# acerbilab/pyvbmc

Measured on AMD Instinct MI355X. Metric: ELBO+entropy evals/sec at D=10, K=50, N=400, Ns=1e6 (1e6-sample-equivalent evals/s), higher is better.
Workload: dtype f64; 1 GPU; BASELINE config 3 per GPU: D=10 K=50 N=400 S=1, Ns=1000000 MC samples per GPU (job Ns=1000000), value+grad _neg_elcbo with soft bounds, eps=philox; parallelism=single GPU

## Files before the change

### include/vbmc_hip.h

```cpp
#ifndef VBMC_HIP_H
#define VBMC_HIP_H

#include <stddef.h>
#include <stdint.h>

#ifdef __cplusplus
extern "C" {
#endif

typedef struct vbmc_ctx vbmc_ctx;

enum {
  VBMC_OK = 0,
  VBMC_E_ARG = -1,
  VBMC_E_HIP = -2,
  VBMC_E_RCCL = -3,
  VBMC_E_NODEV = -4,
  VBMC_E_UNSUP = -5,
  VBMC_E_NONFINITE = -6,
  VBMC_E_NOMEM = -7,
  VBMC_E_NOTPD = -8,
  VBMC_W_GP_CHANGED = 1,
  VBMC_W_NOT_FUSED = 2
};

enum { VBMC_MEAN_ZERO = 0, VBMC_MEAN_CONST = 1, VBMC_MEAN_NEGQUAD = 2 };

enum {
  VBMC_EPS_RESIDENT = 0,
  VBMC_EPS_PHILOX = 1
};


int vbmc_abi_version(void);

int vbmc_device_count(int* n_out);

int vbmc_ctx_create(int device_id, vbmc_ctx** out);
void vbmc_ctx_destroy(vbmc_ctx* ctx);

int vbmc_host_affinity(const vbmc_ctx* ctx, int* bound_out, int* n_cpus_out);

const char* vbmc_last_error(const vbmc_ctx* ctx);

int vbmc_device_info(const vbmc_ctx* ctx, char* name, int name_len, int* cu_count,
                     int* clock_khz, uint64_t* hbm_bytes);

int vbmc_synchronize(vbmc_ctx* ctx);

int vbmc_set_timing(vbmc_ctx* ctx, int on);

int vbmc_last_kernel_ms(vbmc_ctx* ctx, int which, double* ms_out);

int vbmc_last_host_us(const vbmc_ctx* ctx, double out[5]);
int vbmc_last_step_marks(const vbmc_ctx* ctx, double out[4]);
int vbmc_set_release_callback(vbmc_ctx* ctx, void (*fn)(void*), void* user);

int vbmc_set_option(vbmc_ctx* ctx, const char* key, int value);

int vbmc_last_entmc_plan(const vbmc_ctx* ctx, int out[4]);

int vbmc_ws_span_layout(int cus, int pb, int front, int nb, int pad, int K, int64_t* part_lo, int* first_part,
                        int* rows_per_component);

int vbmc_host_checksum(const double* const* ptrs, const int64_t* lens, int n, uint64_t* out);

int vbmc_set_gp_watch(vbmc_ctx* ctx, const double* const* ptrs, const int64_t* lens, int n, uint64_t expected);

int vbmc_armed_stats(const vbmc_ctx* ctx, uint64_t out[6]);

int vbmc_last_elbo_raw(const vbmc_ctx* ctx, double* out, int n);


int vbmc_set_mixture(vbmc_ctx* ctx, int D, int K, const double* mu_KxD,
                     const double* sigma_K, const double* lambd_D, const double* w_K,
                     const double* eta_K);

int vbmc_set_mixture_dk(vbmc_ctx* ctx, int D, int K, const double* mu_DxK,
                        const double* sigma_K, const double* lambd_D, const double* w_K,
                        const double* eta_K);

int vbmc_theta_to_mixture(vbmc_ctx* ctx, const double* theta, int n_theta,
                          int optimize_mask, double* mu_KxD, double* sigma_K,
                          double* lambd_D, double* w_K, double* eta_K);


int vbmc_mixture_pdf(vbmc_ctx* ctx, int64_t n, const double* x_nxD, int log_flag,
                     int grad_flag, double df, double* y_n, double* dy_nxD);


int vbmc_set_eps(vbmc_ctx* ctx, int K, int64_t n_half, int D, const double* eps_half,
                 int64_t row_begin, int64_t row_count);

int vbmc_mt19937_randn(uint32_t* key, int* pos, int* has_gauss, double* gauss, double* out,
                       int64_t n, int n_threads);

int vbmc_mt19937_randn_dev(vbmc_ctx* ctx, uint32_t* key, int* pos, int* has_gauss, double* gauss, double* out,
                           int64_t n);
int vbmc_randn_dev_info(const vbmc_ctx* ctx, int* window_reused);
int vbmc_mt_jump_host(const uint32_t* key_in, uint64_t n_words, uint32_t* key_out);
int vbmc_mt_jump_polys(uint64_t stride_words, int count, uint32_t* out);

int vbmc_set_eps_numpy(vbmc_ctx* ctx, uint32_t* key, int* pos, int* has_gauss, double* gauss, int K,
                       int64_t n_half, int D, int64_t row_begin, int64_t row_count, int n_threads);

int vbmc_entmc(vbmc_ctx* ctx, int64_t ns_per_comp, int eps_mode, uint64_t seed,
               int64_t row_begin, int64_t row_count, int grad_flags, int jacobian_flag,
               double* H, double* dH, double* raw_out);

int vbmc_philox_normals(vbmc_ctx* ctx, int K, int64_t n_half, int D, uint64_t seed, int64_t row_begin,
                        int64_t row_count, double* out);

int vbmc_entmc_finalize(vbmc_ctx* ctx, const double* raw, int grad_flags,
                        int jacobian_flag, double* H, double* dH);

int vbmc_entlb(vbmc_ctx* ctx, int grad_flags, int jacobian_flag, double* H, double* dH);


int vbmc_set_gp(vbmc_ctx* ctx, int N, int D, int S, int P, int mean_kind,
                const double* X_NxD, const double* hyp_SxP, const double* alpha_SxN,
                const double* L_SxNxN, const int32_t* L_chol_S, const double* sW_SxN,
                const double* sn2_mult_S);

int vbmc_gp_posterior(vbmc_ctx* ctx, int N, int D, int S, int P, int mean_kind, const double* X_NxD,
                      const double* y_N, const double* sn2_SxN, const double* sn2_div_S, const double* hyp_SxP,
                      double* alpha_SxN, double* L_SxNxN);

int vbmc_gp_append(vbmc_ctx* ctx, const double* x_D, double y, double* alpha_SxN1, double* L_SxN1xN1);

int vbmc_gp_append_noisy(vbmc_ctx* ctx, const double* x_D, double y, const double* sn2_new_S, double* alpha_SxN1,
                         double* L_SxN1xN1);

int vbmc_gp_fetch(vbmc_ctx* ctx, double* alpha_SxN, double* L_SxNxN);

int vbmc_gp_lml(vbmc_ctx* ctx, int N, int D, int B, int P, int mean_kind, const double* X_NxD, const double* y_N,
                const double* sn2_BxN, const double* sn2_div_B, const double* dsn2_B, const double* hyp_BxP, int want_grad,
                double* lml_B, double* dlml_BxP, int32_t* status_B);

int vbmc_gp_hyp_sample(vbmc_ctx* ctx, int N, int D, int P, int mean_kind, const double* X_NxD, const double* y_N,
                       const double* s2_N, int C, const double* x0_CxP, const double* widths_P, const double* lb_P,
                       const double* ub_P, const double* prior_mu_P, const double* prior_sigma_P, const double* prior_df_P,
                       int n, int thin, int burn_in, uint64_t seed, double* hyp_CxnxP, double* logpost_Cxn,
                       double* logprior_Cxn, int64_t* stats_Cx4, int32_t* invalid_C);

int vbmc_gp_hyp_optimize(vbmc_ctx* ctx, int N, int D, int P, int mean_kind, const double* X_NxD, const double* y_N,
                         const double* s2_N, int R, const double* x0_RxP, const double* lb_P, const double* ub_P,
                         const double* prior_mu_P, const double* prior_sigma_P, const double* prior_df_P, int max_iter, int m,
                         double tol_g, double tol_f, int trace_cap, double* hyp_RxP, double* logpost_R, double* grad_RxP,
                         int64_t* stats_Rx4, int32_t* invalid_R, double* trace_iter, double* trace_eval);

int vbmc_gp_fit(vbmc_ctx* ctx, int N, int D, int P, int mean_kind, const double* X_NxD, const double* y_N,
                const double* s2_N, int H, const double* hyp0_HxP, int init_N, const double* dlb_P, const double* dub_P,
                const double* lb_P, const double* ub_P, const double* prior_mu_P, const double* prior_sigma_P,
                const double* prior_df_P, int opts_N, int max_iter, int m, double tol_g, double tol_f, int n_samples,
                const double* widths_P, int thin, int burn_in, uint64_t seed, double* cand_BxP, double* score_B,
                int32_t* starts_R, double* opt_hyp_RxP, double* opt_logpost_R, int64_t* opt_stats_Rx4,
                int32_t* opt_invalid_R, double* best_P, double* best_logpost, double* hyp_SxP, double* logpost_S,
                double* logprior_S, int64_t* stats_Sx4, double* noise_S, int32_t* status, double* alpha_SxN,
                double* L_SxNxN);


int vbmc_gp_log_joint(vbmc_ctx* ctx, int grad_flags, int avg_flag, int jacobian_flag,
                      int compute_var, double* G, double* dG, double* varG,
                      double* var_ss, double* I_SxK, double* J_SxKxK);


int vbmc_gp_predict(vbmc_ctx* ctx, int64_t M, const double* xs_MxD, int add_noise,
                    int separate_samples, double* fmu, double* fs2);


typedef struct {
  int64_t ns_per_comp;
  int eps_mode;
  uint64_t seed;
  int compute_grad;
  int optimize_mask;
  int64_t row_begin;
  int64_t row_count;
  const double* bnd_lb;
  const double* bnd_ub;
  int n_bnd;
  double tol_con;
  double weight_threshold;
  double weight_penalty;
} vbmc_elbo_opts;

int vbmc_neg_elcbo(vbmc_ctx* ctx, double* theta, int n_theta, const vbmc_elbo_opts* opts,
                   double* F, double* dF, double* G, double* H, double* mu_KxD,
                   double* sigma_K, double* lambd_D, double* w_K, double* eta_K);

typedef struct vbmc_elbo_call {
  double* theta;
  int n_theta;
  const vbmc_elbo_opts* opts;
  double* F;
  double* dF;
  double* G;
  double* H;
  double* mu_KxD;
  double* sigma_K;
  double* lambd_D;
  double* w_K;
  double* eta_K;
} vbmc_elbo_call;
int vbmc_neg_elcbo_call(vbmc_ctx* ctx, const vbmc_elbo_call* c);


int vbmc_neg_elcbo_batch(vbmc_ctx* ctx, const double* thetas_BxN, int B, int n_theta,
                         const vbmc_elbo_opts* opts, double* F_B, double* G_B, double* H_B);


int vbmc_adam_begin(vbmc_ctx* ctx, const double* theta0, int n_theta, const vbmc_elbo_opts* opts,
                    const double* lb, const double* ub, int max_iter, double master_min,
                    double master_max, double master_decay);
int vbmc_adam_run_auto(vbmc_ctx* ctx, int max_iters, double tol_fun, int* n_done, double* y_tab_out,
                       double* x_tab_out, double* G_out, double* H_out);
int vbmc_adam_run(vbmc_ctx* ctx, int n_iters, double* y_tab_out, double* x_tab_out,
                  double* G_out, double* H_out);
int vbmc_adam_end(vbmc_ctx* ctx, double* theta_out, double* mu_KxD, double* sigma_K,
                  double* lambd_D, double* w_K, double* eta_K, int* iterations);


enum {
  VBMC_ACQ_STD = 0,
  VBMC_ACQ_LOG = 1,
  VBMC_ACQ_VANILLA = 2,
  VBMC_ACQ_NOISY = 3
};

int vbmc_acq_eval(vbmc_ctx* ctx, int64_t M, const double* xs_MxD, int kind, double y_max,
                  double tol_gp_var, const double* sn2_M, double* acq_M, double* f_bar_M,
                  double* var_tot_M);

int vbmc_acq_is_set(vbmc_ctx* ctx, int64_t Na, const double* Xa, int per_sample_xa,
                    const double* Ctmp_SxNxNa, const double* fs2a_NaxS, const double* lnw_SxNa);
int vbmc_acq_is_eval(vbmc_ctx* ctx, int64_t M, const double* xs_MxD, const double* sn2_M, double u,
                     double* acq_M, double* var_tot_M );

int vbmc_is_proposal(vbmc_ctx* ctx, int64_t Na, const double* Xa_NaxD, int K2, const double* mu2_KxD,
                     const double* sigma2_K, const double* lambd2_D, const double* w2_K, double w_vp,
                     const double* rect_delta_D, int ln_y_is_fmu, double* lnw_NaxS, double* fs2_NaxS,
                     int* invalid_out);
int vbmc_is_box_sample(vbmc_ctx* ctx, int64_t n_box, uint64_t seed, const double* rect_delta_D, double* x_NboxxD);
int vbmc_acq_is_build(vbmc_ctx* ctx, int64_t Na, const double* Xa, int per_sample_xa, const double* fs2a_NaxS,
                      const double* lnw_SxNa, double* K_out_SxNaxN, double* C_out_SxNxNa);

int vbmc_is_mcmc(vbmc_ctx* ctx, int ln_y_fmu, double u_q, const double* x0_SxD, const double* widths_D,
                 const double* lb_D, const double* ub_D, int n, int thin, int burn_in, uint64_t seed,
                 double* X_SxnxD, double* logp_Sxn, double* fmu_nxS, double* fs2_nxS,
                 int64_t* stats_Sx4 , int* invalid);

int vbmc_sq_dist(vbmc_ctx* ctx, int64_t n, int64_t m, int D, const double* a_nxD,
                 const double* b_mxD, double* c_nxm, int64_t* argmin_n);

enum { VBMC_SRC_COPY = 0, VBMC_SRC_TRANSFORM = 1, VBMC_SRC_MIXTURE = 2, VBMC_SRC_AFFINE = 3, VBMC_SRC_BOX = 4 };
enum { VBMC_ACQ_IS = 4 };
typedef struct vbmc_search_source {
  int kind;
  int64_t rows;
  const double* data;
  double df;
  uint64_t seed;
} vbmc_search_source;
int vbmc_search_fill(vbmc_ctx* ctx, int D, int n_src, const vbmc_search_source* src, const double* lb_search_D,
                     const double* ub_search_D, uint32_t integer_bits, int use_xf, double* X_out_MxD);
int vbmc_search_put(vbmc_ctx* ctx, int64_t M, int D, const double* X_MxD, uint32_t integer_bits, int use_xf);
int vbmc_search_eval(vbmc_ctx* ctx, int kind, double y_max, double tol_gp_var, double u, int64_t n_noise,
                     const double* X_rescaled_NxD, const double* sn2_new_N, const double* length_scale_D, int use_xf,
                     const double* lb_eps_orig_D, const double* ub_eps_orig_D, double* acq_M, int64_t* order_M,
                     double* X_sorted_MxD);

typedef struct vbmc_cmaes_opts {
  int lambda;
  int64_t max_fevals;
  double tol_fun;
  double tol_x;
  uint64_t seed;
} vbmc_cmaes_opts;
int vbmc_search_cmaes(vbmc_ctx* ctx, int kind, double y_max, double tol_gp_var, double u, int64_t n_noise,
                      const double* X_rescaled_NxD, const double* sn2_new_N, const double* length_scale_D, int use_xf,
                      const double* lb_eps_orig_D, const double* ub_eps_orig_D, int R, const double* x0_RxD,
                      const double* sigma0_R, const double* lb_D, const double* ub_D, uint32_t integer_bits,
                      const vbmc_cmaes_opts* opts, double* x_best_RxD, double* f_best_R, double* f0_R, double* mean_RxD,
                      double* sigma_R, double* C_RxDxD, int64_t* stats_Rx4);

typedef struct vbmc_sieve_fill_args {
  int D, K, K_new, optimize_mask;
  int64_t n1, n2, n3;
  const double* mu0_KxD;
  const double* sigma0_K;
  const double* lambd0_D;
  const double* w0_K;
  const double* mu2_KnxD;
  const double* sigma2_Kn;
  const double* lambd_s_D;
  int64_t N_star;
  const double* X_star_NxD;
  double v3;
  const double* Z_BxS;
  int n_slot;
  const int32_t* I_BxKn;
  uint64_t seed;
} vbmc_sieve_fill_args;
int vbmc_sieve_fill(vbmc_ctx* ctx, const vbmc_sieve_fill_args* args, double* thetas_out_BxN);
int vbmc_sieve_put(vbmc_ctx* ctx, int64_t B, int n_theta, const double* thetas_BxN);
int vbmc_sieve_eval(vbmc_ctx* ctx, const vbmc_elbo_opts* opts, double* F_B, double* G_B, double* H_B, int64_t* order_B,
                    double* thetas_sorted_BxN);

int vbmc_elcbo_full(vbmc_ctx* ctx, double* theta, int n_theta, int optimize_mask, int64_t ns_per_comp, int eps_mode,
                    uint64_t seed, int compute_var, double out[7], double* I_SxK, double* J_SxKxK);
int vbmc_elcbo_prune_trial(vbmc_ctx* ctx, int drop, int64_t ns_per_comp, int eps_mode, uint64_t seed, double out[7]);
int vbmc_elcbo_prune_accept(vbmc_ctx* ctx);
int vbmc_elcbo_put(vbmc_ctx* ctx, int S, int K0, const double* I_SxK0, const double* J_SxK0xK0);
int vbmc_elcbo_record_info(const vbmc_ctx* ctx, int64_t info[5], int32_t* alive_K0);


int vbmc_mixture_sample(vbmc_ctx* ctx, int64_t N, uint64_t seed, int balance_flag, double* x_NxD,
                        int32_t* comp_N);
int vbmc_mixture_sample_t(vbmc_ctx* ctx, int64_t N, uint64_t seed, int balance_flag, double df,
                          double* x_NxD, int32_t* comp_N);

int vbmc_kl_div_mc(vbmc_ctx* ctx, int64_t N, uint64_t seed, int K2, const double* mu2_KxD,
                   const double* sigma2_K, const double* lambd2_D, const double* w2_K,
                   double kl_out[2]);

int vbmc_set_transformer(vbmc_ctx* ctx, int slot, int D, const double* type_D, const double* lb_D,
                         const double* ub_D, const double* mu_D, const double* delta_D,
                         const double* R_DxD, const double* scale_D);
int vbmc_clear_transformer(vbmc_ctx* ctx, int slot);

enum { VBMC_XF_FORWARD = 0, VBMC_XF_INVERSE = 1, VBMC_XF_LOG_ABS_DET = 2 };
int vbmc_transform(vbmc_ctx* ctx, int64_t n, int direction, const double* in_nxD, double* out);

int vbmc_mixture_sample_orig(vbmc_ctx* ctx, int64_t N, uint64_t seed, int balance_flag, double df,
                             double* x_NxD, int32_t* comp_N);

int vbmc_mixture_pdf_orig(vbmc_ctx* ctx, int64_t n, const double* x_nxD, int log_flag, int grad_flag,
                          double df, double* y_n, double* dy_nxD);

int vbmc_mixture_moments_orig(vbmc_ctx* ctx, int64_t N, uint64_t seed, int cov_flag, double* mean_D,
                              double* cov_DxD);

int vbmc_kl_div_mc_orig(vbmc_ctx* ctx, int64_t N, uint64_t seed, int K2, const double* mu2_KxD,
                        const double* sigma2_K, const double* lambd2_D, const double* w2_K,
                        double kl_out[2]);

int vbmc_kde_1d(vbmc_ctx* ctx, int ncol, int64_t n, const double* x_colxn, int n_mesh, const double* lb_col,
                const double* ub_col, double* density_colxm, double* xmesh_colxm, double* bandwidth_col,
                int64_t* info_colx2);

enum { VBMC_MTV_HOST = 0, VBMC_MTV_MIX1 = 1, VBMC_MTV_MIX2 = 2 };
typedef struct vbmc_mtv_side {
  int source;
  int64_t n;
  const double* x_NxD;
  uint64_t seed;
  const double* lb_D;
  const double* ub_D;
} vbmc_mtv_side;

int vbmc_mtv(vbmc_ctx* ctx, int D, const vbmc_mtv_side* s1, const vbmc_mtv_side* s2, int K2,
             const double* mu2_KxD, const double* sigma2_K, const double* lambd2_D, const double* w2_K,
             double* mtv_D, int64_t* info_2Dx2);

int vbmc_mixture_mode(vbmc_ctx* ctx, int n_opts, int orig_flag, int64_t n, const double* cand_RxnxD,
                      uint64_t seed, int max_iter, double step_tol, double* x_D, double* f_out,
                      double* rec_Rx5, double* pts_RxD, double* ys_RxD);

enum { VBMC_WARP_FROM_OLD = 0, VBMC_WARP_FROM_ORIG = 1, VBMC_WARP_IN_NEW = 2 };

int vbmc_warp_points(vbmc_ctx* ctx, int D, int64_t n, int source, const double* x_NxD, double* y_NxD, double* lj_new_N,
                     double* lj_old_N);

int vbmc_warp_unscent(vbmc_ctx* ctx, int D, int64_t n, const double* x_NxD, int64_t sigma_rows, const double* sigma,
                      double* mean_NxD, double* std_NxD, double* pts_UxNxD);

int vbmc_warp_gp(vbmc_ctx* ctx, int D, int N, int S, int P, const double* X_NxD, const double* hyp_SxP,
                 double* logell_SxD, double* dy_mean, double* dy_old_mean);

int vbmc_warp_box(vbmc_ctx* ctx, int D, int64_t n, int source, const double* lo_D, const double* hi_D,
                  const double* u_NxD, uint64_t seed, int mode, double* out_2xD, double* sorted_Dxn);


int vbmc_comm_unique_id(uint8_t id_out[128]);
int vbmc_comm_init(vbmc_ctx* ctx, const uint8_t id[128], int rank, int world);
int vbmc_comm_destroy(vbmc_ctx* ctx);
int vbmc_comm_info(vbmc_ctx* ctx, int* rank_out, int* world_out);
int vbmc_comm_allreduce_max(vbmc_ctx* ctx, double* value_inout);
int vbmc_comm_barrier(vbmc_ctx* ctx);

#ifdef __cplusplus
}
#endif
#endif
```

### pyvbmc_amd/_lib.py

```python
import ctypes as C
import os
import sys
import threading
from pathlib import Path

import numpy as np

_HERE = Path(__file__).resolve().parent
LIB_PATH = Path(os.environ.get("VBMC_HIP_LIB", _HERE / "libvbmc_hip.so"))

EPS_RESIDENT, EPS_PHILOX = 0, 1
MEAN_ZERO, MEAN_CONST, MEAN_NEGQUAD = 0, 1, 2
E_ARG, E_HIP, E_RCCL, E_NODEV, E_UNSUP, E_NONFINITE = -1, -2, -3, -4, -5, -6
E_NOTPD = -8
W_GP_CHANGED = 1
W_NOT_FUSED = 2
T_ENTMC, T_GLJ, T_PDF, T_PREDICT, T_ELBO, T_PREDICT_VAR, T_GP_POST, T_IS_MCMC, T_GP_LML = range(9)
T_SEARCH_FILL, T_SEARCH_EVAL, T_SEARCH_SORT = 9, 10, 11
T_GP_HYP = 12
T_SEARCH_CMAES = 13
T_GP_OPT = 14
T_SIEVE_FILL, T_SIEVE_SCORE, T_SIEVE_RANK = 15, 16, 17


class VbmcHipError(RuntimeError):
    def __init__(self, code, msg):
        super().__init__(f"libvbmc_hip error {code}: {msg}")
        self.code = code


class NoDeviceError(VbmcHipError):
    pass


class UnsupportedShape(NotImplementedError):
    """VBMC_E_UNSUP: a shape the kernels do not cover (D > 32, a GP too large for the LDS plans ...).  A
    ``NotImplementedError`` -- there is no CPU fallback inside this package -- that ``pyvbmc_amd.patch`` recognises:
    under the drop-in such a call goes back to the reference callable it replaced (pyvbmc_amd/dropin.py)."""


_dp = C.POINTER(C.c_double)
_vp = C.c_void_p


class ElboOpts(C.Structure):
    _fields_ = [
        ("ns_per_comp", C.c_int64),
        ("eps_mode", C.c_int),
        ("seed", C.c_uint64),
        ("compute_grad", C.c_int),
        ("optimize_mask", C.c_int),
        ("row_begin", C.c_int64),
        ("row_count", C.c_int64),
        ("bnd_lb", _dp),
        ("bnd_ub", _dp),
        ("n_bnd", C.c_int),
        ("tol_con", C.c_double),
        ("weight_threshold", C.c_double),
        ("weight_penalty", C.c_double),
    ]


class ElboCall(C.Structure):

    _fields_ = [
        ("theta", _dp),
        ("n_theta", C.c_int),
        ("opts", C.POINTER(ElboOpts)),
        ("F", _dp),
        ("dF", _dp),
        ("G", _dp),
        ("H", _dp),
        ("mu_KxD", _dp),
        ("sigma_K", _dp),
        ("lambd_D", _dp),
        ("w_K", _dp),
        ("eta_K", _dp),
    ]


MTV_HOST, MTV_MIX1, MTV_MIX2 = 0, 1, 2
KDE_SCOTT, KDE_DEGENERATE, KDE_ROOT_STUCK = 1, 4, 8


class MtvSide(C.Structure):

    _fields_ = [
        ("source", C.c_int),
        ("n", C.c_int64),
        ("x_NxD", _dp),
        ("seed", C.c_uint64),
        ("lb_D", _dp),
        ("ub_D", _dp),
    ]


SRC_COPY, SRC_TRANSFORM, SRC_MIXTURE, SRC_AFFINE, SRC_BOX = range(5)
ACQ_IS = 4


class SearchSource(C.Structure):

    _fields_ = [
        ("kind", C.c_int),
        ("rows", C.c_int64),
        ("data", _dp),
        ("df", C.c_double),
        ("seed", C.c_uint64),
    ]


class SieveFillArgs(C.Structure):

    _fields_ = [
        ("D", C.c_int),
        ("K", C.c_int),
        ("K_new", C.c_int),
        ("optimize_mask", C.c_int),
        ("n1", C.c_int64),
        ("n2", C.c_int64),
        ("n3", C.c_int64),
        ("mu0_KxD", _dp),
        ("sigma0_K", _dp),
        ("lambd0_D", _dp),
        ("w0_K", _dp),
        ("mu2_KnxD", _dp),
        ("sigma2_Kn", _dp),
        ("lambd_s_D", _dp),
        ("N_star", C.c_int64),
        ("X_star_NxD", _dp),
        ("v3", C.c_double),
        ("Z_BxS", _dp),
        ("n_slot", C.c_int),
        ("I_BxKn", C.POINTER(C.c_int32)),
        ("seed", C.c_uint64),
    ]


class CmaesOpts(C.Structure):

    _fields_ = [
        ("lam", C.c_int),
        ("max_fevals", C.c_int64),
        ("tol_fun", C.c_double),
        ("tol_x", C.c_double),
        ("seed", C.c_uint64),
    ]


SIGNATURES = {
    "vbmc_abi_version": (C.c_int, []),
    "vbmc_device_count": (C.c_int, [C.POINTER(C.c_int)]),
    "vbmc_ctx_create": (C.c_int, [C.c_int, C.POINTER(_vp)]),
    "vbmc_ctx_destroy": (None, [_vp]),
    "vbmc_last_error": (C.c_char_p, [_vp]),
    "vbmc_device_info": (
        C.c_int,
        [_vp, C.c_char_p, C.c_int, C.POINTER(C.c_int), C.POINTER(C.c_int), C.POINTER(C.c_uint64)],
    ),
    "vbmc_host_affinity": (C.c_int, [_vp, C.POINTER(C.c_int), C.POINTER(C.c_int)]),
    "vbmc_synchronize": (C.c_int, [_vp]),
    "vbmc_set_option": (C.c_int, [_vp, C.c_char_p, C.c_int]),
    "vbmc_last_entmc_plan": (C.c_int, [_vp, C.POINTER(C.c_int)]),
    "vbmc_ws_span_layout": (C.c_int, [C.c_int, C.c_int, C.c_int, C.c_int, C.c_int, C.c_int, C.POINTER(C.c_int64),
                                      C.POINTER(C.c_int), C.POINTER(C.c_int)]),
    "vbmc_last_elbo_raw": (C.c_int, [_vp, _dp, C.c_int]),
    "vbmc_armed_stats": (C.c_int, [_vp, C.POINTER(C.c_uint64)]),
    "vbmc_set_gp_watch": (C.c_int, [_vp, C.POINTER(C.c_void_p), C.POINTER(C.c_int64), C.c_int, C.c_uint64]),
    "vbmc_host_checksum": (C.c_int, [C.POINTER(C.c_void_p), C.POINTER(C.c_int64), C.c_int, C.POINTER(C.c_uint64)]),
    "vbmc_set_timing": (C.c_int, [_vp, C.c_int]),
    "vbmc_last_kernel_ms": (C.c_int, [_vp, C.c_int, _dp]),
    "vbmc_last_host_us": (C.c_int, [_vp, _dp]),
    "vbmc_last_step_marks": (C.c_int, [_vp, _dp]),
    "vbmc_set_release_callback": (C.c_int, [_vp, C.c_void_p, C.c_void_p]),
    "vbmc_set_mixture": (C.c_int, [_vp, C.c_int, C.c_int, _dp, _dp, _dp, _dp, _dp]),
    "vbmc_set_mixture_dk": (C.c_int, [_vp, C.c_int, C.c_int, _dp, _dp, _dp, _dp, _dp]),
    "vbmc_theta_to_mixture": (C.c_int, [_vp, _dp, C.c_int, C.c_int, _dp, _dp, _dp, _dp, _dp]),
    "vbmc_mixture_pdf": (C.c_int, [_vp, C.c_int64, _dp, C.c_int, C.c_int, C.c_double, _dp, _dp]),
    "vbmc_set_eps": (C.c_int, [_vp, C.c_int, C.c_int64, C.c_int, _dp, C.c_int64, C.c_int64]),
    "vbmc_mt19937_randn": (
        C.c_int,
        [C.POINTER(C.c_uint32), C.POINTER(C.c_int), C.POINTER(C.c_int), _dp, _dp, C.c_int64, C.c_int],
    ),
    "vbmc_randn_dev_info": (C.c_int, [_vp, C.POINTER(C.c_int)]),
    "vbmc_mt19937_randn_dev": (
        C.c_int,
        [_vp, C.POINTER(C.c_uint32), C.POINTER(C.c_int), C.POINTER(C.c_int), _dp, _dp, C.c_int64],
    ),
    "vbmc_mt_jump_host": (C.c_int, [C.POINTER(C.c_uint32), C.c_uint64, C.POINTER(C.c_uint32)]),
    "vbmc_mt_jump_polys": (C.c_int, [C.c_uint64, C.c_int, C.POINTER(C.c_uint32)]),
    "vbmc_set_eps_numpy": (
        C.c_int,
        [_vp, C.POINTER(C.c_uint32), C.POINTER(C.c_int), C.POINTER(C.c_int), _dp, C.c_int, C.c_int64, C.c_int,
         C.c_int64, C.c_int64, C.c_int],
    ),
    "vbmc_entmc": (
        C.c_int,
        [_vp, C.c_int64, C.c_int, C.c_uint64, C.c_int64, C.c_int64, C.c_int, C.c_int, _dp, _dp, _dp],
    ),
    "vbmc_philox_normals": (C.c_int, [_vp, C.c_int, C.c_int64, C.c_int, C.c_uint64, C.c_int64, C.c_int64, _dp]),
    "vbmc_entmc_finalize": (C.c_int, [_vp, _dp, C.c_int, C.c_int, _dp, _dp]),
    "vbmc_entlb": (C.c_int, [_vp, C.c_int, C.c_int, _dp, _dp]),
    "vbmc_set_gp": (
        C.c_int,
        [_vp, C.c_int, C.c_int, C.c_int, C.c_int, C.c_int, _dp, _dp, _dp, _dp,
         C.POINTER(C.c_int32), _dp, _dp],
    ),
    "vbmc_gp_posterior": (
        C.c_int,
        [_vp, C.c_int, C.c_int, C.c_int, C.c_int, C.c_int, _dp, _dp, _dp, _dp, _dp, _dp, _dp],
    ),
    "vbmc_gp_append": (C.c_int, [_vp, _dp, C.c_double, _dp, _dp]),
    "vbmc_gp_append_noisy": (C.c_int, [_vp, _dp, C.c_double, _dp, _dp, _dp]),
    "vbmc_gp_fetch": (C.c_int, [_vp, _dp, _dp]),
    "vbmc_gp_lml": (
        C.c_int,
        [_vp, C.c_int, C.c_int, C.c_int, C.c_int, C.c_int, _dp, _dp, _dp, _dp, _dp, _dp, C.c_int, _dp, _dp,
         C.POINTER(C.c_int32)],
    ),
    "vbmc_gp_hyp_sample": (
        C.c_int,
        [_vp, C.c_int, C.c_int, C.c_int, C.c_int, _dp, _dp, _dp, C.c_int, _dp, _dp, _dp, _dp, _dp, _dp, _dp, C.c_int, C.c_int,
         C.c_int, C.c_uint64, _dp, _dp, _dp, C.POINTER(C.c_int64), C.POINTER(C.c_int32)],
    ),
    "vbmc_gp_hyp_optimize": (
        C.c_int,
        [_vp, C.c_int, C.c_int, C.c_int, C.c_int, _dp, _dp, _dp, C.c_int, _dp, _dp, _dp, _dp, _dp, _dp, C.c_int, C.c_int,
         C.c_double, C.c_double, C.c_int, _dp, _dp, _dp, C.POINTER(C.c_int64), C.POINTER(C.c_int32), _dp, _dp],
    ),
    "vbmc_gp_fit": (
        C.c_int,
        [_vp, C.c_int, C.c_int, C.c_int, C.c_int, _dp, _dp, _dp, C.c_int, _dp, C.c_int, _dp, _dp, _dp, _dp, _dp, _dp, _dp,
         C.c_int, C.c_int, C.c_int, C.c_double, C.c_double, C.c_int, _dp, C.c_int, C.c_int, C.c_uint64, _dp, _dp,
         C.POINTER(C.c_int32), _dp, _dp, C.POINTER(C.c_int64), C.POINTER(C.c_int32), _dp, _dp, _dp, _dp, _dp,
         C.POINTER(C.c_int64), _dp, C.POINTER(C.c_int32), _dp, _dp],
    ),
    "vbmc_gp_log_joint": (
        C.c_int,
        [_vp, C.c_int, C.c_int, C.c_int, C.c_int, _dp, _dp, _dp, _dp, _dp, _dp],
    ),
    "vbmc_gp_predict": (C.c_int, [_vp, C.c_int64, _dp, C.c_int, C.c_int, _dp, _dp]),
    "vbmc_neg_elcbo": (
        C.c_int,
        [_vp, _dp, C.c_int, C.POINTER(ElboOpts), _dp, _dp, _dp, _dp, _dp, _dp, _dp, _dp, _dp],
    ),
    "vbmc_neg_elcbo_call": (C.c_int, [_vp, C.POINTER(ElboCall)]),
    "vbmc_neg_elcbo_batch": (
        C.c_int,
        [_vp, _dp, C.c_int, C.c_int, C.POINTER(ElboOpts), _dp, _dp, _dp],
    ),
    "vbmc_adam_begin": (
        C.c_int,
        [_vp, _dp, C.c_int, C.POINTER(ElboOpts), _dp, _dp, C.c_int, C.c_double, C.c_double, C.c_double],
    ),
    "vbmc_adam_run": (C.c_int, [_vp, C.c_int, _dp, _dp, _dp, _dp]),
    "vbmc_adam_run_auto": (C.c_int, [_vp, C.c_int, C.c_double, C.POINTER(C.c_int), _dp, _dp, _dp, _dp]),
    "vbmc_adam_end": (C.c_int, [_vp, _dp, _dp, _dp, _dp, _dp, _dp, C.POINTER(C.c_int)]),
    "vbmc_acq_eval": (
        C.c_int,
        [_vp, C.c_int64, _dp, C.c_int, C.c_double, C.c_double, _dp, _dp, _dp, _dp],
    ),
    "vbmc_acq_is_set": (C.c_int, [_vp, C.c_int64, _dp, C.c_int, _dp, _dp, _dp]),
    "vbmc_acq_is_eval": (C.c_int, [_vp, C.c_int64, _dp, _dp, C.c_double, _dp, _dp]),
    "vbmc_is_proposal": (C.c_int, [_vp, C.c_int64, _dp, C.c_int, _dp, _dp, _dp, _dp, C.c_double, _dp, C.c_int, _dp, _dp,
                                   C.POINTER(C.c_int)]),
    "vbmc_is_box_sample": (C.c_int, [_vp, C.c_int64, C.c_uint64, _dp, _dp]),
    "vbmc_acq_is_build": (C.c_int, [_vp, C.c_int64, _dp, C.c_int, _dp, _dp, _dp, _dp]),
    "vbmc_is_mcmc": (C.c_int, [_vp, C.c_int, C.c_double, _dp, _dp, _dp, _dp, C.c_int, C.c_int, C.c_int, C.c_uint64, _dp, _dp,
                               _dp, _dp, C.POINTER(C.c_int64), C.POINTER(C.c_int)]),
    "vbmc_sq_dist": (C.c_int, [_vp, C.c_int64, C.c_int64, C.c_int, _dp, _dp, _dp, C.POINTER(C.c_int64)]),
    "vbmc_search_fill": (C.c_int, [_vp, C.c_int, C.c_int, C.POINTER(SearchSource), _dp, _dp, C.c_uint32, C.c_int, _dp]),
    "vbmc_search_put": (C.c_int, [_vp, C.c_int64, C.c_int, _dp, C.c_uint32, C.c_int]),
    "vbmc_search_eval": (C.c_int, [_vp, C.c_int, C.c_double, C.c_double, C.c_double, C.c_int64, _dp, _dp, _dp, C.c_int, _dp,
                                   _dp, _dp, C.POINTER(C.c_int64), _dp]),
    "vbmc_search_cmaes": (C.c_int, [_vp, C.c_int, C.c_double, C.c_double, C.c_double, C.c_int64, _dp, _dp, _dp, C.c_int, _dp,
                                    _dp, C.c_int, _dp, _dp, _dp, _dp, C.c_uint32, C.POINTER(CmaesOpts), _dp, _dp, _dp, _dp,
                                    _dp, _dp, C.POINTER(C.c_int64)]),
    "vbmc_sieve_fill": (C.c_int, [_vp, C.POINTER(SieveFillArgs), _dp]),
    "vbmc_sieve_put": (C.c_int, [_vp, C.c_int64, C.c_int, _dp]),
    "vbmc_sieve_eval": (C.c_int, [_vp, C.POINTER(ElboOpts), _dp, _dp, _dp, C.POINTER(C.c_int64), _dp]),
    "vbmc_elcbo_full": (C.c_int, [_vp, _dp, C.c_int, C.c_int, C.c_int64, C.c_int, C.c_uint64, C.c_int, _dp, _dp, _dp]),
    "vbmc_elcbo_prune_trial": (C.c_int, [_vp, C.c_int, C.c_int64, C.c_int, C.c_uint64, _dp]),
    "vbmc_elcbo_prune_accept": (C.c_int, [_vp]),
    "vbmc_elcbo_put": (C.c_int, [_vp, C.c_int, C.c_int, _dp, _dp]),
    "vbmc_elcbo_record_info": (C.c_int, [_vp, C.POINTER(C.c_int64), C.POINTER(C.c_int32)]),
    "vbmc_mixture_sample": (C.c_int, [_vp, C.c_int64, C.c_uint64, C.c_int, _dp, C.POINTER(C.c_int32)]),
    "vbmc_mixture_sample_t": (C.c_int, [_vp, C.c_int64, C.c_uint64, C.c_int, C.c_double, _dp, C.POINTER(C.c_int32)]),
    "vbmc_kl_div_mc": (C.c_int, [_vp, C.c_int64, C.c_uint64, C.c_int, _dp, _dp, _dp, _dp, _dp]),
    "vbmc_set_transformer": (C.c_int, [_vp, C.c_int, C.c_int, _dp, _dp, _dp, _dp, _dp, _dp, _dp]),
    "vbmc_clear_transformer": (C.c_int, [_vp, C.c_int]),
    "vbmc_transform": (C.c_int, [_vp, C.c_int64, C.c_int, _dp, _dp]),
    "vbmc_mixture_sample_orig": (C.c_int, [_vp, C.c_int64, C.c_uint64, C.c_int, C.c_double, _dp, C.POINTER(C.c_int32)]),
    "vbmc_mixture_pdf_orig": (C.c_int, [_vp, C.c_int64, _dp, C.c_int, C.c_int, C.c_double, _dp, _dp]),
    "vbmc_mixture_moments_orig": (C.c_int, [_vp, C.c_int64, C.c_uint64, C.c_int, _dp, _dp]),
    "vbmc_kl_div_mc_orig": (C.c_int, [_vp, C.c_int64, C.c_uint64, C.c_int, _dp, _dp, _dp, _dp, _dp]),
    "vbmc_kde_1d": (C.c_int, [_vp, C.c_int, C.c_int64, _dp, C.c_int, _dp, _dp, _dp, _dp, _dp, C.POINTER(C.c_int64)]),
    "vbmc_mtv": (C.c_int, [_vp, C.c_int, C.POINTER(MtvSide), C.POINTER(MtvSide), C.c_int, _dp, _dp, _dp, _dp, _dp,
                           C.POINTER(C.c_int64)]),
    "vbmc_mixture_mode": (C.c_int, [_vp, C.c_int, C.c_int, C.c_int64, _dp, C.c_uint64, C.c_int, C.c_double, _dp, _dp,
                                    _dp, _dp, _dp]),
    "vbmc_warp_points": (C.c_int, [_vp, C.c_int, C.c_int64, C.c_int, _dp, _dp, _dp, _dp]),
    "vbmc_warp_unscent": (C.c_int, [_vp, C.c_int, C.c_int64, _dp, C.c_int64, _dp, _dp, _dp, _dp]),
    "vbmc_warp_gp": (C.c_int, [_vp, C.c_int, C.c_int, C.c_int, C.c_int, _dp, _dp, _dp, _dp, _dp]),
    "vbmc_warp_box": (C.c_int, [_vp, C.c_int, C.c_int64, C.c_int, _dp, _dp, _dp, C.c_uint64, C.c_int, _dp, _dp]),
    "vbmc_comm_unique_id": (C.c_int, [C.POINTER(C.c_uint8)]),
    "vbmc_comm_init": (C.c_int, [_vp, C.POINTER(C.c_uint8), C.c_int, C.c_int]),
    "vbmc_comm_destroy": (C.c_int, [_vp]),
    "vbmc_comm_info": (C.c_int, [_vp, C.POINTER(C.c_int), C.POINTER(C.c_int)]),
    "vbmc_comm_allreduce_max": (C.c_int, [_vp, _dp]),
    "vbmc_comm_barrier": (C.c_int, [_vp]),
}

_lib = None
_lib_lock = threading.Lock()


def load():
    global _lib
    with _lib_lock:
        if _lib is None:
            if not LIB_PATH.exists():
                raise ImportError(
                    f"{LIB_PATH} not found: build it with `python -m pyvbmc_amd.build` "
                    "(hipcc, gfx950).  pyvbmc_amd has no CPU fallback."
                )
            lib = C.CDLL(str(LIB_PATH), mode=C.RTLD_GLOBAL)
            for name, (res, args) in SIGNATURES.items():
                fn = getattr(lib, name)
                fn.restype = res
                fn.argtypes = args
            _lib = lib
    return _lib


def device_count():
    n = C.c_int(0)
    load().vbmc_device_count(C.byref(n))
    return n.value


def f64(a):
    return np.ascontiguousarray(a, dtype=np.float64)


def ptr(a):
    if a is None:
        return None
    assert a.dtype == np.float64 and a.flags["C_CONTIGUOUS"]
    return a.ctypes.data_as(_dp)


def flags_to_bits(flags):
    if np.isscalar(flags):
        return 15 if flags else 0
    return sum((1 << i) for i, f in enumerate(flags) if f)


class Context:

    def __init__(self, device=None):
        lib = load()
        if device is None:
            device = int(os.environ.get("VBMC_HIP_DEVICE", os.environ.get("LOCAL_RANK", "0")))
        h = _vp()
        rc = lib.vbmc_ctx_create(int(device), C.byref(h))
        if rc != 0:
            msg = (lib.vbmc_last_error(None) or b"").decode()
            raise (NoDeviceError if rc == E_NODEV else VbmcHipError)(rc, msg)
        self._h = h
        self._lib = lib
        self.device = int(device)
        self.rank, self.world = 0, 1

    def close(self):
        if getattr(self, "_h", None):
            self.__dict__.pop("_fused_last", None)
            self.__dict__.pop("_fused_cache", None)
            vo = sys.modules.get(__package__ + ".variational_optimization")
            if vo is not None:
                fs = vo._fast_last[0]
                if fs is not None and fs.ctx is self:
                    vo._fast_last[0] = None
            self._lib.vbmc_ctx_destroy(self._h)
            self._h = None

    def __del__(self):
        try:
            self.close()
        except Exception:
            pass

    def check(self, rc):
        if rc != 0:
            msg = (self._lib.vbmc_last_error(self._h) or b"").decode()
            if rc == E_UNSUP:
                raise UnsupportedShape(msg)
            if rc == E_ARG:
                raise ValueError(msg)
            if rc == E_NODEV:
                raise NoDeviceError(rc, msg)
            if rc == E_NOTPD:
                raise np.linalg.LinAlgError(msg)
            raise VbmcHipError(rc, msg)

    def device_info(self):
        name = C.create_string_buffer(256)
        cu, clk, mem = C.c_int(), C.c_int(), C.c_uint64()
        self.check(self._lib.vbmc_device_info(self._h, name, 256, C.byref(cu), C.byref(clk), C.byref(mem)))
        return {"name": name.value.decode(), "cu_count": cu.value, "clock_khz": clk.value,
                "hbm_bytes": mem.value}

    def host_affinity(self):
        b, n = C.c_int(), C.c_int()
        self.check(self._lib.vbmc_host_affinity(self._h, C.byref(b), C.byref(n)))
        return bool(b.value), n.value

    def synchronize(self):
        self.check(self._lib.vbmc_synchronize(self._h))

    def set_timing(self, on):
        self.check(self._lib.vbmc_set_timing(self._h, int(on) if on else 0))

    def set_option(self, key, value):
        self.check(self._lib.vbmc_set_option(self._h, key.encode(), int(value)))

    def last_entmc_plan(self):
        out = (C.c_int * 4)()
        self.check(self._lib.vbmc_last_entmc_plan(self._h, out))
        return {"kernel": ("valu", "ws", "small", "mfma", "adam_fused", "ws", "ws")[out[0]] if out[0] >= 0 else None, "rg": out[1],
                "chunks": out[2], "resident_draws": bool(out[3] & 1), "roles": bool(out[3] & 2), "span": out[0] in (5, 6), "adam_tail": out[0] == 6}

    def philox_normals(self, K, n_half, D, seed, row_begin=0, row_count=None):
        row_count = n_half - row_begin if row_count is None else row_count
        out = np.empty((K, row_count, D))
        self.check(self._lib.vbmc_philox_normals(self._h, K, n_half, D, C.c_uint64(seed), row_begin, row_count, ptr(out)))
        return out

    def armed_stats(self):
        out = (C.c_uint64 * 6)()
        self.check(self._lib.vbmc_armed_stats(self._h, out))
        return dict(zip(("hits", "cancels", "late", "ident_checked", "ident_bad", "lost"), (int(v) for v in out)))

    def last_elbo_raw(self, D, K):
        out = np.empty(1 + D * K + 2 * K + D)
        self.check(self._lib.vbmc_last_elbo_raw(self._h, ptr(out), out.size))
        return out

    def last_kernel_ms(self, which=T_ENTMC):
        v = C.c_double()
        self.check(self._lib.vbmc_last_kernel_ms(self._h, which, C.byref(v)))
        return v.value

    def last_host_us(self):
        out = np.zeros(5)
        self.check(self._lib.vbmc_last_host_us(self._h, ptr(out)))
        return out

    def last_step_marks(self):
        out = np.zeros(4)
        self.check(self._lib.vbmc_last_step_marks(self._h, ptr(out)))
        return {"gp_word_us": out[0], "entropy_word_us": out[1],
                "gp_sums_in": ("prep launch", "finish launch", "entropy launch")[int(out[2])]}

    def set_mixture(self, mu_DK, sigma, lambd, w, eta):
        mu_DK = np.asarray(mu_DK, dtype=np.float64)
        D, K = mu_DK.shape
        mu_kd = f64(mu_DK.T)
        s, l, ww = f64(np.ravel(sigma)), f64(np.ravel(lambd)), f64(np.ravel(w))
        e = f64(np.ravel(eta)) if eta is not None and np.size(eta) == K else None
        if s.size != K or l.size != D or ww.size != K:
            raise ValueError("mixture attribute shapes do not match (D, K)")
        self.check(self._lib.vbmc_set_mixture(self._h, D, K, ptr(mu_kd), ptr(s), ptr(l), ptr(ww), ptr(e)))
        self.D, self.K = D, K

    def mixture_changed(self, D, K):
        self.__dict__["_vp_args"] = None
        self.D, self.K = int(D), int(K)
        vo = sys.modules.get(__package__ + ".variational_optimization")
        if vo is not None:
            vo.clear_fast_path()

    def set_eps(self, eps_half, row_begin=0, row_count=None):
        eps_half = f64(eps_half)
        K, h, D = eps_half.shape
        if row_count is None:
            row_count = h - row_begin
        self.check(self._lib.vbmc_set_eps(self._h, K, h, D, ptr(eps_half), row_begin, row_count))

    def set_eps_numpy(self, K, n_half, D, row_begin=0, row_count=None, threads=0, view=None):
        if row_count is None:
            row_count = n_half - row_begin
        with NP_STREAM_LOCK:
            left = self.__dict__.get("_np_left")
            fp = view() if view is not None and left is not None else None
            if fp is not None and fp == left and view._words is not None:
                bg, words = view._bg, view._words
                has_gauss, gauss = C.c_int(0), C.c_double(0.0)
                with bg.lock:
                    addr = C.addressof(words)
                    rc = self._lib.vbmc_set_eps_numpy(self._h, C.cast(addr, C.POINTER(C.c_uint32)),
                                                      C.cast(addr + 624 * 4, C.POINTER(C.c_int)), C.byref(has_gauss),
                                                      C.byref(gauss), K, n_half, D, row_begin, row_count,
                                                      threads or host_threads())
                    if has_gauss.value:
                        key = np.array(words[:624], dtype=np.uint32)
                        pos = int(words[624])
                if has_gauss.value:
                    np.random.set_state(("MT19937", key, pos, has_gauss.value, gauss.value))
                    self.__dict__["_np_left"] = None
                else:
                    self.__dict__["_np_left"] = view()
                self.check(rc)
                return True
            st = np.random.get_state(legacy=True)
            if not isinstance(st, tuple) or st[0] != "MT19937":
                return False
            key = np.array(st[1], dtype=np.uint32)
            pos, has_gauss, gauss = C.c_int(int(st[2])), C.c_int(int(st[3])), C.c_double(float(st[4]))
            rc = self._lib.vbmc_set_eps_numpy(self._h, key.ctypes.data_as(C.POINTER(C.c_uint32)), C.byref(pos),
                                              C.byref(has_gauss), C.byref(gauss), K, n_half, D, row_begin, row_count,
                                              threads or host_threads())
            np.random.set_state(("MT19937", key, pos.value, has_gauss.value, gauss.value))
            self.__dict__["_np_left"] = view() if view is not None and has_gauss.value == 0 else None
        self.check(rc)
        return True

    def comm_init(self, uid_bytes, rank, world):
        buf = (C.c_uint8 * 128).from_buffer_copy(uid_bytes)
        self.check(self._lib.vbmc_comm_init(self._h, buf, rank, world))
        self.rank, self.world = rank, world

    def comm_info(self):
        r, w = C.c_int(), C.c_int()
        self.check(self._lib.vbmc_comm_info(self._h, C.byref(r), C.byref(w)))
        return r.value, w.value

    def comm_barrier(self):
        self.check(self._lib.vbmc_comm_barrier(self._h))

    def comm_max(self, value):
        v = C.c_double(value)
        self.check(self._lib.vbmc_comm_allreduce_max(self._h, C.byref(v)))
        return v.value


def comm_unique_id():
    buf = (C.c_uint8 * 128)()
    rc = load().vbmc_comm_unique_id(buf)
    if rc != 0:
        raise VbmcHipError(rc, (load().vbmc_last_error(None) or b"").decode())
    return bytes(buf)


NP_STREAM_LOCK = threading.Lock()


def host_threads():
    try:
        n = len(os.sched_getaffinity(0))
    except (AttributeError, OSError):
        n = os.cpu_count() or 1
    return max(1, min(64, n))


_default_ctx = None


def default_context():
    global _default_ctx
    if _default_ctx is None:
        _default_ctx = Context()
    return _default_ctx


def set_default_context(ctx):
    global _default_ctx
    _default_ctx = ctx
```

### pyvbmc_amd/csrc/api_elbo.hip

```cpp
#include <algorithm>
#include <chrono>
#include <cstdlib>
#include <cmath>
#include <cstring>

#include "common.h"
#include "entropy_args.h"

static double soft_bound_loss(const std::vector<double>& x, const double* lb, const double* ub,
                              double tol_con, std::vector<double>* dy) {
  double y = 0.0;
  if (dy) dy->assign(x.size(), 0.0);
  for (size_t i = 0; i < x.size(); ++i) {
    if (x[i] >= lb[i] && x[i] <= ub[i]) continue;
    const double ell = (ub[i] - lb[i]) * tol_con;
    if (x[i] < lb[i]) {
      const double t = (lb[i] - x[i]) / ell;
      y += 0.5 * t * t;
      if (dy) (*dy)[i] = (x[i] - lb[i]) / (ell * ell);
    }
    if (x[i] > ub[i]) {
      const double t = (x[i] - ub[i]) / ell;
      y += 0.5 * t * t;
      if (dy) (*dy)[i] = (x[i] - ub[i]) / (ell * ell);
    }
  }
  return y;
}

#ifdef FIN_TIMES
static int64_t g_host_stamps[64][6];
static uint64_t g_host_n = 0;
static inline int64_t host_ns() {
  return std::chrono::duration_cast<std::chrono::nanoseconds>(std::chrono::steady_clock::now().time_since_epoch()).count();
}
namespace {
__global__ void clock_stamp_kernel(unsigned long long* out) {
  if (threadIdx.x == 0) __hip_atomic_store(out, (unsigned long long)wall_clock64(), __ATOMIC_RELAXED, __HIP_MEMORY_SCOPE_SYSTEM);
}
}
extern "C" int vbmc_debug_host_stamps(int64_t* out) {
  memcpy(out, g_host_stamps, sizeof(g_host_stamps));
  return (int)(g_host_n & 63);
}
extern "C" int vbmc_debug_clock_pair(vbmc_ctx* ctx, int64_t* host_before, int64_t* host_after, unsigned long long* gpu) {
  volatile unsigned long long* f = (volatile unsigned long long*)(ctx->h_done + 6);
  *f = 0;
  (void)hipStreamSynchronize(ctx->stream);
  *host_before = host_ns();
  hipLaunchKernelGGL(clock_stamp_kernel, dim3(1), dim3(64), 0, ctx->stream, (unsigned long long*)(ctx->hd_done + 6));
  while (*f == 0) __builtin_ia32_pause();
  *host_after = host_ns();
  *gpu = *f;
  return 0;
}
#define HSTAMP(i) g_host_stamps[g_host_n & 63][i] = host_ns()
#else
#define HSTAMP(i) (void)0
#endif

static inline uint64_t* ctl_word(vbmc_ctx* ctx, uint64_t seq) { return ctx->d_ctl + (seq & 7); }

void spec_disarm(vbmc_ctx* ctx) {
  vbmc_ctx::ArmedEval& sp = ctx->spec;
  if (!sp.armed) return;
  *(volatile uint64_t*)ctl_word(ctx, sp.seq) = ~(uint64_t)0;
  __builtin_ia32_sfence();
  sp.armed = false;
  ++sp.cancels;
  ctx->gen_cur = sp.gen_cur_before;
  ctx->ahead.valid = sp.ahead_before_valid;
  ctx->ahead.seed = sp.ahead_before_seed;
  ctx->ahead.buf = sp.ahead_before_buf;
  ctx->ahead.frac = sp.ahead_before_frac;
}

extern "C" int vbmc_neg_elcbo(vbmc_ctx* ctx, double* theta, int n_theta,
                              const vbmc_elbo_opts* opts, double* F, double* dF, double* G,
                              double* H, double* mu_KxD, double* sigma_K, double* lambd_D,
                              double* w_K, double* eta_K) {
  if (!ctx || !theta || !opts) return VBMC_E_ARG;
  struct KeepArmed {
    vbmc_ctx* c;
    explicit KeepArmed(vbmc_ctx* c_) : c(c_) { c->spec.keep = true; }
    ~KeepArmed() { c->spec.keep = false; }
  } keep_armed(ctx);
  NEED_DEVICE(ctx);
  if (!ctx->mix_set) return vbmc_fail(ctx, VBMC_E_ARG, "neg_elcbo: mixture (D,K) not set");
  if (!ctx->gp.set) return vbmc_fail(ctx, VBMC_E_ARG, "neg_elcbo: GP not set");
  if (ctx->gp.D != ctx->D) return vbmc_fail(ctx, VBMC_E_ARG, "neg_elcbo: GP/mixture D mismatch");
  using clk = std::chrono::steady_clock;
  const auto t_begin = clk::now();
  HSTAMP(0);
  auto us_since = [](clk::time_point a) {
    return std::chrono::duration<double, std::micro>(clk::now() - a).count();
  };
  const int D = ctx->D, K = ctx->K;
  const int mask = opts->optimize_mask;
  const ThetaMap tm(D, K, mask, n_theta);
  ctx->defer_mix_upload = true;
  int rc = vbmc_theta_to_mixture(ctx, theta, n_theta, mask, mu_KxD, sigma_K, lambd_D, w_K, eta_K);
  ctx->defer_mix_upload = false;
  if (rc) return rc;
  if (tm.o_w()) {
    double* e = theta + (n_theta - K);
    double mx = e[0];
    for (int k = 1; k < K; ++k) mx = e[k] > mx ? e[k] : mx;
    for (int k = 0; k < K; ++k) e[k] -= mx;
  }
  const int grad_flags = opts->compute_grad ? mask : 0;
  const GpState& g = ctx->gp;
  const int S = g.S;
  const int st = 1 + 2 * D;
  const size_t n_res = (size_t)S * K * st;
  const int n_raw = raw_len(D, K);
  const bool mc = opts->ns_per_comp > 0;
  const bool lb_dev = !mc && K > 1;

  int64_t row_begin = opts->row_begin, row_count = opts->row_count;
  if (mc) {
    if (opts->ns_per_comp & 1)
      return vbmc_fail(ctx, VBMC_E_ARG, "neg_elcbo: ns_per_comp must be even");
    rc = resolve_row_slice(ctx, opts, "neg_elcbo", &row_begin, &row_count);
    if (rc) return rc;
  }

  rc = ensure_pinned(ctx, n_res + (size_t)n_raw);
  if (rc) return rc;
  double* hp_dev = ctx->hp_dev;
  double* res_out = hp_dev;
  double* raw_host = hp_dev + n_res;
  const bool multi = ctx_is_multi(ctx);
  double* raw_out = raw_host;
  if (multi && mc) {
    rc = ensure_dev(ctx, &ctx->d_out, &ctx->d_out_cap, (size_t)n_raw);
    if (rc) return rc;
    raw_out = ctx->d_out;
  }

  ctx->host_us[0] = us_since(t_begin);
  const auto t_launch = clk::now();
  const bool can_poll = mc;
  double* stage = nullptr;
  if (can_poll) {
    rc = ensure_dev(ctx, &ctx->d_stage, &ctx->d_stage_cap, n_res + (size_t)n_raw);
    if (rc) return rc;
    stage = ctx->d_stage;
  }
  vbmc_ctx::ArmedEval& sp = ctx->spec;
  constexpr double ARM_MAX_EVAL_US = 1000.0, ARM_LIMIT_MS = 0.3, ARM_DEVICE_WAIT_MS = 0.5;
  const bool arm_allowed = ctx->opt_elbo_arm >= 2 || (ctx->opt_elbo_arm == 1 && vbmc_live_contexts_on(ctx->device) <= 1);
  const bool arm_next = can_poll && !multi && arm_allowed && ctx->opt_mix_bar && !ctx->timing &&
                        opts->eps_mode == VBMC_EPS_PHILOX && ctx->host_us[4] <= ARM_MAX_EVAL_US;
  constexpr double ARM_LATE_SLACK_MS = 0.15;
  const double arm_limit_ms = 1e-3 * ctx->host_us[4] + ARM_LIMIT_MS;
  static_assert(ARM_LIMIT_MS + ARM_LATE_SLACK_MS < ARM_DEVICE_WAIT_MS, "the host's cut-off must come before the device's");

  bool polled = false;
  uint64_t cur_seq = 0;
  bool ident_out_flag = false;
  auto issue = [&](uint64_t seed, bool spin, bool& polled_out, uint64_t& seq_out) -> int {
    int rc2;
    PrepArgs pa;
    glj_fill_prep(ctx, grad_flags != 0, res_out, nullptr, pa);
    EntPlan plan;
    if (mc) {
      rc2 = entmc_plan(ctx, opts->ns_per_comp, opts->eps_mode, seed, row_begin, row_count, grad_flags != 0, plan,
                       pa.n_glj);
      if (rc2) return rc2;
      entmc_fill_prep(ctx, plan, pa);
      rc2 = entmc_pregen(ctx, plan, pa);
      if (rc2) return rc2;
    }
    const bool ahead_ok = can_poll && opts->eps_mode == VBMC_EPS_PHILOX && ctx->opt_elbo_ahead &&
                          plan.a.eps != nullptr && plan.a.eps == ctx->d_epsgen[ctx->gen_cur];
    const bool ws_form = plan.kernel == EntKernel::Ws || plan.kernel == EntKernel::WsSpan || plan.kernel == EntKernel::Mfma;
    if (spin && !(ahead_ok && plan.pregen_hit && ws_form))
      return -1000;
    if (can_poll) {
      pa.done.cnt = ctx->d_done_cnt + 8;
      pa.done.flag = ctx->hd_done + 4;
      pa.done.seq = ++ctx->done_seq;
      pa.done.host_out = res_out;
      pa.done.host_n = (int)n_res;
      pa.res = stage;
    }
    seq_out = ctx->done_seq;
    ident_out_flag = false;
    ctx->gp_where = 0;
    double* fg = nullptr;
    if (can_poll && ctx->opt_mix_bar) fg = spin ? ctx->d_mix_fg : write_pack_to_device(ctx);
    if (spin && !fg) return -1000;
    const bool ident = fg != nullptr && mc;
    if (ident) pa.ident_out = (uint64_t*)(ctx->d_done_cnt + 12);
    if (fg) {
      PrepArgs gp_tail = pa;
      gp_tail.n_table = 0;
      gp_tail.gen = GenSlice();
      gp_tail.mix = ctx->d_mix;
      if (entmc_take_gp(ctx, plan, gp_tail)) {
        pa.n_glj = 0;
        ctx->gp_where = 2;
      }
      if (mc && pa.n_glj > 0 && pa.done.flag != nullptr && ctx->opt_gp_ship && plan.kernel == EntKernel::Mfma) {
        plan.a.ship_src = pa.res;
        plan.a.ship_dst = pa.done.host_out;
        plan.a.ship_n = pa.done.host_n;
        plan.a.ship_flag = pa.done.flag;
        plan.a.ship_seq = pa.done.seq;
        pa.done = DoneSignal();
      }
      pa.mix = fg;
      pa.mix_copy = ctx->d_mix;
      pa.mix_copy_n = ctx->ml.total;
    } else {
      rc2 = upload_packed_mixture(ctx);
      if (rc2) return rc2;
    }
    uint64_t* ctl = nullptr;
    if (spin) {
      ctl = ctl_word(ctx, seq_out);
      *(volatile uint64_t*)ctl = 0;
      __builtin_ia32_sfence();
      pa.go = ctl;
      pa.go_seq = seq_out;
      pa.go_timeout = (uint64_t)(ARM_DEVICE_WAIT_MS * 1e5);
      pa.dead = ctx->hd_done + 5;
      plan.a.cancel = ctl;
    }
    HSTAMP(1);
    rc2 = launch_prep(ctx, pa);
    if (rc2) return rc2;
    polled_out = false;
    if (mc) {
      rc2 = entmc_launch_main(ctx, plan);
      if (rc2) return rc2;
      GenSlice ahead_gen;
      DoneSignal done;
      if (can_poll) {
        if (ahead_ok) ahead_gen = entmc_ahead_slice(ctx, plan);
        done.cnt = ctx->d_done_cnt;
        done.sub = ctx->d_done_sub;
        {
          static const int sub_min = [] { const char* e = getenv("VBMC_FIN_SUB_MIN"); return e ? atoi(e) : 256; }();
          done.sub_min = sub_min;
        }
        done.flag = ctx->hd_done;
        done.seq = seq_out;
        done.host_out = raw_out;
        done.host_n = n_raw;
        done.cancel = ctl;
        if (ident) {
          done.ident_src = (const uint64_t*)(ctx->d_done_cnt + 12);
          done.ident_dst = ctx->hd_done + 1;
          done.ident_seed = seed;
        }
        polled_out = true;
        ident_out_flag = ident;
      }
      const GenSlice* gen_here = ahead_gen.n_blocks > 0 ? &ahead_gen : nullptr;
      if (!multi) {
        rc2 = entmc_launch_finish(ctx, plan, polled_out ? stage + n_res : raw_out, gen_here, polled_out ? &done : nullptr);
        if (rc2) return rc2;
      } else {
        rc2 = entmc_launch_finish(ctx, plan, raw_out, nullptr, nullptr);
        if (rc2) return rc2;
        rc2 = comm_allreduce_sum(ctx, raw_out, n_raw);
        if (rc2) return rc2;
        if (polled_out) {
          done.host_out = raw_host;
          rc2 = entmc_launch_publish(ctx, raw_out, done, gen_here);
          if (rc2) return rc2;
        } else {
          HIP_TRY(ctx, hipMemcpyAsync(ctx->h_pinned + n_res, raw_out, sizeof(double) * n_raw,
                                      hipMemcpyDeviceToHost, ctx->stream));
        }
      }
    } else if (lb_dev) {
      rc2 = launch_entlb(ctx, raw_host);
      if (rc2) return rc2;
    }
    return 0;
  };

  uint64_t want_ck = 0;
  bool check_ident = false;
  bool used_armed = false;
  if (sp.armed) {
    const bool match = can_poll && sp.seed == opts->seed && sp.n_theta == n_theta && sp.mask == mask &&
                       sp.grad_flags == grad_flags && sp.eps_mode == opts->eps_mode &&
                       sp.ns_per_comp == opts->ns_per_comp && sp.row_begin == row_begin && sp.row_count == row_count &&
                       !ctx->timing &&
                       std::chrono::duration<double, std::milli>(clk::now() - sp.t_armed).count() < sp.limit_ms;
    if (match) {
      memcpy(ctx->d_mix_fg, ctx->h_pack, sizeof(double) * (size_t)ctx->ml.total);
      __builtin_ia32_sfence();
      *(volatile uint64_t*)ctl_word(ctx, sp.seq) = sp.seq;
      __builtin_ia32_sfence();
      ctx->pack_valid = true;
      sp.armed = false;
      const bool force_late = ctx->opt_arm_late_test > 0 && --ctx->opt_arm_late_test == 0;
      if (!force_late && std::chrono::duration<double, std::milli>(clk::now() - sp.t_armed).count() < sp.limit_ms + ARM_LATE_SLACK_MS) {
        ++sp.hits;
        used_armed = true;
        polled = true;
        cur_seq = sp.seq;
        check_ident = sp.ident;
        HSTAMP(1);
      } else {
        *(volatile uint64_t*)ctl_word(ctx, sp.seq) = ~(uint64_t)0;
        __builtin_ia32_sfence();
        HIP_TRY(ctx, stream_wait(ctx));
        HIP_TRY(ctx, hipMemsetAsync(ctx->d_done_cnt, 0, sizeof(int) * 16, ctx->stream));
        HIP_TRY(ctx, hipMemsetAsync(ctx->d_done_sub, 0, sizeof(int) * 16 * 64, ctx->stream));
        ctx->gen_cur = sp.gen_cur_before;
        ctx->ahead.valid = sp.ahead_before_valid;
        ctx->ahead.seed = sp.ahead_before_seed;
        ctx->ahead.buf = sp.ahead_before_buf;
        ctx->ahead.frac = sp.ahead_before_frac;
        ++sp.cancels;
        ++sp.late;
      }
    } else {
      spec_disarm(ctx);
    }
  }
  if (!used_armed) {
    rc = issue(opts->seed, false, polled, cur_seq);
    if (rc) return rc;
    check_ident = polled && ident_out_flag;
  }
  if (mc && can_poll && ctx->opt_mix_bar) want_ck = pack_checksum(ctx->h_pack, (size_t)ctx->ml.total);
  ctx->step_marks[2] = (double)ctx->gp_where;
  if (polled && arm_next && ctx->d_ctl && ctx->d_mix_fg) {
    sp.gen_cur_before = ctx->gen_cur;
    sp.ahead_before_valid = ctx->ahead.valid;
    sp.ahead_before_seed = ctx->ahead.seed;
    sp.ahead_before_buf = ctx->ahead.buf;
    sp.ahead_before_frac = ctx->ahead.frac;
    const uint64_t seq_before = ctx->done_seq;
    bool p2 = false;
    uint64_t seq2 = 0;
    const auto t_arm0 = clk::now();
    const int rc2 = issue(opts->seed + 1, true, p2, seq2);
    if (rc2 == 0 && p2) {
      sp.armed = true;
      sp.ident = ident_out_flag;
      sp.limit_ms = arm_limit_ms;
      sp.t_armed = t_arm0;
      sp.seq = seq2;
      sp.seed = opts->seed + 1;
      sp.n_theta = n_theta;
      sp.mask = mask;
      sp.grad_flags = grad_flags;
      sp.eps_mode = opts->eps_mode;
      sp.ns_per_comp = opts->ns_per_comp;
      sp.row_begin = row_begin;
      sp.row_count = row_count;
    } else if (rc2 == -1000) {
      ctx->done_seq = seq_before;
      ctx->gen_cur = sp.gen_cur_before;
      ctx->ahead.valid = sp.ahead_before_valid;
      ctx->ahead.seed = sp.ahead_before_seed;
      ctx->ahead.buf = sp.ahead_before_buf;
      ctx->ahead.frac = sp.ahead_before_frac;
    } else if (rc2 != 0) {
      return rc2;
    }
  }
  if (ctx->release_cb && !ctx->ident_retry) ctx->release_cb(ctx->release_cb_user);
  ElboScratch& sc = ctx->elbo;
  const bool has_bnd = opts->bnd_lb && opts->bnd_ub;
  double F_bnd = 0.0;
  std::vector<double>& dFb = sc.dFb;
  if (has_bnd && grad_flags) dFb.assign((size_t)n_theta, 0.0);
  if (has_bnd) {
    if (tm.n_bnd() != opts->n_bnd)
      return vbmc_fail(ctx, VBMC_E_ARG, "neg_elcbo: bounds length %d != %d", opts->n_bnd, tm.n_bnd());
    std::vector<double>& ext = sc.ext;
    ext.resize((size_t)tm.n_bnd());
    const int sc0 = tm.p_sg;
    for (int i = 0; i < tm.n_bnd(); ++i) ext[i] = tm.bound_coord(i, theta, ctx->sigma.data(), ctx->lambd.data());
    std::vector<double>& dL = sc.dL;
    const double L = soft_bound_loss(ext, opts->bnd_lb, opts->bnd_ub, opts->tol_con,
                                     grad_flags ? &dL : nullptr);
    F_bnd += L;
    if (grad_flags) {
      if (tm.o_mu())
        for (int i = 0; i < D * K; ++i) dFb[i] += dL[i];
      if (tm.o_sg())
        for (int k = 0; k < K; ++k) {
          double a = 0.0;
          for (int d = 0; d < D; ++d) a += dL[sc0 + d * K + k];
          dFb[tm.p_sg + k] += a;
        }
      if (tm.o_lm())
        for (int d = 0; d < D; ++d) {
          double a = 0.0;
          for (int k = 0; k < K; ++k) a += dL[sc0 + d * K + k];
          dFb[tm.p_lm + d] += a;
        }
      if (tm.o_w())
        for (int k = 0; k < K; ++k) dFb[tm.p_w + k] += dL[dL.size() - K + k];
    }
    if (tm.o_w()) {
      const double th = opts->weight_threshold, pen = opts->weight_penalty;
      double a = 0.0;
      std::vector<double>& wg = sc.wpen;
      wg.resize(K);
      for (int k = 0; k < K; ++k) {
        const bool small = ctx->w[k] < th;
        a += small ? ctx->w[k] : th;
        wg[k] = small ? pen : 0.0;
      }
      F_bnd += a * pen;
      if (grad_flags) {
        std::vector<double>& jw = sc.jw;
        jw.resize(K);
        softmax_jacobian_apply(ctx, wg.data(), jw.data());
        for (int k = 0; k < K; ++k) dFb[n_theta - K + k] += jw[k];
      }
    }
  }
  bool gp_changed = false;
  if (!ctx->gp_watch_ptrs.empty()) {
    uint64_t ck = 0;
    vbmc_host_checksum(ctx->gp_watch_ptrs.data(), ctx->gp_watch_lens.data(), (int)ctx->gp_watch_ptrs.size(), &ck);
    gp_changed = ck != ctx->gp_watch_ck;
  }
  ctx->host_us[1] = us_since(t_launch);
  HSTAMP(2);
  const auto t_wait = clk::now();
  auto spin_on = [&](const volatile uint64_t* f, uint64_t want) -> int {
    const volatile uint64_t* dead = ctx->h_done + 5;
    unsigned spins = 0;
    for (;;) {
      if (*f == want) break;
      if (*dead == want) return 1;
      __builtin_ia32_pause();
      if ((++spins & 0xFFFF) == 0 && us_since(t_wait) > 5e6) return 2;
    }
    __atomic_thread_fence(__ATOMIC_ACQUIRE);
    return 0;
  };
  auto redo_unarmed = [&](const char* why) -> int {
    HIP_TRY(ctx, stream_wait(ctx));
    HIP_TRY(ctx, hipMemsetAsync(ctx->d_done_cnt, 0, sizeof(int) * 16, ctx->stream));
        HIP_TRY(ctx, hipMemsetAsync(ctx->d_done_sub, 0, sizeof(int) * 16 * 64, ctx->stream));
    ctx->ahead.valid = false;
    if (ctx->ident_retry) return vbmc_fail(ctx, VBMC_E_HIP, "neg_elcbo: %s, twice in a row", why);
    ctx->ident_retry = true;
    const int arm_was = ctx->opt_elbo_arm;
    ctx->opt_elbo_arm = 0;
    const int rc3 = vbmc_neg_elcbo(ctx, theta, n_theta, opts, F, dF, G, H, mu_KxD, sigma_K, lambd_D, w_K, eta_K);
    ctx->opt_elbo_arm = arm_was;
    ctx->ident_retry = false;
    ctx->spec.keep = true;
    return rc3;
  };
  GljHost& o = sc.glj;
  double Gv = 0.0;
  std::vector<double>&dGv = sc.dG, &dHv = sc.dH;
  auto finalize_gp = [&]() -> int {
    glj_finalize(ctx, ctx->h_pinned, grad_flags != 0, o);
    for (int s = 0; s < S; ++s) Gv += o.G[s];
    Gv /= S;
    dGv.assign((size_t)n_theta, 0.0);
    if (grad_flags) {
      std::vector<double>&mu = sc.mu, &sg = sc.sg, &lm = sc.lm, &wg = sc.wg;
      mu.assign((size_t)K * D, 0.0);
      sg.assign(K, 0.0);
      lm.assign(D, 0.0);
      wg.assign(K, 0.0);
      for (int s = 0; s < S; ++s) {
        for (int i = 0; i < K * D; ++i) mu[i] += o.mu[(size_t)s * K * D + i] / S;
        for (int k = 0; k < K; ++k) sg[k] += o.sigma[(size_t)s * K + k] / S;
        for (int d = 0; d < D; ++d) lm[d] += o.lambd[(size_t)s * D + d] / S;
        for (int k = 0; k < K; ++k) wg[k] += o.w[(size_t)s * K + k] / S;
      }
      const int n = glj_pack(ctx, mu.data(), sg.data(), lm.data(), wg.data(), grad_flags, 1, dGv.data());
      if (n != n_theta) return vbmc_fail(ctx, VBMC_E_ARG, "neg_elcbo: gradient length %d != n_theta %d", n, n_theta);
    }
    return 0;
  };
  bool gp_done = false;
  if (polled) {
    int st_w = spin_on(ctx->h_done + 4, cur_seq);
    HSTAMP(3);
    ctx->step_marks[0] = us_since(t_begin);
    if (st_w == 0) {
      rc = finalize_gp();
      if (rc) return rc;
      gp_done = true;
      st_w = spin_on(ctx->h_done, cur_seq);
    }
    if (st_w != 0) {
      ++sp.lost;
      return redo_unarmed(st_w == 1 ? "the armed launches gave up before the go word reached them"
                                    : "no completion word from the device after 5 s");
    }
    if (check_ident) {
      const volatile uint64_t* id = ctx->h_done + 1;
      ++sp.ident_checked;
      const bool force_bad = ctx->opt_ident_test > 0 && --ctx->opt_ident_test == 0;
      if (force_bad || id[0] != want_ck || id[1] != opts->seed) {
        ++sp.ident_bad;
        return redo_unarmed("the result block does not identify as this evaluation");
      }
    }
  } else {
    HIP_TRY(ctx, stream_wait(ctx));
  }
  ctx->pack_in_flight = false;
  ctx->step_marks[1] = us_since(t_begin);
  if (!polled) ctx->step_marks[0] = ctx->step_marks[1];
  ctx->host_us[2] = us_since(t_wait);
  HSTAMP(4);
  const auto t_fin = clk::now();
  if (!gp_done) {
    rc = finalize_gp();
    if (rc) return rc;
  }
  dHv.assign((size_t)n_theta, 0.0);
  double Hv = 0.0;
  if (mc || lb_dev) {
    const double* r = ctx->h_pinned + n_res;
    entropy_pack(ctx, r[0], r + 1, r + 1 + D * K, r + 1 + D * K + K, r + 1 + D * K + K + D,
                 grad_flags, 1, &Hv, grad_flags ? dHv.data() : nullptr);
  } else {
    rc = vbmc_entlb(ctx, grad_flags, 1, &Hv, grad_flags ? dHv.data() : nullptr);
    if (rc) return rc;
  }
  ctx->last_raw_off = n_res;
  ctx->last_raw_n = mc ? n_raw : 0;
  double Fv = -Gv - Hv;
  std::vector<double>& dFv = sc.dF;
  dFv.assign((size_t)n_theta, 0.0);
  if (grad_flags)
    for (int i = 0; i < n_theta; ++i) dFv[i] = -dGv[i] - dHv[i];

  Fv += F_bnd;
  if (grad_flags && has_bnd)
    for (int i = 0; i < n_theta; ++i) dFv[i] += dFb[i];
  ctx->host_us[3] = us_since(t_fin);
  ctx->host_us[4] = us_since(t_begin);
#ifdef FIN_TIMES
  HSTAMP(5);
  ++g_host_n;
#endif
  if (F) *F = Fv;
  if (G) *G = Gv;
  if (H) *H = Hv;
  if (dF && grad_flags) memcpy(dF, dFv.data(), sizeof(double) * n_theta);
  return gp_changed ? VBMC_W_GP_CHANGED : VBMC_OK;
}

extern "C" int vbmc_neg_elcbo_call(vbmc_ctx* ctx, const vbmc_elbo_call* c) {
  if (!c) return VBMC_E_ARG;
  return vbmc_neg_elcbo(ctx, c->theta, c->n_theta, c->opts, c->F, c->dF, c->G, c->H, c->mu_KxD, c->sigma_K, c->lambd_D, c->w_K,
                        c->eta_K);
}

extern "C" int vbmc_armed_stats(const vbmc_ctx* ctx, uint64_t out[6]) {
  if (!ctx || !out) return VBMC_E_ARG;
  const vbmc_ctx::ArmedEval& sp = ctx->spec;
  out[0] = sp.hits;
  out[1] = sp.cancels;
  out[2] = sp.late;
  out[3] = sp.ident_checked;
  out[4] = sp.ident_bad;
  out[5] = sp.lost;
  return VBMC_OK;
}

extern "C" int vbmc_last_elbo_raw(const vbmc_ctx* ctx, double* out, int n) {
  if (!ctx || !out || ctx->last_raw_n <= 0 || n != ctx->last_raw_n || !ctx->h_pinned) return VBMC_E_ARG;
  memcpy(out, ctx->h_pinned + ctx->last_raw_off, sizeof(double) * (size_t)n);
  return VBMC_OK;
}

extern "C" int vbmc_set_release_callback(vbmc_ctx* ctx, void (*fn)(void*), void* user) {
  if (!ctx) return VBMC_E_ARG;
  ctx->release_cb = fn;
  ctx->release_cb_user = user;
  return VBMC_OK;
}

extern "C" int vbmc_last_step_marks(const vbmc_ctx* ctx, double out[4]) {
  if (!ctx || !out) return VBMC_E_ARG;
  for (int i = 0; i < 4; ++i) out[i] = ctx->step_marks[i];
  return VBMC_OK;
}

extern "C" int vbmc_last_host_us(const vbmc_ctx* ctx, double out[5]) {
  if (!ctx || !out) return VBMC_E_ARG;
  for (int i = 0; i < 5; ++i) out[i] = ctx->host_us[i];
  return VBMC_OK;
}
```

### pyvbmc_amd/csrc/common.h

```cpp
#pragma once
#include <hip/hip_runtime.h>
#include <chrono>

#include <cstdint>
#include <cstdio>
#include <string>
#include <vector>

#include "../../include/vbmc_hip.h"
#include "gp_cand_host.h"
#include "gp_fit_host.h"
#include "scratch.h"
#include "transform.h"

struct ncclComm;

struct MixLayout {
  int D = 0, K = 0;
  int o_mup = 0;
  int o_mu = 0;
  int o_is2 = 0;
  int o_wc = 0;
  int o_rc = 0;
  int o_lrc = 0;
  int o_sig = 0;
  int o_w = 0;
  int o_lam = 0;
  int o_ilam = 0;
  int total = 0;
  void plan(int D_, int K_) {
    D = D_;
    K = K_;
    int o = 0;
    o_mup = o; o += K * D;
    o_mu = o; o += K * D;
    o_is2 = o; o += K;
    o_wc = o; o += K;
    o_rc = o; o += K;
    o_lrc = o; o += K;
    o_sig = o; o += K;
    o_w = o; o += K;
    o_lam = o; o += D;
    o_ilam = o; o += D;
    total = o;
  }
};

struct ThetaMap {
  int D, K;
  int mask;
  __host__ __device__ bool o_mu() const { return mask & 1; }
  __host__ __device__ bool o_sg() const { return mask & 2; }
  __host__ __device__ bool o_lm() const { return mask & 4; }
  __host__ __device__ bool o_w() const { return mask & 8; }
  int p_sg, p_lm, p_w;
  int n_sc;
  __host__ __device__ ThetaMap(int D_, int K_, int mask_) : ThetaMap(D_, K_, mask_, 0) { p_w = n_theta() - K; }
  __host__ __device__ ThetaMap(int D_, int K_, int mask_, int n_theta_)
      : D(D_), K(K_), mask(mask_), p_sg((mask_ & 1) ? D_ * K_ : 0), p_lm(p_sg + ((mask_ & 2) ? K_ : 0)), p_w(n_theta_ - K_),
        n_sc((mask_ & 6) ? D_ * K_ : 0) {}
  __host__ __device__ int n_theta() const { return p_lm + (o_lm() ? D : 0) + (o_w() ? K : 0); }
  __host__ __device__ int n_bnd() const { return p_sg + n_sc + (o_w() ? K : 0); }
  __host__ __device__ bool in_mu(int i) const { return o_mu() && i < D * K; }
  __host__ __device__ bool in_sg(int i) const { return o_sg() && i >= p_sg && i < p_sg + K; }
  __host__ __device__ bool in_lm(int i) const { return o_lm() && i >= p_lm && i < p_lm + D; }
  __host__ __device__ int raw_w() const { return 1 + D * K + K + D; }
  __host__ __device__ int raw_index(int i) const {
    if (o_w() && i >= p_w) return raw_w() + (i - p_w);
    if (o_lm() && i >= p_lm) return 1 + D * K + K + (i - p_lm);
    if (o_sg() && i >= p_sg) return 1 + D * K + (i - p_sg);
    return 1 + i;
  }
  __host__ __device__ double bound_coord(int i, const double* theta, const double* sigma, const double* lambda) const {
    double x;
    if (i < p_sg) {
      x = theta[i];
    } else if (i < p_sg + n_sc) {
      const int q = i - p_sg, k = q / D, d = q - k * D;
      const double ls = o_sg() ? theta[p_sg + k] : log(sigma[k]);
      const double ll = o_lm() ? theta[p_lm + d] : log(lambda[d]);
      x = ll + ls;
    } else {
      x = theta[p_w + (i - p_sg - n_sc)];
    }
    return x;
  }
};

struct GpState {
  bool set = false;
  int N = 0, D = 0, S = 0, P = 0, mean_kind = 0;
  std::vector<double> hyp;
  std::vector<int32_t> L_chol;
  std::vector<double> sn2_eff;
  std::vector<double> sn2_mult;
  double* d_X = nullptr;
  double* d_XT = nullptr;
  double* d_alpha = nullptr;
  double* d_L = nullptr;
  double* d_Linv = nullptr;
  double* d_LinvP = nullptr;
  double* d_sW = nullptr;
  double* d_hyp = nullptr;
  double* d_xc = nullptr;
  double* d_smeta = nullptr;
  size_t cap_X = 0, cap_XT = 0, cap_alpha = 0, cap_L = 0, cap_Linv = 0, cap_LinvP = 0, cap_sW = 0, cap_hyp = 0, cap_xc = 0, cap_smeta = 0;
  std::vector<double> h_small;
  std::vector<double> h_XT;
  bool dev_built = false;
  bool homo = false;
  double* d_y = nullptr;
  double* d_r = nullptr;
  double* d_sn2 = nullptr;
  double* d_sl = nullptr;
  size_t cap_y = 0, cap_r = 0, cap_sn2 = 0, cap_sl = 0;
  std::vector<double> h_X, h_y, h_sl;
  std::vector<double> h_sn2;
};

struct GljHost {
  std::vector<double> G;
  std::vector<double> I_sk;
  std::vector<double> mu;
  std::vector<double> sigma;
  std::vector<double> lambd;
  std::vector<double> w;
};

struct ElboScratch {
  GljHost glj;
  std::vector<double> dG, dH, dF, dFb, mu, sg, lm, wg, ext, dL, wpen, jw;
};

enum TimingPair { T_ENTMC = 0, T_GLJ, T_PDF, T_PREDICT, T_ELBO, T_PREDICT_VAR, T_GP_POST, T_IS_MCMC, T_GP_LML, T_SEARCH_FILL,
                  T_SEARCH_EVAL, T_SEARCH_SORT, T_GP_HYP, T_SEARCH_CMAES, T_GP_OPT, T_SIEVE_FILL, T_SIEVE_SCORE, T_SIEVE_RANK, T_COUNT };

struct vbmc_ctx {
  int device = 0;
  hipStream_t stream = nullptr;
  hipEvent_t ev[2 * T_COUNT] = {};
  bool ev_valid[T_COUNT] = {};
  std::string err;
  hipDeviceProp_t prop;

  bool mix_set = false;
  int D = 0, K = 0;
  std::vector<double> mu, sigma, lambd, w, eta;
  MixLayout ml;
  double* d_mix = nullptr;
  struct ArmedEval {
    bool armed = false;
    bool keep = false;
    uint64_t seq = 0;
    uint64_t seed = 0;
    int n_theta = 0, mask = 0, grad_flags = 0, eps_mode = 0;
    int64_t ns_per_comp = 0, row_begin = 0, row_count = 0;
    int gen_cur_before = 0;
    bool ahead_before_valid = false;
    uint64_t ahead_before_seed = 0;
    int ahead_before_buf = 0;
    double ahead_before_frac = 1.0;
    uint64_t hits = 0, cancels = 0, late = 0, ident_checked = 0, ident_bad = 0, lost = 0;
    bool ident = false;
    double limit_ms = 1.0;
    std::chrono::steady_clock::time_point t_armed;
  } spec;
  uint64_t* d_ctl = nullptr;
  double* d_stage = nullptr;
  size_t d_stage_cap = 0;
  double* d_mix_fg = nullptr;
  std::vector<double> mu_scratch;
  std::vector<double> t2m_mu, t2m_sg, t2m_lm, t2m_w, t2m_eta;
  double* d_acq_fg = nullptr;
  bool acq_fg_failed = false;
  uint64_t acq_seq = 0;
  size_t d_mix_fg_cap = 0;
  bool mix_fg_failed = false;
  size_t d_mix_cap = 0;

  double* d_epsgen[2] = {nullptr, nullptr};
  size_t d_epsgen_cap[2] = {0, 0};
  int gen_cur = 0;
  struct AheadDraws {
    bool valid = false;
    uint64_t seed = 0;
    int K = 0, D = 0, buf = 0;
    int64_t rows = 0, n_half = 0, row_begin = 0;
    double frac = 1.0;
  } ahead;
  uint64_t* h_done = nullptr;
  uint64_t* hd_done = nullptr;
  int* d_done_cnt = nullptr;
  int* d_done_sub = nullptr;
  uint64_t done_seq = 0;

  double* d_eps = nullptr;
  size_t d_eps_cap = 0;
  int eps_K = 0, eps_D = 0;
  int64_t eps_rows = 0, eps_row_begin = 0, eps_n_half = 0;

  double* d_scratch = nullptr;
  size_t d_scratch_cap = 0;
  double* d_out = nullptr;
  size_t d_out_cap = 0;
  double* d_ptick = nullptr;
  size_t d_ptick_cap = 0;
  double* h_pinned = nullptr;
  double* h_eps = nullptr;
  size_t h_eps_cap = 0;
  size_t h_pinned_cap = 0;
  double* h_pack = nullptr;
  size_t h_pack_cap = 0;
  bool pack_in_flight = false;
  bool pack_valid = false;
  bool defer_mix_upload = false;
  double* hp_dev = nullptr;
  int timing = 0;
  double host_us[5] = {0, 0, 0, 0, 0};
  double step_marks[4] = {0, 0, 0, 0};
  int gp_where = 0;
  int opt_entmc_valu = 0;
  int opt_gp_ship = 1;
  int opt_entmc_mfma = 1;
  int opt_elbo_pregen = 1;
  int opt_elbo_ahead = 1;
  int opt_predict_dma = 1;
  int opt_predict_fused = 1;
  int opt_arm_late_test = 0;
  int opt_acq_poll = 1;
  int opt_is_mcmc_threads = 512;
  int opt_gp_lml_chunk = 0;
  int opt_gp_hyp_rounds = 4;
  int opt_gp_opt_rounds = 4;
  int opt_cmaes_rounds = 8;
  void (*release_cb)(void*) = nullptr;
  void* release_cb_user = nullptr;
  int opt_adam_fused = 1;
  int opt_adam_tail = 1;
  int opt_ident_test = 0;
  bool ident_retry = false;
  int opt_elbo_arm = 1;
  bool counted = false;
  int opt_ws_span = 1;
  int opt_ws_front = 0;
  int opt_ws_pad = -1;
  int opt_ws_roles = 1;
  int opt_mix_bar = 1;
  double* h_pack_dev = nullptr;
  double* h_pack_dev_of = nullptr;
  std::vector<double> exp_eta;
  double exp_eta_sum = 0.0;
  bool exp_eta_valid = false;
  int last_plan[4] = {-1, 0, 0, 0};
  size_t last_raw_off = 0;
  int last_raw_n = 0;

  GpState gp;
  GpState gp_next;
  double* d_post_ws = nullptr;
  size_t d_post_ws_cap = 0;

  ncclComm* comm = nullptr;
  int rank = 0, world = 1;

  std::vector<const double*> gp_watch_ptrs;
  std::vector<int64_t> gp_watch_lens;
  uint64_t gp_watch_ck = 0;

  ElboScratch elbo;
  void* adam = nullptr;
  void* acq_is = nullptr;
  bool host_bound = false;
  int host_cpus = 0;
  void* randn_dev = nullptr;
  int randn_last_reused = 0;
  int opt_randn_dev = 1;
  void* xf = nullptr;
  void* search = nullptr;
  void* sieve = nullptr;
  void* elcbo = nullptr;
  uint64_t stream_waits = 0;
  uint64_t gp_launches = 0;
};
inline int ctx_cus(const vbmc_ctx* ctx) { return ctx->prop.multiProcessorCount > 0 ? ctx->prop.multiProcessorCount : 256; }
int vbmc_live_contexts_on(int device);
void adam_free(vbmc_ctx* ctx);
void acq_is_free(vbmc_ctx* ctx);
void randn_dev_free(vbmc_ctx* ctx);
void xf_free(vbmc_ctx* ctx);
void search_free(vbmc_ctx* ctx);
void sieve_free(vbmc_ctx* ctx);
void elcbo_free(vbmc_ctx* ctx);
int randn_device(vbmc_ctx* ctx, uint32_t* key, int* pos, int* has_gauss, double* gauss, double* d_out, int64_t n);

int vbmc_fail(vbmc_ctx* ctx, int code, const char* fmt, ...);
extern thread_local std::string g_create_err;

#define HIP_TRY(ctx, call)                                                            \
  do {                                                                                \
    hipError_t e_ = (call);                                                           \
    if (e_ != hipSuccess)                                                             \
      return vbmc_fail((ctx), VBMC_E_HIP, "%s failed: %s (%s:%d)", #call,             \
                       hipGetErrorString(e_), __FILE__, __LINE__);                    \
  } while (0)

#define VBMC_DISPATCH_DP(D, CALL)   \
  do {                              \
    if ((D) <= 2) CALL(2);          \
    else if ((D) <= 4) CALL(4);     \
    else if ((D) <= 6) CALL(6);     \
    else if ((D) <= 8) CALL(8);     \
    else if ((D) <= 10) CALL(10);   \
    else if ((D) <= 12) CALL(12);   \
    else if ((D) <= 16) CALL(16);   \
    else if ((D) <= 20) CALL(20);   \
    else if ((D) <= 24) CALL(24);   \
    else CALL(32);                  \
  } while (0)

void spec_disarm(vbmc_ctx* ctx);
#define NEED_DEVICE(ctx)                                                                     \
  do {                                                                                       \
    if ((ctx)->device < 0)                                                                   \
      return vbmc_fail((ctx), VBMC_E_NODEV,                                                  \
                       "host-only context: this entry point needs a gfx950 device "          \
                       "(libvbmc_hip has no CPU fallback)");                                 \
    if ((ctx)->spec.armed && !(ctx)->spec.keep) spec_disarm(ctx);                            \
  } while (0)

void write_mixture_pack(const MixLayout& ml, const double* mu_KxD, const double* sigma,
                        const double* lambd, const double* w, double* p);
int make_mixture2(vbmc_ctx* ctx, const char* who, int err, int D, int K2, const double* mu2_KxD, const double* sigma2_K,
                  const double* lambd2_D, const double* w2_K, MixLayout& ml2, std::vector<double>& pack2);
int theta_to_arrays(int D, int K, const double* theta, int n_theta, int optimize_mask, double* mu,
                    double* sg, double* lm, double* w, double* eta);
void ctx_pack_aux(const vbmc_ctx* ctx, double* dst);
void ctx_unpack_aux(vbmc_ctx* ctx, const double* src);
int resolve_row_slice(vbmc_ctx* ctx, const vbmc_elbo_opts* opts, const char* who, int64_t* row_begin, int64_t* row_count);
int upload_packed_mixture(vbmc_ctx* ctx);
double* write_pack_to_device(vbmc_ctx* ctx);
int set_mixture_host(vbmc_ctx* ctx, int D, int K, const double* mu_KxD, const double* sigma_K,
                     const double* lambd_D, const double* w_K, const double* eta_K, bool skip_if_same);

int ensure_dev(vbmc_ctx* ctx, double** p, size_t* cap, size_t n_doubles);
int ensure_pinned(vbmc_ctx* ctx, size_t n_doubles);
int reserve_in(vbmc_ctx* ctx, double** p, size_t* cap, Scratch& sc);
int reserve(vbmc_ctx* ctx, Scratch& sc);
int download_chunked(vbmc_ctx* ctx, const double* d_src, double* dst, size_t n);
int fetch_vectors(vbmc_ctx* ctx, int k, const double* const* d_src, double* const* dst, size_t count, size_t stride, size_t o);
int randn_with_progress(uint32_t* key, int* pos, int* has_gauss, double* gauss, double* out, int64_t n, int n_threads,
                        void (*progress)(void*, int64_t), void* user);

static inline int raw_len(int D, int K) { return 1 + D * K + 2 * K + D; }

struct DoneSignal {
  int* cnt = nullptr;
  int* sub = nullptr;
  int sub_min = 256;
  uint64_t* flag = nullptr;
  uint64_t seq = 0;
  double* host_out = nullptr;
  int host_n = 0;
  const uint64_t* cancel = nullptr;
  const uint64_t* ident_src = nullptr;
  uint64_t* ident_dst = nullptr;
  uint64_t ident_seed = 0;
  int dev = 0;
};

__host__ __device__ inline uint64_t pack_ck_term(double v, uint32_t i) {
  uint64_t b;
  __builtin_memcpy(&b, &v, 8);
  return b * (0x9E3779B97F4A7C15ull + 2ull * i);
}
inline uint64_t pack_checksum(const double* p, size_t n) {
  uint64_t s0 = 0, s1 = 0, s2 = 0, s3 = 0;
  size_t i = 0;
  for (; i + 4 <= n; i += 4) {
    s0 += pack_ck_term(p[i], (uint32_t)i);
    s1 += pack_ck_term(p[i + 1], (uint32_t)i + 1);
    s2 += pack_ck_term(p[i + 2], (uint32_t)i + 2);
    s3 += pack_ck_term(p[i + 3], (uint32_t)i + 3);
  }
  for (; i < n; ++i) s0 += pack_ck_term(p[i], (uint32_t)i);
  return (s0 + s1) + (s2 + s3);
}

#ifdef __HIPCC__
__device__ __forceinline__ void staged_copy_to_host(const double* __restrict__ src, double* __restrict__ dst, int n) {
  for (int base = 0; base < n; base += 256 * 8) {
    double v[8];
#pragma unroll
    for (int u = 0; u < 8; ++u) {
      const int i = min(base + u * 256 + (int)threadIdx.x, n - 1);
      v[u] = __hip_atomic_load(src + i, __ATOMIC_RELAXED, __HIP_MEMORY_SCOPE_AGENT);
    }
#pragma unroll
    for (int u = 0; u < 8; ++u) {
      const int i = min(base + u * 256 + (int)threadIdx.x, n - 1);
      __hip_atomic_store(dst + i, v[u], __ATOMIC_RELAXED, __HIP_MEMORY_SCOPE_SYSTEM);
    }
  }
  __builtin_amdgcn_s_waitcnt(0x0F70);
}
#endif

struct GenSlice {
  double* eps = nullptr;
  int K = 0, D = 0;
  int nb = 0;
  uint32_t nb_magic = 0, rows_magic = 0;
  int64_t rows = 0;
  int64_t n_half = 0, row_begin = 0;
  uint64_t seed = 0;
  const int* seed_add = nullptr;
  int64_t item_begin = 0, item_count = 0;
  int n_blocks = 0;
};

struct PrepArgs {
  const double* mix = nullptr;
  MixLayout ml;
  double* mix_copy = nullptr;
  int mix_copy_n = 0;
  uint64_t* ident_out = nullptr;
  uint64_t* go = nullptr;
  uint64_t go_seq = 0;
  uint64_t go_timeout = 200000;
  uint64_t* dead = nullptr;
  int n_table = 0, DP = 0, K4 = 0;
  double* table = nullptr;
  int n_glj = 0, N = 0, P = 0, want_grad = 0;
  int batch = 1;
  size_t mix_stride = 0, res_stride = 0;
  const double* X = nullptr;
  const double* XT = nullptr;
  int x_lds = 0;
  const double* alpha = nullptr;
  const double* hyp = nullptr;
  double* res = nullptr;
  double* Z = nullptr;
  GenSlice gen;
  DoneSignal done;
};
GenSlice make_gen_slice(double* eps, int K, int D, int64_t rows, int64_t n_half, int64_t row_begin,
                        uint64_t seed, const int* seed_add, double frac_begin, double frac_end);
inline hipError_t stream_wait(vbmc_ctx* ctx) {
  if (ctx->spec.armed) spec_disarm(ctx);
  ++ctx->stream_waits;
  const hipError_t e = hipStreamSynchronize(ctx->stream);
  if (e == hipSuccess) ctx->pack_in_flight = false;
  return e;
}
inline int timing_begin(vbmc_ctx* ctx, TimingPair p) {
  if (ctx->timing) HIP_TRY(ctx, hipEventRecord(ctx->ev[2 * p], ctx->stream));
  return 0;
}
inline int timing_end(vbmc_ctx* ctx, TimingPair p) {
  if (ctx->timing) {
    HIP_TRY(ctx, hipEventRecord(ctx->ev[2 * p + 1], ctx->stream));
    ctx->ev_valid[p] = true;
  }
  return 0;
}
int launch_prep(vbmc_ctx* ctx, const PrepArgs& a);
int launch_prep_on(vbmc_ctx* ctx, hipStream_t stream, const PrepArgs& a);

struct EntPlan;
int entmc_plan(vbmc_ctx* ctx, int64_t ns_per_comp, int eps_mode, uint64_t seed, int64_t row_begin,
               int64_t row_count, int want_grad, EntPlan& p, int gp_items = 0, int gp_per_slot = 0);
bool entmc_take_gp(const vbmc_ctx* ctx, EntPlan& p, const PrepArgs& gp);
void entmc_fill_prep(const vbmc_ctx* ctx, const EntPlan& p, PrepArgs& a);
int entmc_pregen(vbmc_ctx* ctx, EntPlan& p, PrepArgs& a);

int entmc_launch_main(vbmc_ctx* ctx, const EntPlan& p);
int entmc_launch_finish(vbmc_ctx* ctx, const EntPlan& p, double* raw_out, const GenSlice* gen = nullptr,
                        const DoneSignal* done = nullptr);
int entmc_launch_publish(vbmc_ctx* ctx, const double* d_raw, const DoneSignal& done, const GenSlice* gen);
GenSlice entmc_ahead_slice(vbmc_ctx* ctx, const EntPlan& p);
void glj_fill_prep(const vbmc_ctx* ctx, int want_grad, double* res, double* Z, PrepArgs& a);

int launch_entmc(vbmc_ctx* ctx, int64_t ns_per_comp, int eps_mode, uint64_t seed,
                 int64_t row_begin, int64_t row_count, int want_grad, double* d_raw);
int launch_entlb(vbmc_ctx* ctx, double* d_res);
int launch_eps_gen(vbmc_ctx* ctx, hipStream_t st, const GenSlice& g);
int launch_mixture_pdf(vbmc_ctx* ctx, int64_t n, const double* d_x, int log_flag,
                       int grad_flag, double df, double* d_y, double* d_dy);
int launch_mixture_pdf_on(vbmc_ctx* ctx, const double* d_pack, const MixLayout& ml, int64_t n,
                          const double* d_x, int log_flag, double* d_y);
struct Selector {
  int64_t n_exact = 0;
  std::vector<int64_t> cum;
  std::vector<double> cdf;
};
void make_selector(const double* w, int K, int64_t N, int balance, Selector& s);
inline size_t selector_cdf_elems(int K) { return (size_t)K; }
inline size_t selector_elems(int K) { return (size_t)K + 1 + selector_cdf_elems(K); }
inline int64_t* selector_cum(double* d_sel) { return (int64_t*)d_sel; }
inline double* selector_cdf(double* d_sel, int K) { return d_sel + K + 1; }
int launch_sample(vbmc_ctx* ctx, const double* d_pack, const MixLayout& ml, const double* w_host, int64_t N,
                  uint64_t seed, int balance, double* d_sel, double* d_x, int32_t* d_comp, double df = INFINITY);
int launch_kl_terms(vbmc_ctx* ctx, const double* d_y_own, const double* d_y_other, int64_t n, int nblk, double* d_part);
int launch_gp_log_joint(vbmc_ctx* ctx, int want_grad, double* d_res, double* d_Z);
int launch_gp_var(vbmc_ctx* ctx, const double* d_Z, double* d_V, double* d_Q);
int launch_trinv(vbmc_ctx* ctx, const double* d_Dinv = nullptr);
int launch_pad_linv(vbmc_ctx* ctx);
int launch_gp_post_build(vbmc_ctx* ctx, double* d_Dinv, int* d_flag);
struct GpAppendWs {
  Scratch sc;
  Piece<int> flag;
  Piece<> kvec, lvec, uvec, dd, rnew, tvec;
};
GpAppendWs gp_post_append_ws(int S, int N);
int launch_gp_post_append(vbmc_ctx* ctx, const GpState& from, double y_new, const double* d_sn2_new, size_t sn2_stride,
                          const GpAppendWs& ws);
void gp_post_free(vbmc_ctx* ctx);
void gp_post_host_fields(GpState& w, int N, int D, int S, int P, int mean_kind, std::vector<double>& sW_host);
int launch_gp_fit_design(vbmc_ctx* ctx, const GpFitArgs& f);
int launch_gp_fit_stage(vbmc_ctx* ctx, const GpFitArgs& f, int b0, int S);
int launch_gp_fit_rank(vbmc_ctx* ctx, const GpFitArgs& f);
int launch_gp_fit_select(vbmc_ctx* ctx, const GpFitArgs& f);
int launch_gp_fit_handover(vbmc_ctx* ctx, const GpFitArgs& f);
int launch_gp_lml(vbmc_ctx* ctx, int want_grad, const double* d_dsn2, double* d_sums, double* d_part, double* d_mg,
                  double* d_lml, double* d_dlml);
int gp_stage_data(vbmc_ctx* ctx, GpState& w, int N, int D, int P, int mean_kind, const double* X, const double* y);
int gp_cand_begin(vbmc_ctx* ctx, int N, int D, int P, int chunk);
int gp_lml_chunk(vbmc_ctx* ctx, const Scratch& sc, const GpLmlWs& ws, int S, int slot0);
int gp_cand_stage(vbmc_ctx* ctx, const char* who, const Scratch& sc, const GpLmlWs& ws, double* d_in,
                  const std::vector<double>& in, size_t own_off, int mean_kind, const double* X, const double* y, GpCandArgs& a);
template <class Advance>
int gp_cand_round(vbmc_ctx* ctx, const Scratch& sc, const GpLmlWs& ws, int runs, int chunk, Advance advance) {
  int rc = 0;
  for (int b0 = 0; b0 < runs && !rc; b0 += chunk) {
    const int S = runs - b0 < chunk ? runs - b0 : chunk;
    if (!(rc = advance(b0, S))) rc = gp_lml_chunk(ctx, sc, ws, S, b0);
  }
  return rc;
}
struct LockstepWord {
  size_t state_elems = 0, offset_bytes = 0;
  int done_value = 0;
};
int launch_lockstep_count(vbmc_ctx* ctx, const double* d_state, int n_runs, size_t state_elems, size_t word_offset_bytes,
                          int done_value, int* d_count);
template <class RoundFn>
int lockstep_rounds(vbmc_ctx* ctx, const char* what, int per_batch, long long max_rounds, int n_runs, const double* d_state,
                    const LockstepWord& word, int* d_count, RoundFn round_fn, long long* rounds, int* left) {
  int rc = 0;
  *rounds = 0;
  *left = n_runs;
  while (*left > 0 && *rounds < max_rounds) {
    for (int q = 0; q < per_batch && *rounds < max_rounds; ++q, ++*rounds)
      if ((rc = round_fn(*rounds))) return rc;
    if ((rc = launch_lockstep_count(ctx, d_state, n_runs, word.state_elems, word.offset_bytes, word.done_value, d_count)))
      return rc;
    hipError_t e = hipMemcpyAsync(ctx->h_pinned, d_count, sizeof(int), hipMemcpyDeviceToHost, ctx->stream);
    if (e == hipSuccess) e = stream_wait(ctx);
    if (e != hipSuccess) return vbmc_fail(ctx, VBMC_E_HIP, "%s: %s", what, hipGetErrorString(e));
    *left = *(const int*)ctx->h_pinned;
  }
  return 0;
}
struct FetchPiece {
  size_t off;
  void* dst;
  size_t bytes;
};
int fetch_tail(vbmc_ctx* ctx, const Scratch& sc, size_t from, std::initializer_list<FetchPiece> pieces);
struct GpHypArgs : GpCandArgs {
  int C = 0, n = 0, thin = 0, burn_in = 0;
  uint64_t seed = 0;
  const double* widths = nullptr;
  double *x = nullptr, *xp = nullptr;
  double *hyp_out = nullptr, *logpost = nullptr, *logprior = nullptr;
};
size_t gp_hyp_state_elems();
LockstepWord gp_hyp_done_word();
int launch_gp_hyp_advance(vbmc_ctx* ctx, const GpHypArgs& a, int b0, int S);
struct GpOptArgs : GpCandArgs {
  int R = 0, max_iter = 0, m = 0, trace_cap = 0;
  double tol_g = 0.0, tol_f = 0.0;
  const double* dlml = nullptr;
  double* dsn2 = nullptr;
  double *hyp_out = nullptr, *logpost = nullptr, *grad = nullptr;
  double *trace_it = nullptr, *trace_ev = nullptr;
};
size_t gp_opt_state_elems(int P, int m);
LockstepWord gp_opt_done_word(int P, int m);
int launch_gp_opt_advance(vbmc_ctx* ctx, const GpOptArgs& a, int b0, int S);
int gp_state_grow(vbmc_ctx* ctx, GpState& g, int N, int D, int S, int P, bool with_post);
inline int predict_ld(int N) { return (N + 63) / 64 * 64; }
inline size_t predict_ks_elems(int S, int64_t mb, int N) {
  return (size_t)S * (size_t)((mb + 63) / 64 * 64) * (size_t)predict_ld(N);
}
struct PredictPlan {
  int64_t mb = 0;
  int ntiles = 0;
  Scratch sc;
  Piece<> p_xs, p_Ks, p_part, p_fmu, p_fs2;
  double *xs = nullptr, *Ks = nullptr, *part = nullptr, *fmu = nullptr, *fs2 = nullptr;
};
inline void predict_plan(const vbmc_ctx* ctx, int64_t M, int64_t budget, int64_t cost, int64_t cap, PredictPlan& p) {
  const int S = ctx->gp.S, N = ctx->gp.N, D = ctx->gp.D;
  p.ntiles = (N + 63) / 64;
  int64_t mb = budget / cost;
  mb = mb > cap ? cap : (mb < 64 ? 64 : (mb / 64) * 64);
  p.mb = mb = M < mb ? M : mb;
  p.p_xs = p.sc.add((size_t)mb * D);
  p.p_Ks = p.sc.add(predict_ks_elems(S, mb, N), 32);
  p.p_part = p.sc.add(2 * (size_t)S * p.ntiles * mb);
  p.p_fmu = p.sc.add((size_t)S * mb);
  p.p_fs2 = p.sc.add((size_t)S * mb);
}
inline int predict_reserve(vbmc_ctx* ctx, PredictPlan& p, size_t pinned_per_point) {
  int rc = reserve(ctx, p.sc);
  if (rc) return rc;
  rc = ensure_pinned(ctx, pinned_per_point * (size_t)p.mb);
  if (rc) return rc;
  p.xs = p.sc.ptr(p.p_xs);
  p.Ks = p.sc.ptr(p.p_Ks);
  p.part = p.sc.ptr(p.p_part);
  p.fmu = p.sc.ptr(p.p_fmu);
  p.fs2 = p.sc.ptr(p.p_fs2);
  return 0;
}
int launch_gp_predict_products(vbmc_ctx* ctx, int64_t M, const double* d_xs, double* d_Ks, double* d_part,
                               const void* fin = nullptr, bool* fin_done = nullptr);
int launch_gp_panel_product(vbmc_ctx* ctx, const double* d_A, const double* d_B, double* d_C, int64_t M, int KD, int NC,
                            bool upper_b = false);
int launch_gp_predict_all(vbmc_ctx* ctx, int64_t M, const double* d_xs, double* d_Ks, double* d_part,
                          int add_noise, double* d_fmu, double* d_fs2, int64_t ld);
int launch_acq_closed(vbmc_ctx* ctx, const PredictPlan& p, int64_t m, const double* d_xs, const double* d_sn2, int kind,
                      double y_max, double tol_gp_var, double* d_dens, double* d_res);
int acq_is_need(vbmc_ctx* ctx, const char* who, int64_t* Na);
int launch_acq_is(vbmc_ctx* ctx, const PredictPlan& p, int64_t m, const double* d_xs, const double* d_sn2, double u,
                  double* d_Kx, double* d_T, double* d_as, double* d_res);
struct XfView;
struct SearchSrcDev {
  int kind, pad;
  long long begin, count;
  unsigned long long seed;
  long long par;
};
int launch_search_fill(vbmc_ctx* ctx, double* d_X, int64_t M, int D, const SearchSrcDev* d_src, int n_src, const double* d_par,
                       const double* d_lb, const double* d_ub, uint32_t int_bits, const XfView* t);
int launch_search_mask(vbmc_ctx* ctx, const double* d_X, int64_t M, int D, const XfView* t, const double* d_lb,
                       const double* d_ub, double* d_acq);
constexpr int search_sum_blocks = 64;
int launch_search_scale(vbmc_ctx* ctx, const double* d_X, int64_t M, int D, const double* d_ell, double* d_xsc);
int launch_search_colsum(vbmc_ctx* ctx, const double* d_x, int64_t n, int D, double* d_part);
int launch_search_centre(vbmc_ctx* ctx, const double* d_part_a, int64_t n, const double* d_part_b, int64_t m, int D,
                         double* d_cen);
int launch_search_take(vbmc_ctx* ctx, const double* d_table, int64_t n_table, const int64_t* d_pos, int64_t M, double* d_out);
int launch_search_is_finish(vbmc_ctx* ctx, int64_t M, double tol_gp_var, const double* d_var_tot, double* d_acq);
int64_t search_sort_len(int64_t M);
int launch_search_sort(vbmc_ctx* ctx, const double* d_acq, int64_t M, uint64_t* d_keys, uint32_t* d_idx);
int launch_search_gather(vbmc_ctx* ctx, const double* d_X, const uint32_t* d_idx, int64_t M, int D, int64_t* d_order,
                         double* d_Xs);
struct SearchScore {
  int kind = 0, use_xf = 0;
  bool is_kind = false, noisy = false;
  int64_t Na = 0, n_noise = 0, M = 0;
  XfView t;
  const double *X_rescaled = nullptr, *sn2_new = nullptr, *length_scale = nullptr, *lb_eps = nullptr, *ub_eps = nullptr;
  std::vector<double> bnd;
  PredictPlan p;
  Piece<> p_dens, p_Kx, p_T, p_as, p_res, p_sn2, p_bnd, p_ell, p_xsc, p_b, p_tab, p_cen, p_part, p_pmin;
  Piece<int64_t> p_am;
};
int search_score_check(vbmc_ctx* ctx, const char* who, int kind, int64_t n_noise, const double* X_rescaled_NxD,
                       const double* sn2_new_N, const double* length_scale_D, int use_xf, const double* lb_eps_orig_D,
                       const double* ub_eps_orig_D, SearchScore& s);
int search_score_list(vbmc_ctx* ctx, const char* who, int64_t M, SearchScore& s);
int search_score_upload(vbmc_ctx* ctx, SearchScore& s);
int search_score_rows(vbmc_ctx* ctx, const SearchScore& s, const double* d_X, int64_t m, double y_max, double tol_gp_var,
                      double u, double* d_acq);
int search_set_rows_cap();
int search_fail_wait(vbmc_ctx* ctx, int rc);
struct BatchScore {
  int B = 0, n_theta = 0, n_bnd = 0, n_aux = 0, mask = 0;
  size_t stride = 0;
  MixLayout ml;
  Piece<> p_aux, p_packs, p_res, p_H, p_out, p_base, p_bnd;
  Piece<int> p_flags;
  int flags0[2] = {0, 0};
};
int batch_score_check(vbmc_ctx* ctx, const char* who, int B, int n_theta, const vbmc_elbo_opts* opts);
void batch_score_list(const vbmc_ctx* ctx, int B, int n_theta, const vbmc_elbo_opts* opts, Scratch& sc, BatchScore& s);
size_t batch_score_pinned(const BatchScore& s);
int batch_score_queue(vbmc_ctx* ctx, const char* who, const Scratch& sc, BatchScore& s, const vbmc_elbo_opts* opts, double* d_th,
                      double* hp);
struct SieveFillDev {
  int D = 0, K = 0, Kn = 0, mask = 0, n_theta = 0, Ns = 0, n_slot = 0;
  long long n1 = 0, n2 = 0, n3 = 0;
  unsigned long long seed = 0;
  const double* base = nullptr;
  const double* t2 = nullptr;
  const double* lam_s = nullptr;
  const double* Xs = nullptr;
  double v3 = 0.0;
  const double* Z = nullptr;
  const int* I = nullptr;
  double* thetas = nullptr;
};
size_t sieve_fill_lds_bytes(int D, int Kn, int n_keys);
int launch_sieve_fill(vbmc_ctx* ctx, const SieveFillDev& a);
int launch_sieve_nan_rows(vbmc_ctx* ctx, const double* d_thetas, int64_t B, int n_theta, double* d_F, double* d_G, double* d_H);
int launch_elcbo_isk(vbmc_ctx* ctx, const double* d_res, double* d_I);
int launch_elcbo_reweight(vbmc_ctx* ctx, int S, int K0, int Ka, const double* d_I, const double* d_J, const double* d_w,
                          const int* d_alive, double* d_part, double* d_out);
struct CmaesArgs {
  int R = 0, D = 0, lam = 0, mu = 0, hist = 0;
  long long max_fevals = 0;
  uint64_t seed = 0;
  double tol_fun = 0.0, tol_x = 0.0;
  double one_cs = 0, a_ps = 0, q_cs = 0, hs_thresh = 0, one_cc = 0, a_pc = 0, c_old = 0, c1 = 0, cmu = 0, cc2 = 0, cs_ds = 0, inv_chi = 0;
  const double* w = nullptr;
  const double *x0 = nullptr, *sigma0 = nullptr, *lb = nullptr, *ub = nullptr;
  uint32_t int_bits = 0;
  int has_xf = 0;
  XfView t;
  const double* val = nullptr;
  double* rows = nullptr;
  double* state = nullptr;
  double *x_best = nullptr, *f_best = nullptr, *f0 = nullptr, *mean = nullptr, *sigma = nullptr, *C = nullptr;
  long long* stats = nullptr;
};
int launch_cmaes_advance(vbmc_ctx* ctx, const CmaesArgs& a);
LockstepWord cmaes_done_word(const CmaState& ly);
size_t is_mcmc_lds_bytes(int N, int threads);
int launch_is_mcmc(vbmc_ctx* ctx, int ln_y_fmu, double u_q, const double* d_x0, const double* d_widths, const double* d_lb,
                   const double* d_ub, int n, int thin, int burn_in, uint64_t seed, double* d_X, double* d_logp,
                   double* d_fmu, double* d_fs2, long long* d_stats, int* d_invalid);
int launch_sq_dist(vbmc_ctx* ctx, const double* d_a, int64_t n, const double* d_b, int m, int D,
                   const double* d_cen, double* d_c, double* d_pmin, int64_t* d_argmin);

void glj_finalize(const vbmc_ctx* ctx, const double* res, int want_grad, GljHost& o);
int glj_pack(vbmc_ctx* ctx, const double* mu, const double* sg, const double* lm,
             const double* wg, int grad_flags, int jacobian_flag, double* out);
bool ctx_is_multi(const vbmc_ctx* ctx);
int comm_allreduce_sum(vbmc_ctx* ctx, double* d_buf, int n);

void softmax_jacobian_apply(vbmc_ctx* ctx, const double* g, double* out);
int entropy_pack(vbmc_ctx* ctx, double H, const double* mu, const double* sg,
                 const double* lm, const double* wg, int grad_flags, int jacobian_flag,
                 double* H_out, double* dH_out);
```

### pyvbmc_amd/csrc/ctx.hip

```cpp
#include <algorithm>
#include <cmath>
#include <cstdarg>
#include <cstdlib>
#include <cstring>

#include <sched.h>

#include <cctype>
#include <cstdio>

#include "common.h"

thread_local std::string g_create_err;

int vbmc_fail(vbmc_ctx* ctx, int code, const char* fmt, ...) {
  char buf[1024];
  va_list ap;
  va_start(ap, fmt);
  vsnprintf(buf, sizeof buf, fmt, ap);
  va_end(ap);
  if (ctx)
    ctx->err = buf;
  else
    g_create_err = buf;
  return code;
}

int ensure_dev(vbmc_ctx* ctx, double** p, size_t* cap, size_t n) {
  if (*cap >= n && *p) return 0;
  if (*p) {
    HIP_TRY(ctx, stream_wait(ctx));
    HIP_TRY(ctx, hipFree(*p));
    *p = nullptr;
    *cap = 0;
  }
  size_t want = n + n / 4 + 64;
  HIP_TRY(ctx, hipMalloc((void**)p, want * sizeof(double)));
  *cap = want;
  return 0;
}

int ensure_pinned(vbmc_ctx* ctx, size_t n) {
  if (ctx->h_pinned_cap >= n && ctx->h_pinned) return 0;
  if (ctx->h_pinned) {
    HIP_TRY(ctx, stream_wait(ctx));
    HIP_TRY(ctx, hipHostFree(ctx->h_pinned));
    ctx->h_pinned = nullptr;
    ctx->h_pinned_cap = 0;
  }
  size_t want = n + n / 4 + 64;
  HIP_TRY(ctx, hipHostMalloc((void**)&ctx->h_pinned, want * sizeof(double), hipHostMallocDefault));
  ctx->h_pinned_cap = want;
  HIP_TRY(ctx, hipHostGetDevicePointer((void**)&ctx->hp_dev, ctx->h_pinned, 0));
  return 0;
}

int reserve_in(vbmc_ctx* ctx, double** p, size_t* cap, Scratch& sc) {
  const int rc = ensure_dev(ctx, p, cap, sc.total);
  if (rc) return rc;
  sc.base = *p;
  return 0;
}
int reserve(vbmc_ctx* ctx, Scratch& sc) { return reserve_in(ctx, &ctx->d_scratch, &ctx->d_scratch_cap, sc); }

int download_chunked(vbmc_ctx* ctx, const double* d_src, double* dst, size_t n) {
  const size_t chunk = (size_t)1 << 20;
  int rc = ensure_pinned(ctx, n < chunk ? n : chunk);
  if (rc) return rc;
  for (size_t o = 0; o < n; o += chunk) {
    const size_t m = (n - o) < chunk ? (n - o) : chunk;
    HIP_TRY(ctx, hipMemcpyAsync(ctx->h_pinned, d_src + o, sizeof(double) * m, hipMemcpyDeviceToHost, ctx->stream));
    HIP_TRY(ctx, stream_wait(ctx));
    memcpy(dst + o, ctx->h_pinned, sizeof(double) * m);
  }
  return 0;
}

int fetch_vectors(vbmc_ctx* ctx, int k, const double* const* d_src, double* const* dst, size_t count, size_t stride, size_t o) {
  for (int i = 0; i < k; ++i)
    if (!dst || dst[i])
      HIP_TRY(ctx, hipMemcpyAsync(ctx->h_pinned + i * stride, d_src[i], sizeof(double) * count, hipMemcpyDeviceToHost, ctx->stream));
  HIP_TRY(ctx, stream_wait(ctx));
  for (int i = 0; dst && i < k; ++i)
    if (dst[i]) memcpy(dst[i] + o, ctx->h_pinned + i * stride, sizeof(double) * count);
  return 0;
}

#include <atomic>
static std::atomic<int> g_live_ctx[64];
int vbmc_live_contexts_on(int device) { return device >= 0 && device < 64 ? g_live_ctx[device].load() : 2; }

static void options_from_env(vbmc_ctx* c) {
  const char* e = getenv("VBMC_ENTMC_KERNEL");
  c->opt_entmc_valu = (e && e[0] == 'v') ? 1 : 0;
  e = getenv("VBMC_ELBO_PREGEN");
  c->opt_elbo_pregen = !(e && e[0] == '0');
  e = getenv("VBMC_ELBO_AHEAD");
  c->opt_elbo_ahead = !(e && e[0] == '0');
  e = getenv("VBMC_ELBO_ARM");
  c->opt_elbo_arm = e ? atoi(e) : 1;
  e = getenv("VBMC_ACQ_POLL");
  c->opt_acq_poll = !(e && e[0] == '0');
  e = getenv("VBMC_ADAM_FUSED");
  c->opt_adam_fused = e ? atoi(e) : 1;
  e = getenv("VBMC_RANDN_DEVICE");
  c->opt_randn_dev = e ? (e[0] == '0' ? 0 : e[0] == '2' ? 2 : 1) : 1;
  e = getenv("VBMC_ADAM_TAIL");
  c->opt_adam_tail = e ? atoi(e) : 1;
  e = getenv("VBMC_WS_SPAN");
  c->opt_ws_span = !(e && e[0] == '0');
  e = getenv("VBMC_WS_FRONT");
  if (e) c->opt_ws_front = atoi(e);
  e = getenv("VBMC_WS_PAD");
  if (e) c->opt_ws_pad = atoi(e);
  e = getenv("VBMC_WS_ROLES");
  c->opt_ws_roles = !(e && e[0] == '0');
  e = getenv("VBMC_MIX_BAR");
  c->opt_mix_bar = !(e && e[0] == '0');
  e = getenv("VBMC_PREDICT_DMA");
  c->opt_predict_dma = !(e && e[0] == '0');
  e = getenv("VBMC_PREDICT_FUSED_FINISH");
  if (e) c->opt_predict_fused = atoi(e);
  e = getenv("VBMC_GP_SHIP");
  c->opt_gp_ship = !(e && e[0] == '0');
}

extern "C" {

int vbmc_abi_version(void) { return 2; }

int vbmc_device_count(int* n_out) {
  int n = 0;
  hipError_t e = hipGetDeviceCount(&n);
  if (e != hipSuccess) {
    n = 0;
    (void)hipGetLastError();
  }
  if (n_out) *n_out = n;
  return VBMC_OK;
}

}

static void bind_host_thread(vbmc_ctx* ctx) {
  const char* e = getenv("VBMC_HOST_AFFINITY");
  if (e && e[0] == '0') return;
  char bus[64] = {0};
  if (hipDeviceGetPCIBusId(bus, (int)sizeof(bus) - 1, ctx->device) != hipSuccess) {
    (void)hipGetLastError();
    return;
  }
  for (char* c = bus; *c; ++c) *c = (char)tolower((unsigned char)*c);
  char path[160];
  snprintf(path, sizeof(path), "/sys/bus/pci/devices/%s/local_cpulist", bus);
  FILE* f = fopen(path, "r");
  if (!f) return;
  char list[1024] = {0};
  const bool got = fgets(list, sizeof(list), f) != nullptr;
  fclose(f);
  if (!got) return;
  cpu_set_t local, cur, both;
  CPU_ZERO(&local);
  for (char* p = list; *p;) {
    char* end = nullptr;
    const long a = strtol(p, &end, 10);
    if (end == p) break;
    long b = a;
    p = end;
    if (*p == '-') {
      b = strtol(p + 1, &end, 10);
      if (end == p + 1) break;
      p = end;
    }
    for (long c = a; c <= b && c < CPU_SETSIZE; ++c)
      if (c >= 0) CPU_SET((int)c, &local);
    while (*p == ',' || *p == ' ' || *p == '\n') ++p;
  }
  if (CPU_COUNT(&local) == 0 || sched_getaffinity(0, sizeof(cur), &cur) != 0) return;
  CPU_AND(&both, &cur, &local);
  const int n_both = CPU_COUNT(&both), n_cur = CPU_COUNT(&cur);
  ctx->host_cpus = n_cur;
  if (n_both == 0 || n_both == n_cur) return;
  if (sched_setaffinity(0, sizeof(both), &both) == 0) {
    ctx->host_bound = true;
    ctx->host_cpus = n_both;
  }
}

extern "C" {

int vbmc_host_affinity(const vbmc_ctx* ctx, int* bound_out, int* n_cpus_out) {
  if (!ctx) return VBMC_E_ARG;
  if (bound_out) *bound_out = ctx->host_bound ? 1 : 0;
  if (n_cpus_out) *n_cpus_out = ctx->host_cpus;
  return VBMC_OK;
}

int vbmc_ctx_create(int device_id, vbmc_ctx** out) {
  if (!out) return vbmc_fail(nullptr, VBMC_E_ARG, "vbmc_ctx_create: out is NULL");
  *out = nullptr;
  if (device_id == -1) {
    vbmc_ctx* h = new vbmc_ctx();
    h->device = -1;
    options_from_env(h);
    *out = h;
    return VBMC_OK;
  }
  int n = 0;
  hipError_t e = hipGetDeviceCount(&n);
  if (e != hipSuccess || n <= 0) {
    (void)hipGetLastError();
    return vbmc_fail(nullptr, VBMC_E_NODEV,
                     "no HIP device visible (%s); libvbmc_hip has no CPU fallback",
                     e == hipSuccess ? "device count 0" : hipGetErrorString(e));
  }
  if (device_id < 0 || device_id >= n)
    return vbmc_fail(nullptr, VBMC_E_ARG, "device_id %d out of range [0,%d)", device_id, n);
  vbmc_ctx* ctx = new vbmc_ctx();
  ctx->device = device_id;
  options_from_env(ctx);
  e = hipSetDevice(device_id);
  if (e == hipSuccess) e = hipGetDeviceProperties(&ctx->prop, device_id);
  if (e == hipSuccess) bind_host_thread(ctx);
  if (e == hipSuccess) e = hipStreamCreateWithFlags(&ctx->stream, hipStreamNonBlocking);
  for (int i = 0; i < 2 * T_COUNT && e == hipSuccess; ++i) e = hipEventCreate(&ctx->ev[i]);
  if (e == hipSuccess) e = hipHostMalloc((void**)&ctx->h_done, 64, hipHostMallocDefault);
  if (e == hipSuccess) {
    for (int i = 0; i < 8; ++i) ctx->h_done[i] = 0;
    e = hipHostGetDevicePointer((void**)&ctx->hd_done, ctx->h_done, 0);
  }
  if (e == hipSuccess) e = hipMalloc((void**)&ctx->d_done_cnt, 64);
  if (e == hipSuccess) e = hipMemset(ctx->d_done_cnt, 0, 64);
  if (e == hipSuccess) e = hipMalloc((void**)&ctx->d_done_sub, 16 * 64 * sizeof(int));
  if (e == hipSuccess) e = hipMemset(ctx->d_done_sub, 0, 16 * 64 * sizeof(int));
  if (e != hipSuccess) {
    int rc = vbmc_fail(nullptr, VBMC_E_HIP, "context setup failed: %s", hipGetErrorString(e));
    delete ctx;
    return rc;
  }
  if (strncmp(ctx->prop.gcnArchName, "gfx950", 6) != 0) {
    int rc = vbmc_fail(nullptr, VBMC_E_NODEV, "device %d is %s; this library is built for gfx950 only",
                       device_id, ctx->prop.gcnArchName);
    vbmc_ctx_destroy(ctx);
    return rc;
  }
  if (device_id < 64) g_live_ctx[device_id].fetch_add(1);
  ctx->counted = true;
  *out = ctx;
  return VBMC_OK;
}

void vbmc_ctx_destroy(vbmc_ctx* ctx) {
  if (!ctx) return;
  if (ctx->device < 0) {
    delete ctx;
    return;
  }
  if (ctx->counted && ctx->device < 64) g_live_ctx[ctx->device].fetch_sub(1);
  (void)hipSetDevice(ctx->device);
  spec_disarm(ctx);
  if (getenv("VBMC_DEBUG_ARM")) fprintf(stderr, "[vbmc] armed evaluations: %llu used, %llu cancelled\n", (unsigned long long)ctx->spec.hits, (unsigned long long)ctx->spec.cancels);
  if (ctx->stream) (void)hipStreamSynchronize(ctx->stream);
  if (ctx->d_ctl) (void)hipFree(ctx->d_ctl);
  vbmc_comm_destroy(ctx);
  adam_free(ctx);
  acq_is_free(ctx);
  randn_dev_free(ctx);
  xf_free(ctx);
  search_free(ctx);
  sieve_free(ctx);
  elcbo_free(ctx);
  gp_post_free(ctx);
  double* bufs[] = {ctx->d_mix, ctx->d_mix_fg, ctx->d_acq_fg, ctx->d_stage, ctx->d_eps, ctx->d_scratch, ctx->d_out, ctx->d_ptick, ctx->gp.d_X, ctx->gp.d_XT,
                    ctx->gp.d_alpha, ctx->gp.d_L, ctx->gp.d_Linv, ctx->gp.d_LinvP, ctx->gp.d_sW, ctx->gp.d_hyp,
                    ctx->gp.d_xc, ctx->gp.d_smeta};
  for (double* b : bufs)
    if (b) (void)hipFree(b);
  for (double* b : ctx->d_epsgen)
    if (b) (void)hipFree(b);
  if (ctx->h_done) (void)hipHostFree(ctx->h_done);
  if (ctx->d_done_cnt) (void)hipFree(ctx->d_done_cnt);
  if (ctx->d_done_sub) (void)hipFree(ctx->d_done_sub);
  if (ctx->h_pinned) (void)hipHostFree(ctx->h_pinned);
  if (ctx->h_eps) (void)hipHostFree(ctx->h_eps);
  if (ctx->h_pack) (void)hipHostFree(ctx->h_pack);

  for (hipEvent_t e : ctx->ev)
    if (e) (void)hipEventDestroy(e);
  if (ctx->stream) (void)hipStreamDestroy(ctx->stream);
  delete ctx;
}

const char* vbmc_last_error(const vbmc_ctx* ctx) {
  return ctx ? ctx->err.c_str() : g_create_err.c_str();
}

int vbmc_device_info(const vbmc_ctx* ctx, char* name, int name_len, int* cu_count,
                     int* clock_khz, uint64_t* hbm_bytes) {
  if (!ctx) return VBMC_E_ARG;
  if (ctx->device < 0) return vbmc_fail(const_cast<vbmc_ctx*>(ctx), VBMC_E_NODEV, "host-only context");
  if (name && name_len > 0) {
    snprintf(name, (size_t)name_len, "%s (%s)", ctx->prop.name, ctx->prop.gcnArchName);
  }
  if (cu_count) *cu_count = ctx->prop.multiProcessorCount;
  if (clock_khz) *clock_khz = ctx->prop.clockRate;
  if (hbm_bytes) *hbm_bytes = (uint64_t)ctx->prop.totalGlobalMem;
  return VBMC_OK;
}

int vbmc_synchronize(vbmc_ctx* ctx) {
  if (!ctx) return VBMC_E_ARG;
  if (ctx->device < 0) return VBMC_OK;
  HIP_TRY(ctx, hipSetDevice(ctx->device));
  HIP_TRY(ctx, stream_wait(ctx));
  return VBMC_OK;
}

int vbmc_set_option(vbmc_ctx* ctx, const char* key, int value) {
  if (!ctx || !key) return VBMC_E_ARG;
  if (!strcmp(key, "arm_late_test")) {
    ctx->opt_arm_late_test = value;
    return VBMC_OK;
  }
  if (!strcmp(key, "ident_test")) {
    ctx->opt_ident_test = value;
    return VBMC_OK;
  }
  spec_disarm(ctx);
  if (!strcmp(key, "entmc_kernel")) ctx->opt_entmc_valu = value == 1;
  else if (!strcmp(key, "entmc_mfma")) ctx->opt_entmc_mfma = value != 0;
  else if (!strcmp(key, "gp_ship")) ctx->opt_gp_ship = value != 0;
  else if (!strcmp(key, "elbo_pregen")) ctx->opt_elbo_pregen = value != 0;
  else if (!strcmp(key, "elbo_ahead")) ctx->opt_elbo_ahead = value != 0;
  else if (!strcmp(key, "predict_dma")) ctx->opt_predict_dma = value != 0;
  else if (!strcmp(key, "predict_fused")) ctx->opt_predict_fused = value < 0 ? 0 : value > 2 ? 2 : value;
  else if (!strcmp(key, "mix_bar")) ctx->opt_mix_bar = value != 0;
  else if (!strcmp(key, "ws_span")) ctx->opt_ws_span = value != 0;
  else if (!strcmp(key, "ws_roles")) ctx->opt_ws_roles = value != 0;
  else if (!strcmp(key, "ws_pad")) ctx->opt_ws_pad = value > 8 ? 8 : value;
  else if (!strcmp(key, "ws_front")) ctx->opt_ws_front = value < 0 ? 0 : value > 990 ? 990 : value;
  else if (!strcmp(key, "elbo_arm")) ctx->opt_elbo_arm = value < 0 ? 0 : value > 2 ? 2 : value;
  else if (!strcmp(key, "acq_poll")) ctx->opt_acq_poll = value != 0;
  else if (!strcmp(key, "is_mcmc_threads")) ctx->opt_is_mcmc_threads = value <= 256 ? 256 : value >= 768 ? 768 : 512;
  else if (!strcmp(key, "gp_lml_chunk")) ctx->opt_gp_lml_chunk = value < 0 ? 0 : value;
  else if (!strcmp(key, "gp_hyp_rounds")) ctx->opt_gp_hyp_rounds = value < 1 ? 4 : value > 4096 ? 4096 : value;
  else if (!strcmp(key, "gp_opt_rounds")) ctx->opt_gp_opt_rounds = value < 1 ? 4 : value > 4096 ? 4096 : value;
  else if (!strcmp(key, "cmaes_rounds")) ctx->opt_cmaes_rounds = value < 1 ? 8 : value > 4096 ? 4096 : value;
  else if (!strcmp(key, "randn_device")) ctx->opt_randn_dev = value < 0 ? 0 : value > 3 ? 3 : value;
  else if (!strcmp(key, "adam_tail")) ctx->opt_adam_tail = value;
  else if (!strcmp(key, "adam_fused")) ctx->opt_adam_fused = value;
  else return vbmc_fail(ctx, VBMC_E_ARG, "vbmc_set_option: unknown key '%s'", key);
  return VBMC_OK;
}

int vbmc_set_gp_watch(vbmc_ctx* ctx, const double* const* ptrs, const int64_t* lens, int n, uint64_t expected) {
  if (!ctx || n < 0 || (n > 0 && (!ptrs || !lens))) return VBMC_E_ARG;
  ctx->gp_watch_ptrs.assign(ptrs, ptrs + n);
  ctx->gp_watch_lens.assign(lens, lens + n);
  ctx->gp_watch_ck = expected;
  return VBMC_OK;
}

int vbmc_host_checksum(const double* const* ptrs, const int64_t* lens, int n, uint64_t* out) {
  if (!ptrs || !lens || n < 0 || !out) return VBMC_E_ARG;
  uint64_t s = 0;
  for (int a = 0; a < n; ++a) {
    if (!ptrs[a] || lens[a] < 0) return VBMC_E_ARG;
    s += (pack_checksum(ptrs[a], (size_t)lens[a]) + (uint64_t)lens[a]) * (0xD1B54A32D192ED03ull + 2ull * (uint64_t)a);
  }
  *out = s;
  return VBMC_OK;
}

int vbmc_last_entmc_plan(const vbmc_ctx* ctx, int out[4]) {
  if (!ctx || !out) return VBMC_E_ARG;
  for (int i = 0; i < 4; ++i) out[i] = ctx->last_plan[i];
  return VBMC_OK;
}

int vbmc_set_timing(vbmc_ctx* ctx, int on) {
  if (!ctx) return VBMC_E_ARG;
  ctx->timing = on < 0 ? 0 : on > 2 ? 2 : on;
  return VBMC_OK;
}

int vbmc_last_kernel_ms(vbmc_ctx* ctx, int which, double* ms_out) {
  if (!ctx || which < 0 || which >= T_COUNT || !ms_out) return VBMC_E_ARG;
  NEED_DEVICE(ctx);
  if (!ctx->ev_valid[which])
    return vbmc_fail(ctx, VBMC_E_ARG, which == T_PREDICT_VAR ? "no timed launch recorded for 5 (gp_predict's product alone is timed at vbmc_set_timing(ctx, 2) only)"
                                                 : "no timed launch recorded for %d", which);
  HIP_TRY(ctx, hipEventSynchronize(ctx->ev[2 * which + 1]));
  float ms = 0.f;
  HIP_TRY(ctx, hipEventElapsedTime(&ms, ctx->ev[2 * which], ctx->ev[2 * which + 1]));
  *ms_out = (double)ms;
  return VBMC_OK;
}

}

void write_mixture_pack(const MixLayout& ml, const double* mu_KxD, const double* sigma,
                        const double* lambd, const double* w, double* p) {
  const int D = ml.D, K = ml.K;
  double prod_lam = 1.0;
  for (int d = 0; d < D; ++d) prod_lam *= lambd[d];
  const double nconst = 1.0 / std::pow(2.0 * M_PI, 0.5 * D) / prod_lam;
  const double l2n = std::log2(nconst);
  for (int k = 0; k < K; ++k) {
    for (int d = 0; d < D; ++d) {
      p[ml.o_mu + k * D + d] = mu_KxD[(size_t)k * D + d];
      p[ml.o_mup + k * D + d] = mu_KxD[(size_t)k * D + d] / lambd[d];
    }
    const double s = sigma[k];
    double sD = 1.0, b = s;
    for (int e = D; e > 0; e >>= 1) {
      if (e & 1) sD *= b;
      b *= b;
    }
    p[ml.o_is2 + k] = 1.0 / (s * s);
    p[ml.o_rc + k] = nconst / sD;
    p[ml.o_lrc + k] = l2n - D * std::log2(s);
    p[ml.o_wc + k] = w[k] * nconst / sD;
    p[ml.o_sig + k] = s;
    p[ml.o_w + k] = w[k];
  }
  for (int d = 0; d < D; ++d) {
    p[ml.o_lam + d] = lambd[d];
    p[ml.o_ilam + d] = 1.0 / lambd[d];
  }
}

int make_mixture2(vbmc_ctx* ctx, const char* who, int err, int D, int K2, const double* mu2_KxD, const double* sigma2_K,
                  const double* lambd2_D, const double* w2_K, MixLayout& ml2, std::vector<double>& pack2) {
  for (int k = 0; k < K2; ++k)
    if (!(sigma2_K[k] > 0.0) || !std::isfinite(sigma2_K[k]))
      return vbmc_fail(ctx, err, "%s: sigma2[%d] must be finite and > 0", who, k);
  ml2.plan(D, K2);
  pack2.resize((size_t)ml2.total);
  write_mixture_pack(ml2, mu2_KxD, sigma2_K, lambd2_D, w2_K, pack2.data());
  return 0;
}

int theta_to_arrays(int D, int K, const double* theta, int n_theta, int optimize_mask, double* mu,
                    double* sg, double* lm, double* w, double* eta) {
  const ThetaMap tm(D, K, optimize_mask);
  if (n_theta != tm.n_theta()) return -1;
  for (int i = 0; i < n_theta; ++i)
    if (!std::isfinite(theta[i])) return -2;
  if (tm.o_mu())
    for (int i = 0; i < D * K; ++i) mu[i] = theta[i];
  if (tm.o_sg())
    for (int k = 0; k < K; ++k) sg[k] = std::exp(theta[tm.p_sg + k]);
  if (tm.o_lm())
    for (int d = 0; d < D; ++d) lm[d] = std::exp(theta[tm.p_lm + d]);
  if (tm.o_w()) {
    const double* e = theta + tm.p_w;
    double mx = e[0];
    for (int k = 1; k < K; ++k) mx = e[k] > mx ? e[k] : mx;
    for (int k = 0; k < K; ++k) {
      eta[k] = e[k] - mx;
      w[k] = std::exp(eta[k]);
    }
  }
  double s2 = 0.0;
  for (int d = 0; d < D; ++d) s2 += lm[d] * lm[d];
  const double nl = std::sqrt(s2 / D);
  for (int d = 0; d < D; ++d) lm[d] /= nl;
  for (int k = 0; k < K; ++k) sg[k] *= nl;
  if (tm.o_w()) {
    double ws = 0.0;
    for (int k = 0; k < K; ++k) ws += w[k];
    for (int k = 0; k < K; ++k) w[k] /= ws;
  }
  return 0;
}

void ctx_pack_aux(const vbmc_ctx* ctx, double* dst) {
  for (const std::vector<double>* v : {&ctx->mu, &ctx->sigma, &ctx->lambd, &ctx->w, &ctx->eta}) dst = std::copy(v->begin(), v->end(), dst);
}

void ctx_unpack_aux(vbmc_ctx* ctx, const double* src) {
  for (std::vector<double>* v : {&ctx->mu, &ctx->sigma, &ctx->lambd, &ctx->w, &ctx->eta}) {
    std::copy(src, src + v->size(), v->begin());
    src += v->size();
  }
}

int resolve_row_slice(vbmc_ctx* ctx, const vbmc_elbo_opts* opts, const char* who, int64_t* row_begin, int64_t* row_count) {
  const int64_t n_half = opts->ns_per_comp / 2;
  *row_begin = opts->row_begin;
  *row_count = opts->row_count;
  if (*row_count < 0) {
    *row_begin = n_half * ctx->rank / ctx->world;
    *row_count = n_half * (ctx->rank + 1) / ctx->world - *row_begin;
  }
  if (*row_begin < 0 || *row_begin + *row_count > n_half) return vbmc_fail(ctx, VBMC_E_ARG, "%s: bad row slice", who);
  if (opts->eps_mode == VBMC_EPS_RESIDENT &&
      (!ctx->d_eps || ctx->eps_K != ctx->K || ctx->eps_D != ctx->D || ctx->eps_n_half != n_half ||
       ctx->eps_row_begin != *row_begin || ctx->eps_rows != *row_count))
    return vbmc_fail(ctx, VBMC_E_ARG, "%s: resident eps does not match the request", who);
  return 0;
}

static int pack_mixture(vbmc_ctx* ctx) {
  const int D = ctx->D, K = ctx->K;
  ctx->ml.plan(D, K);
  const MixLayout& ml = ctx->ml;
  if (ctx->device < 0) return 0;
  if (ctx->h_pack_cap < (size_t)ml.total) {
    if (ctx->h_pack) {
      HIP_TRY(ctx, stream_wait(ctx));
      HIP_TRY(ctx, hipHostFree(ctx->h_pack));
      ctx->h_pack = nullptr;
    }
    const size_t want = (size_t)ml.total * 2 + 64;
    HIP_TRY(ctx, hipHostMalloc((void**)&ctx->h_pack, want * sizeof(double), hipHostMallocDefault));
    ctx->h_pack_cap = want;
  }
  if (ctx->pack_in_flight) {
    HIP_TRY(ctx, stream_wait(ctx));
    ctx->pack_in_flight = false;
  }
  write_mixture_pack(ml, ctx->mu.data(), ctx->sigma.data(), ctx->lambd.data(), ctx->w.data(), ctx->h_pack);
  return ensure_dev(ctx, &ctx->d_mix, &ctx->d_mix_cap, (size_t)ml.total);
}

namespace {
__global__ void mix_upload_kernel(const double* __restrict__ src, double* __restrict__ dst, int n) {
  const int i = blockIdx.x * blockDim.x + threadIdx.x;
  if (i < n) dst[i] = src[i];
}
}

double* write_pack_to_device(vbmc_ctx* ctx) {
  if (ctx->device < 0 || ctx->mix_fg_failed) return nullptr;
  const size_t n = (size_t)ctx->ml.total;
  if (ctx->d_mix_fg_cap < n) {
    if (ctx->d_mix_fg) {
      (void)hipStreamSynchronize(ctx->stream);
      (void)hipFree(ctx->d_mix_fg);
      ctx->d_mix_fg = nullptr;
    }
    const size_t want = n * 2 + 64;
    int large_bar = 0;
    if (hipDeviceGetAttribute(&large_bar, hipDeviceAttributeIsLargeBar, ctx->device) != hipSuccess || !large_bar) {
      (void)hipGetLastError();
      ctx->mix_fg_failed = true;
      return nullptr;
    }
    if (hipExtMallocWithFlags((void**)&ctx->d_mix_fg, want * sizeof(double), hipDeviceMallocFinegrained) != hipSuccess) {
      (void)hipGetLastError();
      ctx->d_mix_fg = nullptr;
      ctx->d_mix_fg_cap = 0;
      ctx->mix_fg_failed = true;
      return nullptr;
    }
    ctx->d_mix_fg_cap = want;
  }
  if (!ctx->d_ctl) {
    if (hipExtMallocWithFlags((void**)&ctx->d_ctl, 64, hipDeviceMallocFinegrained) != hipSuccess) {
      (void)hipGetLastError();
      ctx->d_ctl = nullptr;
    } else {
      memset(ctx->d_ctl, 0, 64);
      __builtin_ia32_sfence();
    }
  }
  memcpy(ctx->d_mix_fg, ctx->h_pack, n * sizeof(double));
  __builtin_ia32_sfence();
  ctx->pack_valid = true;
  return ctx->d_mix_fg;
}

int upload_packed_mixture(vbmc_ctx* ctx) {
  if (ctx->device < 0) return 0;
  if (ctx->spec.armed) spec_disarm(ctx);
  {
    double* src = nullptr;
    if (ctx->h_pack_dev_of != ctx->h_pack) {
      HIP_TRY(ctx, hipHostGetDevicePointer((void**)&ctx->h_pack_dev, ctx->h_pack, 0));
      ctx->h_pack_dev_of = ctx->h_pack;
    }
    src = ctx->h_pack_dev;
    const int n = ctx->ml.total;
    hipLaunchKernelGGL(mix_upload_kernel, dim3((n + 255) / 256), dim3(256), 0, ctx->stream, (const double*)src,
                       ctx->d_mix, n);
    HIP_TRY(ctx, hipGetLastError());
  }
  ctx->pack_in_flight = true;
  ctx->pack_valid = true;
  return 0;
}

int set_mixture_host(vbmc_ctx* ctx, int D, int K, const double* mu_KxD, const double* sigma_K,
                     const double* lambd_D, const double* w_K, const double* eta_K, bool skip_if_same) {
  if (D < 1 || K < 1) return vbmc_fail(ctx, VBMC_E_ARG, "set_mixture: bad D=%d K=%d", D, K);
  if (skip_if_same && ctx->mix_set && ctx->pack_valid && ctx->D == D && ctx->K == K &&
      memcmp(ctx->mu.data(), mu_KxD, sizeof(double) * K * D) == 0 &&
      memcmp(ctx->sigma.data(), sigma_K, sizeof(double) * K) == 0 &&
      memcmp(ctx->lambd.data(), lambd_D, sizeof(double) * D) == 0 &&
      memcmp(ctx->w.data(), w_K, sizeof(double) * K) == 0) {
    if (eta_K) ctx->eta.assign(eta_K, eta_K + K);
    ctx->exp_eta_valid = false;
    return 0;
  }
  ctx->pack_valid = false;
  ctx->D = D;
  ctx->K = K;
  ctx->mu.assign(mu_KxD, mu_KxD + (size_t)K * D);
  ctx->sigma.assign(sigma_K, sigma_K + K);
  ctx->lambd.assign(lambd_D, lambd_D + D);
  ctx->w.assign(w_K, w_K + K);
  if (eta_K)
    ctx->eta.assign(eta_K, eta_K + K);
  else
    ctx->eta.assign((size_t)K, 0.0);
  ctx->exp_eta_valid = false;
  for (int k = 0; k < K; ++k)
    if (!(ctx->sigma[k] > 0.0) || !std::isfinite(ctx->sigma[k]))
      return vbmc_fail(ctx, VBMC_E_NONFINITE, "set_mixture: sigma[%d]=%g must be finite and > 0", k,
                       ctx->sigma[k]);
  for (int d = 0; d < D; ++d)
    if (!(ctx->lambd[d] > 0.0) || !std::isfinite(ctx->lambd[d]))
      return vbmc_fail(ctx, VBMC_E_NONFINITE, "set_mixture: lambd[%d]=%g must be finite and > 0", d,
                       ctx->lambd[d]);
  ctx->mix_set = true;
  int rc = pack_mixture(ctx);
  if (rc || ctx->defer_mix_upload) return rc;
  return upload_packed_mixture(ctx);
}

extern "C" {

int vbmc_set_mixture(vbmc_ctx* ctx, int D, int K, const double* mu_KxD, const double* sigma_K,
                     const double* lambd_D, const double* w_K, const double* eta_K) {
  if (!ctx || !mu_KxD || !sigma_K || !lambd_D || !w_K) return VBMC_E_ARG;
  if (ctx->device >= 0) HIP_TRY(ctx, hipSetDevice(ctx->device));
  return set_mixture_host(ctx, D, K, mu_KxD, sigma_K, lambd_D, w_K, eta_K, true);
}

int vbmc_set_mixture_dk(vbmc_ctx* ctx, int D, int K, const double* mu_DxK, const double* sigma_K,
                        const double* lambd_D, const double* w_K, const double* eta_K) {
  if (!ctx || !mu_DxK || !sigma_K || !lambd_D || !w_K || D < 1 || K < 1) return VBMC_E_ARG;
  if (ctx->device >= 0) HIP_TRY(ctx, hipSetDevice(ctx->device));
  std::vector<double>& t = ctx->mu_scratch;
  t.resize((size_t)D * K);
  for (int d = 0; d < D; ++d)
    for (int k = 0; k < K; ++k) t[(size_t)k * D + d] = mu_DxK[(size_t)d * K + k];
  return set_mixture_host(ctx, D, K, t.data(), sigma_K, lambd_D, w_K, eta_K, true);
}

int vbmc_theta_to_mixture(vbmc_ctx* ctx, const double* theta, int n_theta, int optimize_mask,
                          double* mu_KxD, double* sigma_K, double* lambd_D, double* w_K,
                          double* eta_K) {
  if (!ctx || !theta) return VBMC_E_ARG;
  if (!ctx->mix_set) return vbmc_fail(ctx, VBMC_E_ARG, "theta_to_mixture: mixture (D,K) not set");
  if (ctx->device >= 0) HIP_TRY(ctx, hipSetDevice(ctx->device));
  const int D = ctx->D, K = ctx->K;
  std::vector<double>&mu = ctx->t2m_mu, &sg = ctx->t2m_sg, &lm = ctx->t2m_lm, &w = ctx->t2m_w, &eta = ctx->t2m_eta;
  mu = ctx->mu;
  sg = ctx->sigma;
  lm = ctx->lambd;
  w = ctx->w;
  eta = ctx->eta;
  const int st = theta_to_arrays(D, K, theta, n_theta, optimize_mask, mu.data(), sg.data(), lm.data(),
                                 w.data(), eta.data());
  if (st == -1)
    return vbmc_fail(ctx, VBMC_E_ARG, "theta length %d does not match D=%d K=%d mask=%d", n_theta, D, K,
                     optimize_mask);
  if (st == -2) return vbmc_fail(ctx, VBMC_E_NONFINITE, "theta has a non-finite entry");
  int rc = set_mixture_host(ctx, D, K, mu.data(), sg.data(), lm.data(), w.data(), eta.data(), false);
  if (rc) return rc;
  if (mu_KxD) memcpy(mu_KxD, mu.data(), sizeof(double) * D * K);
  if (sigma_K) memcpy(sigma_K, sg.data(), sizeof(double) * K);
  if (lambd_D) memcpy(lambd_D, lm.data(), sizeof(double) * D);
  if (w_K) memcpy(w_K, w.data(), sizeof(double) * K);
  if (eta_K) memcpy(eta_K, eta.data(), sizeof(double) * K);
  return VBMC_OK;
}

static int upload_eps(vbmc_ctx* ctx, int K, int64_t n_half, int D, const double* eps_half, int64_t row_begin,
                      int64_t row_count) {
  HIP_TRY(ctx, hipSetDevice(ctx->device));
  size_t n = (size_t)K * (size_t)row_count * (size_t)D;
  int rc = ensure_dev(ctx, &ctx->d_eps, &ctx->d_eps_cap, n ? n : 1);
  if (rc) return rc;
  if (row_begin == 0 && row_count == n_half && n > 0) {
    HIP_TRY(ctx, hipMemcpyAsync(ctx->d_eps, eps_half, sizeof(double) * n, hipMemcpyHostToDevice, ctx->stream));
  } else {
    for (int j = 0; j < K && row_count > 0; ++j) {
      const double* src = eps_half + ((size_t)j * (size_t)n_half + (size_t)row_begin) * D;
      double* dst = ctx->d_eps + (size_t)j * (size_t)row_count * D;
      HIP_TRY(ctx, hipMemcpyAsync(dst, src, sizeof(double) * (size_t)row_count * D,
                                  hipMemcpyHostToDevice, ctx->stream));
    }
  }
  HIP_TRY(ctx, stream_wait(ctx));
  ctx->eps_K = K;
  ctx->eps_D = D;
  ctx->eps_rows = row_count;
  ctx->eps_row_begin = row_begin;
  ctx->eps_n_half = n_half;
  return VBMC_OK;
}

int vbmc_set_eps(vbmc_ctx* ctx, int K, int64_t n_half, int D, const double* eps_half,
                 int64_t row_begin, int64_t row_count) {
  if (!ctx || !eps_half || K < 1 || D < 1 || n_half < 0) return VBMC_E_ARG;
  if (row_begin < 0 || row_count < 0 || row_begin + row_count > n_half)
    return vbmc_fail(ctx, VBMC_E_ARG, "set_eps: rows [%lld,+%lld) outside [0,%lld)",
                     (long long)row_begin, (long long)row_count, (long long)n_half);
  NEED_DEVICE(ctx);
  return upload_eps(ctx, K, n_half, D, eps_half, row_begin, row_count);
}

int vbmc_set_eps_numpy(vbmc_ctx* ctx, uint32_t* key, int* pos, int* has_gauss, double* gauss, int K,
                       int64_t n_half, int D, int64_t row_begin, int64_t row_count, int n_threads) {
  if (!ctx || !key || !pos || !has_gauss || !gauss || K < 1 || D < 1 || n_half < 0) return VBMC_E_ARG;
  if (row_begin < 0 || row_count < 0 || row_begin + row_count > n_half)
    return vbmc_fail(ctx, VBMC_E_ARG, "set_eps_numpy: rows [%lld,+%lld) outside [0,%lld)",
                     (long long)row_begin, (long long)row_count, (long long)n_half);
  NEED_DEVICE(ctx);
  HIP_TRY(ctx, hipSetDevice(ctx->device));
  const size_t n_all = (size_t)K * (size_t)n_half * (size_t)D;
  {
    const bool whole = row_begin == 0 && row_count == n_half && n_all > 0;
    if (whole) {
      const int erc = ensure_dev(ctx, &ctx->d_eps, &ctx->d_eps_cap, n_all);
      if (erc) return erc;
    }
  if (whole && ctx->opt_randn_dev && n_all >= ((size_t)1 << 16) && ctx->world == 1) {
      const int drc = randn_device(ctx, key, pos, has_gauss, gauss, ctx->d_eps, (int64_t)n_all);
      if (drc != VBMC_W_NOT_FUSED) {
        if (drc) return drc;
        ctx->eps_K = K;
        ctx->eps_D = D;
        ctx->eps_rows = row_count;
        ctx->eps_row_begin = row_begin;
        ctx->eps_n_half = n_half;
        return VBMC_OK;
      }
    }
  }
  if (ctx->h_eps_cap < n_all || !ctx->h_eps) {
    if (ctx->h_eps) {
      HIP_TRY(ctx, stream_wait(ctx));
      HIP_TRY(ctx, hipHostFree(ctx->h_eps));
      ctx->h_eps = nullptr;
      ctx->h_eps_cap = 0;
    }
    const size_t want = n_all + n_all / 8 + 64;
    HIP_TRY(ctx, hipHostMalloc((void**)&ctx->h_eps, want * sizeof(double), hipHostMallocDefault));
    ctx->h_eps_cap = want;
  }
  struct Up {
    vbmc_ctx* ctx;
    int64_t sent;
    hipError_t err;
  } up{ctx, 0, hipSuccess};
  const bool whole = row_begin == 0 && row_count == n_half && n_all > 0;
  if (whole) {
    const int erc = ensure_dev(ctx, &ctx->d_eps, &ctx->d_eps_cap, n_all);
    if (erc) return erc;
  }
  auto progress = [](void* user, int64_t m) {
    Up* u = (Up*)user;
    if (m <= u->sent || u->err != hipSuccess) return;
    u->err = hipMemcpyAsync(u->ctx->d_eps + u->sent, u->ctx->h_eps + u->sent, sizeof(double) * (size_t)(m - u->sent),
                            hipMemcpyHostToDevice, u->ctx->stream);
    u->sent = m;
  };
  const int rc = randn_with_progress(key, pos, has_gauss, gauss, ctx->h_eps, (int64_t)n_all, n_threads,
                                     whole ? +progress : nullptr, &up);
  if (rc) return vbmc_fail(ctx, rc, rc == VBMC_E_NOMEM ? "set_eps_numpy: out of host memory" : "set_eps_numpy: generator state rejected");
  if (!whole) return upload_eps(ctx, K, n_half, D, ctx->h_eps, row_begin, row_count);
  progress(&up, (int64_t)n_all);
  HIP_TRY(ctx, up.err);
  HIP_TRY(ctx, stream_wait(ctx));
  ctx->eps_K = K;
  ctx->eps_D = D;
  ctx->eps_rows = row_count;
  ctx->eps_row_begin = row_begin;
  ctx->eps_n_half = n_half;
  return VBMC_OK;
}

}
```

### pyvbmc_amd/csrc/prep.hip

```cpp
#include <cstdlib>

#include "common.h"
#include "fastmath.h"
#include "philox.h"
#ifdef PREP_TIMES
__device__ unsigned long long g_glj_phase[8 * 1024];
#define GLJ_T(i) do { if (threadIdx.x == 0 && blockIdx.x < 1024) g_glj_phase[8 * blockIdx.x + (i)] = wall_clock64(); } while (0)
#endif
#include "glj_block.h"
#include "ws_table.h"

namespace {

__device__ __forceinline__ double wave_sum(double v) {
  return fm::wave_sum_dpp(v);
}

#ifdef FIN_TIMES
__device__ unsigned long long g_prep_times[2 + 64];
#endif
#ifdef PREP_TIMES
__device__ unsigned long long g_prep_blocks[2 * 1024];
struct PrepStamp {
  int b;
  __device__ PrepStamp() : b((int)blockIdx.x) {
    if (threadIdx.x == 0 && b < 1024 && blockIdx.y == 0) g_prep_blocks[2 * b] = wall_clock64();
  }
  __device__ ~PrepStamp() {
    __syncthreads();
    if (threadIdx.x == 0 && b < 1024 && blockIdx.y == 0) g_prep_blocks[2 * b + 1] = wall_clock64();
  }
};
#endif
__global__ __launch_bounds__(256) void elbo_prep_kernel(PrepArgs a) {
  extern __shared__ double lds[];
#ifdef PREP_TIMES
  PrepStamp stamp_;
#endif
#ifdef FIN_TIMES
  if (blockIdx.x == 0 && blockIdx.y == 0 && threadIdx.x == 0) g_prep_times[2 + (g_prep_times[0]++ & 63)] = wall_clock64();
#endif
  const int tid = threadIdx.x;
  if (a.gen.n_blocks > 0 && (int)blockIdx.x >= a.n_table + a.n_glj && (int)blockIdx.x < a.n_table + a.n_glj + a.gen.n_blocks) {
    gen_slice_block(a.gen, blockIdx.x - a.n_table - a.n_glj, tid);
    return;
  }
  if (a.go) {
    __shared__ int s_go;
    if (tid == 0) {
      const unsigned long long t0 = wall_clock64();
      int st = 0;
      for (;;) {
        const uint64_t v = __hip_atomic_load(a.go, __ATOMIC_RELAXED, __HIP_MEMORY_SCOPE_SYSTEM);
        if (v == a.go_seq) { st = 1; break; }
        if (v == ~(uint64_t)0) break;
        if (wall_clock64() - t0 > a.go_timeout) {
          if (blockIdx.x == 0 && blockIdx.y == 0) {
            __hip_atomic_store(a.go, ~(uint64_t)0, __ATOMIC_RELAXED, __HIP_MEMORY_SCOPE_SYSTEM);
            __hip_atomic_store(a.dead, a.go_seq, __ATOMIC_RELAXED, __HIP_MEMORY_SCOPE_SYSTEM);
          }
          break;
        }
        __builtin_amdgcn_s_sleep(2);
      }
      s_go = st;
    }
    __syncthreads();
    if (!s_go) return;
  }
  if (a.mix_copy && blockIdx.x == gridDim.x - 1) {
    uint64_t ck = 0;
    constexpr int U = 16;
    const int n = a.mix_copy_n;
    for (int base = 0; base < n; base += U * 256) {
      double v[U];
#pragma unroll
      for (int u = 0; u < U; ++u) {
        if (base + u * 256 >= n) break;
        v[u] = a.mix[min(base + u * 256 + tid, n - 1)];
      }
#pragma unroll
      for (int u = 0; u < U; ++u) {
        if (base + u * 256 >= n) break;
        const int i = base + u * 256 + tid;
        if (i < n) {
          a.mix_copy[i] = v[u];
          ck += pack_ck_term(v[u], (uint32_t)i);
        }
      }
    }
    if (a.ident_out) {
      __shared__ unsigned long long s_ck[16];
      if (tid < 16) s_ck[tid] = 0;
      __syncthreads();
      atomicAdd(&s_ck[tid & 15], (unsigned long long)ck);
      __syncthreads();
      if (tid == 0) {
        unsigned long long t = 0;
#pragma unroll
        for (int i = 0; i < 16; ++i) t += s_ck[i];
        *a.ident_out = t;
      }
    }
    return;
  }
  a.mix += (size_t)blockIdx.y * a.mix_stride;
  a.res += (size_t)blockIdx.y * a.res_stride;

  if ((int)blockIdx.x < a.n_table) {
    ws_table_row_block(a.mix, a.ml, (int)blockIdx.x, a.DP, a.K4, a.table, lds);
    return;
  }


  if (a.x_lds) {
    glj_stage_x(a, lds);
    glj_block<true>(a, blockIdx.x - a.n_table, lds);
  } else {
    glj_block<false>(a, blockIdx.x - a.n_table, lds);
  }
}

}

#ifdef PREP_TIMES
extern "C" int vbmc_debug_prep_blocks(unsigned long long* out) {
  return (int)hipMemcpyFromSymbol(out, HIP_SYMBOL(g_prep_blocks), sizeof(unsigned long long) * 2048);
}
extern "C" int vbmc_debug_glj_phases(unsigned long long* out) {
  return (int)hipMemcpyFromSymbol(out, HIP_SYMBOL(g_glj_phase), sizeof(unsigned long long) * 8192);
}
#endif
#ifdef FIN_TIMES
extern "C" int vbmc_debug_prep_times(unsigned long long* out) {
  return (int)hipMemcpyFromSymbol(out, HIP_SYMBOL(g_prep_times), sizeof(unsigned long long) * 66);
}
#endif
int launch_prep(vbmc_ctx* ctx, const PrepArgs& a) { return launch_prep_on(ctx, ctx->stream, a); }

int launch_prep_on(vbmc_ctx* ctx, hipStream_t stream, const PrepArgs& a_in) {
  PrepArgs a = a_in;
  const int D = a.ml.D;
  const int gblocks = a.n_glj;
  const int grid = a.n_table + gblocks + a.gen.n_blocks + (a.mix_copy ? 1 : 0);
  if (grid <= 0) return 0;
  size_t lds = 0;
  a.x_lds = 0;
  if (gblocks > 0) {
    lds = glj_block_lds(D, a.N);
    if (lds > 150 * 1024) return vbmc_fail(ctx, VBMC_E_UNSUP, "gp_log_joint: N=%d too large", a.N);
    static const bool x_lds_on = [] {
      const char* e = getenv("VBMC_GLJ_X_LDS");
      return !(e && e[0] == '0');
    }();
    if (x_lds_on && a.gen.n_blocks == 0 && a.batch == 1 && glj_block_lds_x(D, a.N) <= 40 * 1024) {
      a.x_lds = 1;
      lds = glj_block_lds_x(D, a.N);
    }
  }
  if (a.n_table > 0) {
    const size_t lt = sizeof(double) * (size_t)a.K4 * a.DP;
    if (lt > 150 * 1024) return vbmc_fail(ctx, VBMC_E_UNSUP, "entropy table: K=%d D=%d too large", a.ml.K, D);
    lds = lt > lds ? lt : lds;
  }
  if (lds > 64 * 1024)
    HIP_TRY(ctx, hipFuncSetAttribute((const void*)elbo_prep_kernel, hipFuncAttributeMaxDynamicSharedMemorySize, (int)lds));
  if (gblocks > 0) ++ctx->gp_launches;
  hipLaunchKernelGGL(elbo_prep_kernel, dim3(grid, a.batch), dim3(256), lds, stream, a);
  HIP_TRY(ctx, hipGetLastError());
  return 0;
}
```

Baseline: 12290 evals/s.

## Ship raw theta to the device and build the mixture pack inside the prep kernel

```diff
diff --git a/include/vbmc_hip.h b/include/vbmc_hip.h
--- a/include/vbmc_hip.h
+++ b/include/vbmc_hip.h
@@ -64,6 +64,8 @@
                         int* rows_per_component);
 
 int vbmc_host_checksum(const double* const* ptrs, const int64_t* lens, int n, uint64_t* out);
+
+int vbmc_theta_wire_fill(double* dst, const double* theta, int n, uint64_t* ck);
 
 int vbmc_set_gp_watch(vbmc_ctx* ctx, const double* const* ptrs, const int64_t* lens, int n, uint64_t expected);
 
diff --git a/pyvbmc_amd/_lib.py b/pyvbmc_amd/_lib.py
--- a/pyvbmc_amd/_lib.py
+++ b/pyvbmc_amd/_lib.py
@@ -168,6 +168,7 @@
     "vbmc_armed_stats": (C.c_int, [_vp, C.POINTER(C.c_uint64)]),
     "vbmc_set_gp_watch": (C.c_int, [_vp, C.POINTER(C.c_void_p), C.POINTER(C.c_int64), C.c_int, C.c_uint64]),
     "vbmc_host_checksum": (C.c_int, [C.POINTER(C.c_void_p), C.POINTER(C.c_int64), C.c_int, C.POINTER(C.c_uint64)]),
+    "vbmc_theta_wire_fill": (C.c_int, [_dp, _dp, C.c_int, C.POINTER(C.c_uint64)]),
     "vbmc_set_timing": (C.c_int, [_vp, C.c_int]),
     "vbmc_last_kernel_ms": (C.c_int, [_vp, C.c_int, _dp]),
     "vbmc_last_host_us": (C.c_int, [_vp, _dp]),
@@ -428,7 +429,8 @@
         out = (C.c_int * 4)()
         self.check(self._lib.vbmc_last_entmc_plan(self._h, out))
         return {"kernel": ("valu", "ws", "small", "mfma", "adam_fused", "ws", "ws")[out[0]] if out[0] >= 0 else None, "rg": out[1],
-                "chunks": out[2], "resident_draws": bool(out[3] & 1), "roles": bool(out[3] & 2), "span": out[0] in (5, 6), "adam_tail": out[0] == 6}
+                "chunks": out[2], "resident_draws": bool(out[3] & 1), "roles": bool(out[3] & 2), "span": out[0] in (5, 6), "adam_tail": out[0] == 6,
+                "theta_wire": bool(out[3] & 4)}
 
     def philox_normals(self, K, n_half, D, seed, row_begin=0, row_count=None):
         row_count = n_half - row_begin if row_count is None else row_count
diff --git a/pyvbmc_amd/csrc/api_elbo.hip b/pyvbmc_amd/csrc/api_elbo.hip
--- a/pyvbmc_amd/csrc/api_elbo.hip
+++ b/pyvbmc_amd/csrc/api_elbo.hip
@@ -29,7 +29,7 @@
 }
 
 #ifdef FIN_TIMES
-static int64_t g_host_stamps[64][6];
+static int64_t g_host_stamps[64][8];
 static uint64_t g_host_n = 0;
 static inline int64_t host_ns() {
   return std::chrono::duration_cast<std::chrono::nanoseconds>(std::chrono::steady_clock::now().time_since_epoch()).count();
@@ -98,15 +98,42 @@
   const int D = ctx->D, K = ctx->K;
   const int mask = opts->optimize_mask;
   const ThetaMap tm(D, K, mask, n_theta);
-  ctx->defer_mix_upload = true;
-  int rc = vbmc_theta_to_mixture(ctx, theta, n_theta, mask, mu_KxD, sigma_K, lambd_D, w_K, eta_K);
-  ctx->defer_mix_upload = false;
-  if (rc) return rc;
-  if (tm.o_w()) {
-    double* e = theta + (n_theta - K);
-    double mx = e[0];
-    for (int k = 1; k < K; ++k) mx = e[k] > mx ? e[k] : mx;
-    for (int k = 0; k < K; ++k) e[k] -= mx;
+  HIP_TRY(ctx, hipSetDevice(ctx->device));
+  if (n_theta != ThetaMap(D, K, mask).n_theta())
+    return vbmc_fail(ctx, VBMC_E_ARG, "theta length %d does not match D=%d K=%d mask=%d", n_theta, D, K, mask);
+  const bool multi = ctx_is_multi(ctx);
+  const bool wire_wanted = opts->ns_per_comp > 0 && ctx->opt_mix_bar && ctx->opt_theta_wire && !multi && !ctx->timing;
+  bool xf_done = false;
+  auto host_transform = [&]() -> int {
+    if (xf_done) return 0;
+    xf_done = true;
+    ctx->defer_mix_upload = true;
+    const int r = theta_to_mixture_host(ctx, theta, n_theta, mask, mu_KxD, sigma_K, lambd_D, w_K, eta_K);
+    ctx->defer_mix_upload = false;
+    if (r) return r;
+    if (tm.o_w()) {
+      double* e = theta + (n_theta - K);
+      double mx = e[0];
+      for (int k = 1; k < K; ++k) mx = e[k] > mx ? e[k] : mx;
+      for (int k = 0; k < K; ++k) e[k] -= mx;
+    }
+    return 0;
+  };
+  bool wire_filled = false;
+  uint64_t wire_ck = 0;
+  auto fill_wire = [&]() -> int {
+    if (wire_filled) return 0;
+    double* fg = mix_fg_buffer(ctx);
+    if (!fg) return 1;
+    if (tpk::wire_fill(fg, theta, n_theta, &wire_ck)) return vbmc_fail(ctx, VBMC_E_NONFINITE, "theta has a non-finite entry");
+    if (mask != 15) write_aux_to_device(ctx);
+    wire_filled = true;
+    return 0;
+  };
+  int rc = 0;
+  if (!wire_wanted) {
+    rc = host_transform();
+    if (rc) return rc;
   }
   const int grad_flags = opts->compute_grad ? mask : 0;
   const GpState& g = ctx->gp;
@@ -130,7 +157,6 @@
   double* hp_dev = ctx->hp_dev;
   double* res_out = hp_dev;
   double* raw_host = hp_dev + n_res;
-  const bool multi = ctx_is_multi(ctx);
   double* raw_out = raw_host;
   if (multi && mc) {
     rc = ensure_dev(ctx, &ctx->d_out, &ctx->d_out_cap, (size_t)n_raw);
@@ -159,6 +185,7 @@
   bool polled = false;
   uint64_t cur_seq = 0;
   bool ident_out_flag = false;
+  bool issued_wire = false;
   auto issue = [&](uint64_t seed, bool spin, bool& polled_out, uint64_t& seq_out) -> int {
     int rc2;
     PrepArgs pa;
@@ -187,9 +214,10 @@
     }
     seq_out = ctx->done_seq;
     ident_out_flag = false;
+    issued_wire = false;
     ctx->gp_where = 0;
     double* fg = nullptr;
-    if (can_poll && ctx->opt_mix_bar) fg = spin ? ctx->d_mix_fg : write_pack_to_device(ctx);
+    if (can_poll && ctx->opt_mix_bar) fg = spin ? ctx->d_mix_fg : mix_fg_buffer(ctx);
     if (spin && !fg) return -1000;
     const bool ident = fg != nullptr && mc;
     if (ident) pa.ident_out = (uint64_t*)(ctx->d_done_cnt + 12);
@@ -210,10 +238,28 @@
         plan.a.ship_seq = pa.done.seq;
         pa.done = DoneSignal();
       }
-      pa.mix = fg;
+      const bool wire = wire_wanted && mc && pa.n_glj == 0 && prep_wire_fits(ctx->ml, n_theta, pa.K4, pa.DP) && (spin || wire_filled);
+      if (wire) {
+        pa.theta = fg;
+        pa.aux = fg + mix_fg_aux_off(ctx);
+        pa.n_theta = n_theta;
+        pa.mask = mask;
+        pa.pow_2pi = pack_pow_2pi(D);
+        pa.mix = nullptr;
+        issued_wire = true;
+      } else {
+        if (!spin) {
+          rc2 = host_transform();
+          if (rc2) return rc2;
+          if (!write_pack_to_device(ctx)) return vbmc_fail(ctx, VBMC_E_HIP, "neg_elcbo: host-written device memory lost");
+        }
+        pa.mix = fg;
+      }
       pa.mix_copy = ctx->d_mix;
       pa.mix_copy_n = ctx->ml.total;
     } else {
+      rc2 = host_transform();
+      if (rc2) return rc2;
       rc2 = upload_packed_mixture(ctx);
       if (rc2) return rc2;
     }
@@ -286,6 +332,7 @@
   uint64_t want_ck = 0;
   bool check_ident = false;
   bool used_armed = false;
+  bool eval_wire = false;
   if (sp.armed) {
     const bool match = can_poll && sp.seed == opts->seed && sp.n_theta == n_theta && sp.mask == mask &&
                        sp.grad_flags == grad_flags && sp.eps_mode == opts->eps_mode &&
@@ -293,11 +340,19 @@
                        !ctx->timing &&
                        std::chrono::duration<double, std::milli>(clk::now() - sp.t_armed).count() < sp.limit_ms;
     if (match) {
-      memcpy(ctx->d_mix_fg, ctx->h_pack, sizeof(double) * (size_t)ctx->ml.total);
+      if (sp.wire) {
+        rc = fill_wire();
+        if (rc) return rc < 0 ? rc : vbmc_fail(ctx, VBMC_E_HIP, "neg_elcbo: host-written device memory lost");
+      } else {
+        rc = host_transform();
+        if (rc) return rc;
+        memcpy(ctx->d_mix_fg, ctx->h_pack, sizeof(double) * (size_t)ctx->ml.total);
+        ctx->pack_valid = true;
+      }
       __builtin_ia32_sfence();
       *(volatile uint64_t*)ctl_word(ctx, sp.seq) = sp.seq;
       __builtin_ia32_sfence();
-      ctx->pack_valid = true;
+      eval_wire = sp.wire;
       sp.armed = false;
       const bool force_late = ctx->opt_arm_late_test > 0 && --ctx->opt_arm_late_test == 0;
       if (!force_late && std::chrono::duration<double, std::milli>(clk::now() - sp.t_armed).count() < sp.limit_ms + ARM_LATE_SLACK_MS) {
@@ -326,11 +381,38 @@
     }
   }
   if (!used_armed) {
+    if (wire_wanted) {
+      rc = fill_wire();
+      if (rc < 0) return rc;
+    }
+    const uint64_t seq_before = ctx->done_seq;
+    const int gen_cur_before = ctx->gen_cur;
+    const vbmc_ctx::AheadDraws ahead_before = ctx->ahead;
+    const bool xf_was_done = xf_done;
     rc = issue(opts->seed, false, polled, cur_seq);
-    if (rc) return rc;
+    if (rc) {
+      if (!xf_was_done && xf_done) {
+        ctx->done_seq = seq_before;
+        ctx->gen_cur = gen_cur_before;
+        ctx->ahead = ahead_before;
+      }
+      return rc;
+    }
     check_ident = polled && ident_out_flag;
-  }
-  if (mc && can_poll && ctx->opt_mix_bar) want_ck = pack_checksum(ctx->h_pack, (size_t)ctx->ml.total);
+    eval_wire = issued_wire;
+  }
+  if (!xf_done) {
+    rc = host_transform();
+    if (rc) {
+      const std::string msg = ctx->err;
+      HIP_TRY(ctx, stream_wait(ctx));
+      ctx->err = msg;
+      return rc;
+    }
+  }
+  if (eval_wire) ctx->pack_valid = true;
+  HSTAMP(6);
+  if (mc && can_poll && ctx->opt_mix_bar) want_ck = eval_wire ? wire_ck : pack_checksum(ctx->h_pack, (size_t)ctx->ml.total);
   ctx->step_marks[2] = (double)ctx->gp_where;
   if (polled && arm_next && ctx->d_ctl && ctx->d_mix_fg) {
     sp.gen_cur_before = ctx->gen_cur;
@@ -346,6 +428,7 @@
     if (rc2 == 0 && p2) {
       sp.armed = true;
       sp.ident = ident_out_flag;
+      sp.wire = issued_wire;
       sp.limit_ms = arm_limit_ms;
       sp.t_armed = t_arm0;
       sp.seq = seq2;
@@ -368,6 +451,7 @@
       return rc2;
     }
   }
+  if (mc) ctx->last_plan[3] = (ctx->last_plan[3] & ~4) | (eval_wire ? 4 : 0);
   if (ctx->release_cb && !ctx->ident_retry) ctx->release_cb(ctx->release_cb_user);
   ElboScratch& sc = ctx->elbo;
   const bool has_bnd = opts->bnd_lb && opts->bnd_ub;
diff --git a/pyvbmc_amd/csrc/common.h b/pyvbmc_amd/csrc/common.h
--- a/pyvbmc_amd/csrc/common.h
+++ b/pyvbmc_amd/csrc/common.h
@@ -11,6 +11,7 @@
 #include "gp_cand_host.h"
 #include "gp_fit_host.h"
 #include "scratch.h"
+#include "theta_pack.h"
 #include "transform.h"
 
 struct ncclComm;
@@ -162,6 +163,7 @@
     double ahead_before_frac = 1.0;
     uint64_t hits = 0, cancels = 0, late = 0, ident_checked = 0, ident_bad = 0, lost = 0;
     bool ident = false;
+    bool wire = false;
     double limit_ms = 1.0;
     std::chrono::steady_clock::time_point t_armed;
   } spec;
@@ -170,7 +172,6 @@
   size_t d_stage_cap = 0;
   double* d_mix_fg = nullptr;
   std::vector<double> mu_scratch;
-  std::vector<double> t2m_mu, t2m_sg, t2m_lm, t2m_w, t2m_eta;
   double* d_acq_fg = nullptr;
   bool acq_fg_failed = false;
   uint64_t acq_seq = 0;
@@ -214,6 +215,7 @@
   bool pack_in_flight = false;
   bool pack_valid = false;
   bool defer_mix_upload = false;
+  bool aux_on_wire = false;
   double* hp_dev = nullptr;
   int timing = 0;
   double host_us[5] = {0, 0, 0, 0, 0};
@@ -246,6 +248,7 @@
   int opt_ws_pad = -1;
   int opt_ws_roles = 1;
   int opt_mix_bar = 1;
+  int opt_theta_wire = 1;
   double* h_pack_dev = nullptr;
   double* h_pack_dev_of = nullptr;
   std::vector<double> exp_eta;
@@ -330,6 +333,7 @@
 
 void write_mixture_pack(const MixLayout& ml, const double* mu_KxD, const double* sigma,
                         const double* lambd, const double* w, double* p);
+double pack_pow_2pi(int D);
 int make_mixture2(vbmc_ctx* ctx, const char* who, int err, int D, int K2, const double* mu2_KxD, const double* sigma2_K,
                   const double* lambd2_D, const double* w2_K, MixLayout& ml2, std::vector<double>& pack2);
 int theta_to_arrays(int D, int K, const double* theta, int n_theta, int optimize_mask, double* mu,
@@ -339,6 +343,11 @@
 int resolve_row_slice(vbmc_ctx* ctx, const vbmc_elbo_opts* opts, const char* who, int64_t* row_begin, int64_t* row_count);
 int upload_packed_mixture(vbmc_ctx* ctx);
 double* write_pack_to_device(vbmc_ctx* ctx);
+double* mix_fg_buffer(vbmc_ctx* ctx);
+inline size_t mix_fg_aux_off(const vbmc_ctx* ctx) { return (size_t)ctx->ml.total; }
+void write_aux_to_device(vbmc_ctx* ctx);
+int theta_to_mixture_host(vbmc_ctx* ctx, const double* theta, int n_theta, int optimize_mask, double* mu_KxD, double* sigma_K,
+                          double* lambd_D, double* w_K, double* eta_K);
 int set_mixture_host(vbmc_ctx* ctx, int D, int K, const double* mu_KxD, const double* sigma_K,
                      const double* lambd_D, const double* w_K, const double* eta_K, bool skip_if_same);
 
@@ -368,11 +377,7 @@
   int dev = 0;
 };
 
-__host__ __device__ inline uint64_t pack_ck_term(double v, uint32_t i) {
-  uint64_t b;
-  __builtin_memcpy(&b, &v, 8);
-  return b * (0x9E3779B97F4A7C15ull + 2ull * i);
-}
+__host__ __device__ inline uint64_t pack_ck_term(double v, uint32_t i) { return tpk::ck_term(v, i); }
 inline uint64_t pack_checksum(const double* p, size_t n) {
   uint64_t s0 = 0, s1 = 0, s2 = 0, s3 = 0;
   size_t i = 0;
@@ -421,6 +426,10 @@
 struct PrepArgs {
   const double* mix = nullptr;
   MixLayout ml;
+  const double* theta = nullptr;
+  const double* aux = nullptr;
+  int n_theta = 0, mask = 0;
+  double pow_2pi = 0.0;
   double* mix_copy = nullptr;
   int mix_copy_n = 0;
   uint64_t* ident_out = nullptr;
@@ -443,6 +452,10 @@
   GenSlice gen;
   DoneSignal done;
 };
+inline size_t prep_wire_lds(const MixLayout& ml, int n_theta, int K4, int DP) {
+  return sizeof(double) * ((size_t)n_theta + (size_t)ml.total + (size_t)K4 * DP);
+}
+inline bool prep_wire_fits(const MixLayout& ml, int n_theta, int K4, int DP) { return prep_wire_lds(ml, n_theta, K4, DP) <= 150 * 1024; }
 GenSlice make_gen_slice(double* eps, int K, int D, int64_t rows, int64_t n_half, int64_t row_begin,
                         uint64_t seed, const int* seed_add, double frac_begin, double frac_end);
 inline hipError_t stream_wait(vbmc_ctx* ctx) {
diff --git a/pyvbmc_amd/csrc/ctx.hip b/pyvbmc_amd/csrc/ctx.hip
--- a/pyvbmc_amd/csrc/ctx.hip
+++ b/pyvbmc_amd/csrc/ctx.hip
@@ -117,6 +117,8 @@
   c->opt_ws_roles = !(e && e[0] == '0');
   e = getenv("VBMC_MIX_BAR");
   c->opt_mix_bar = !(e && e[0] == '0');
+  e = getenv("VBMC_THETA_WIRE");
+  c->opt_theta_wire = !(e && e[0] == '0');
   e = getenv("VBMC_PREDICT_DMA");
   c->opt_predict_dma = !(e && e[0] == '0');
   e = getenv("VBMC_PREDICT_FUSED_FINISH");
@@ -335,6 +337,7 @@
   else if (!strcmp(key, "predict_dma")) ctx->opt_predict_dma = value != 0;
   else if (!strcmp(key, "predict_fused")) ctx->opt_predict_fused = value < 0 ? 0 : value > 2 ? 2 : value;
   else if (!strcmp(key, "mix_bar")) ctx->opt_mix_bar = value != 0;
+  else if (!strcmp(key, "theta_wire")) ctx->opt_theta_wire = value != 0;
   else if (!strcmp(key, "ws_span")) ctx->opt_ws_span = value != 0;
   else if (!strcmp(key, "ws_roles")) ctx->opt_ws_roles = value != 0;
   else if (!strcmp(key, "ws_pad")) ctx->opt_ws_pad = value > 8 ? 8 : value;
@@ -372,6 +375,11 @@
   return VBMC_OK;
 }
 
+int vbmc_theta_wire_fill(double* dst, const double* theta, int n, uint64_t* ck) {
+  if (!dst || !theta || n < 0 || !ck) return VBMC_E_ARG;
+  return tpk::wire_fill(dst, theta, n, ck) ? VBMC_E_NONFINITE : VBMC_OK;
+}
+
 int vbmc_last_entmc_plan(const vbmc_ctx* ctx, int out[4]) {
   if (!ctx || !out) return VBMC_E_ARG;
   for (int i = 0; i < 4; ++i) out[i] = ctx->last_plan[i];
@@ -399,29 +407,24 @@
 
 }
 
+double pack_pow_2pi(int D) { return std::pow(2.0 * M_PI, 0.5 * D); }
+
 void write_mixture_pack(const MixLayout& ml, const double* mu_KxD, const double* sigma,
                         const double* lambd, const double* w, double* p) {
   const int D = ml.D, K = ml.K;
-  double prod_lam = 1.0;
-  for (int d = 0; d < D; ++d) prod_lam *= lambd[d];
-  const double nconst = 1.0 / std::pow(2.0 * M_PI, 0.5 * D) / prod_lam;
-  const double l2n = std::log2(nconst);
+  const double nconst = tpk::norm_const(lambd, D, pack_pow_2pi(D));
+  const double l2n = tpk::log2_s(nconst);
   for (int k = 0; k < K; ++k) {
     for (int d = 0; d < D; ++d) {
       p[ml.o_mu + k * D + d] = mu_KxD[(size_t)k * D + d];
       p[ml.o_mup + k * D + d] = mu_KxD[(size_t)k * D + d] / lambd[d];
     }
-    const double s = sigma[k];
-    double sD = 1.0, b = s;
-    for (int e = D; e > 0; e >>= 1) {
-      if (e & 1) sD *= b;
-      b *= b;
-    }
-    p[ml.o_is2 + k] = 1.0 / (s * s);
-    p[ml.o_rc + k] = nconst / sD;
-    p[ml.o_lrc + k] = l2n - D * std::log2(s);
-    p[ml.o_wc + k] = w[k] * nconst / sD;
-    p[ml.o_sig + k] = s;
+    const tpk::PackK c = tpk::pack_component(sigma[k], w[k], D, nconst, l2n);
+    p[ml.o_is2 + k] = c.is2;
+    p[ml.o_rc + k] = c.rc;
+    p[ml.o_lrc + k] = c.lrc;
+    p[ml.o_wc + k] = c.wc;
+    p[ml.o_sig + k] = sigma[k];
     p[ml.o_w + k] = w[k];
   }
   for (int d = 0; d < D; ++d) {
@@ -450,26 +453,23 @@
   if (tm.o_mu())
     for (int i = 0; i < D * K; ++i) mu[i] = theta[i];
   if (tm.o_sg())
-    for (int k = 0; k < K; ++k) sg[k] = std::exp(theta[tm.p_sg + k]);
+    for (int k = 0; k < K; ++k) sg[k] = tpk::exp_s(theta[tm.p_sg + k]);
   if (tm.o_lm())
-    for (int d = 0; d < D; ++d) lm[d] = std::exp(theta[tm.p_lm + d]);
+    for (int d = 0; d < D; ++d) lm[d] = tpk::exp_s(theta[tm.p_lm + d]);
   if (tm.o_w()) {
     const double* e = theta + tm.p_w;
     double mx = e[0];
     for (int k = 1; k < K; ++k) mx = e[k] > mx ? e[k] : mx;
     for (int k = 0; k < K; ++k) {
       eta[k] = e[k] - mx;
-      w[k] = std::exp(eta[k]);
-    }
-  }
-  double s2 = 0.0;
-  for (int d = 0; d < D; ++d) s2 += lm[d] * lm[d];
-  const double nl = std::sqrt(s2 / D);
+      w[k] = tpk::exp_s(eta[k]);
+    }
+  }
+  const double nl = tpk::lambda_norm(lm, D);
   for (int d = 0; d < D; ++d) lm[d] /= nl;
   for (int k = 0; k < K; ++k) sg[k] *= nl;
   if (tm.o_w()) {
-    double ws = 0.0;
-    for (int k = 0; k < K; ++k) ws += w[k];
+    const double ws = tpk::sum16(w, K);
     for (int k = 0; k < K; ++k) w[k] /= ws;
   }
   return 0;
@@ -533,6 +533,24 @@
 }
 
 double* write_pack_to_device(vbmc_ctx* ctx) {
+  if (!mix_fg_buffer(ctx)) return nullptr;
+  memcpy(ctx->d_mix_fg, ctx->h_pack, (size_t)ctx->ml.total * sizeof(double));
+  __builtin_ia32_sfence();
+  ctx->pack_valid = true;
+  return ctx->d_mix_fg;
+}
+
+void write_aux_to_device(vbmc_ctx* ctx) {
+  if (ctx->aux_on_wire) return;
+  double* dst = ctx->d_mix_fg + mix_fg_aux_off(ctx);
+  for (const std::vector<double>* v : {&ctx->mu, &ctx->sigma, &ctx->lambd, &ctx->w}) {
+    memcpy(dst, v->data(), v->size() * sizeof(double));
+    dst += v->size();
+  }
+  ctx->aux_on_wire = true;
+}
+
+double* mix_fg_buffer(vbmc_ctx* ctx) {
   if (ctx->device < 0 || ctx->mix_fg_failed) return nullptr;
   const size_t n = (size_t)ctx->ml.total;
   if (ctx->d_mix_fg_cap < n) {
@@ -556,6 +574,7 @@
       return nullptr;
     }
     ctx->d_mix_fg_cap = want;
+    ctx->aux_on_wire = false;
   }
   if (!ctx->d_ctl) {
     if (hipExtMallocWithFlags((void**)&ctx->d_ctl, 64, hipDeviceMallocFinegrained) != hipSuccess) {
@@ -566,9 +585,6 @@
       __builtin_ia32_sfence();
     }
   }
-  memcpy(ctx->d_mix_fg, ctx->h_pack, n * sizeof(double));
-  __builtin_ia32_sfence();
-  ctx->pack_valid = true;
   return ctx->d_mix_fg;
 }
 
@@ -591,6 +607,8 @@
   ctx->pack_valid = true;
   return 0;
 }
+
+static int mixture_arrays_changed(vbmc_ctx* ctx);
 
 int set_mixture_host(vbmc_ctx* ctx, int D, int K, const double* mu_KxD, const double* sigma_K,
                      const double* lambd_D, const double* w_K, const double* eta_K, bool skip_if_same) {
@@ -604,7 +622,6 @@
     ctx->exp_eta_valid = false;
     return 0;
   }
-  ctx->pack_valid = false;
   ctx->D = D;
   ctx->K = K;
   ctx->mu.assign(mu_KxD, mu_KxD + (size_t)K * D);
@@ -615,6 +632,13 @@
     ctx->eta.assign(eta_K, eta_K + K);
   else
     ctx->eta.assign((size_t)K, 0.0);
+  return mixture_arrays_changed(ctx);
+}
+
+static int mixture_arrays_changed(vbmc_ctx* ctx) {
+  const int D = ctx->D, K = ctx->K;
+  ctx->pack_valid = false;
+  ctx->aux_on_wire = false;
   ctx->exp_eta_valid = false;
   for (int k = 0; k < K; ++k)
     if (!(ctx->sigma[k] > 0.0) || !std::isfinite(ctx->sigma[k]))
@@ -656,28 +680,31 @@
   if (!ctx || !theta) return VBMC_E_ARG;
   if (!ctx->mix_set) return vbmc_fail(ctx, VBMC_E_ARG, "theta_to_mixture: mixture (D,K) not set");
   if (ctx->device >= 0) HIP_TRY(ctx, hipSetDevice(ctx->device));
+  return theta_to_mixture_host(ctx, theta, n_theta, optimize_mask, mu_KxD, sigma_K, lambd_D, w_K, eta_K);
+}
+
+}
+
+int theta_to_mixture_host(vbmc_ctx* ctx, const double* theta, int n_theta, int optimize_mask, double* mu_KxD, double* sigma_K,
+                          double* lambd_D, double* w_K, double* eta_K) {
   const int D = ctx->D, K = ctx->K;
-  std::vector<double>&mu = ctx->t2m_mu, &sg = ctx->t2m_sg, &lm = ctx->t2m_lm, &w = ctx->t2m_w, &eta = ctx->t2m_eta;
-  mu = ctx->mu;
-  sg = ctx->sigma;
-  lm = ctx->lambd;
-  w = ctx->w;
-  eta = ctx->eta;
-  const int st = theta_to_arrays(D, K, theta, n_theta, optimize_mask, mu.data(), sg.data(), lm.data(),
-                                 w.data(), eta.data());
+  const int st = theta_to_arrays(D, K, theta, n_theta, optimize_mask, ctx->mu.data(), ctx->sigma.data(), ctx->lambd.data(),
+                                 ctx->w.data(), ctx->eta.data());
   if (st == -1)
     return vbmc_fail(ctx, VBMC_E_ARG, "theta length %d does not match D=%d K=%d mask=%d", n_theta, D, K,
                      optimize_mask);
   if (st == -2) return vbmc_fail(ctx, VBMC_E_NONFINITE, "theta has a non-finite entry");
-  int rc = set_mixture_host(ctx, D, K, mu.data(), sg.data(), lm.data(), w.data(), eta.data(), false);
+  int rc = mixture_arrays_changed(ctx);
   if (rc) return rc;
-  if (mu_KxD) memcpy(mu_KxD, mu.data(), sizeof(double) * D * K);
-  if (sigma_K) memcpy(sigma_K, sg.data(), sizeof(double) * K);
-  if (lambd_D) memcpy(lambd_D, lm.data(), sizeof(double) * D);
-  if (w_K) memcpy(w_K, w.data(), sizeof(double) * K);
-  if (eta_K) memcpy(eta_K, eta.data(), sizeof(double) * K);
-  return VBMC_OK;
-}
+  if (mu_KxD) memcpy(mu_KxD, ctx->mu.data(), sizeof(double) * D * K);
+  if (sigma_K) memcpy(sigma_K, ctx->sigma.data(), sizeof(double) * K);
+  if (lambd_D) memcpy(lambd_D, ctx->lambd.data(), sizeof(double) * D);
+  if (w_K) memcpy(w_K, ctx->w.data(), sizeof(double) * K);
+  if (eta_K) memcpy(eta_K, ctx->eta.data(), sizeof(double) * K);
+  return VBMC_OK;
+}
+
+extern "C" {
 
 static int upload_eps(vbmc_ctx* ctx, int K, int64_t n_half, int D, const double* eps_half, int64_t row_begin,
                       int64_t row_count) {
diff --git a/pyvbmc_amd/csrc/prep.hip b/pyvbmc_amd/csrc/prep.hip
--- a/pyvbmc_amd/csrc/prep.hip
+++ b/pyvbmc_amd/csrc/prep.hip
@@ -14,6 +14,101 @@
 
 __device__ __forceinline__ double wave_sum(double v) {
   return fm::wave_sum_dpp(v);
+}
+
+__device__ __forceinline__ void publish_checksum(uint64_t ck, uint64_t* out) {
+  __shared__ unsigned long long s_ck[16];
+  const int tid = threadIdx.x;
+  if (tid < 16) s_ck[tid] = 0;
+  __syncthreads();
+  atomicAdd(&s_ck[tid & 15], (unsigned long long)ck);
+  __syncthreads();
+  if (tid == 0) {
+    unsigned long long t = 0;
+#pragma unroll
+    for (int i = 0; i < 16; ++i) t += s_ck[i];
+    *out = t;
+  }
+}
+
+template <bool CK>
+__device__ __forceinline__ uint64_t wire_pack_block(const PrepArgs& a, double* th, double* p) {
+  __shared__ double s_red[4 + tpk::SUM_WAYS];
+  const MixLayout& ml = a.ml;
+  const int D = ml.D, K = ml.K, n = a.n_theta, tid = threadIdx.x;
+  const ThetaMap tm(D, K, a.mask, n);
+  uint64_t ck = 0;
+  constexpr int U = 8;
+  for (int base = 0; base < n; base += U * 256) {
+    double v[U];
+#pragma unroll
+    for (int u = 0; u < U; ++u) {
+      if (base + u * 256 >= n) break;
+      v[u] = a.theta[min(base + u * 256 + tid, n - 1)];
+    }
+#pragma unroll
+    for (int u = 0; u < U; ++u) {
+      if (base + u * 256 >= n) break;
+      const int i = base + u * 256 + tid;
+      if (i < n) {
+        th[i] = v[u];
+        if (CK) ck += pack_ck_term(v[u], (uint32_t)i);
+      }
+    }
+  }
+  if (a.mask != 15) {
+    const double* ax = a.aux;
+    if (!tm.o_mu())
+      for (int i = tid; i < K * D; i += 256) p[ml.o_mu + i] = ax[i];
+    if (!tm.o_sg())
+      for (int k = tid; k < K; k += 256) p[ml.o_sig + k] = ax[K * D + k];
+    if (!tm.o_lm())
+      for (int d = tid; d < D; d += 256) p[ml.o_lam + d] = ax[K * D + K + d];
+    if (!tm.o_w())
+      for (int k = tid; k < K; k += 256) p[ml.o_w + k] = ax[K * D + K + D + k];
+  }
+  __syncthreads();
+  if (tm.o_lm())
+    for (int d = tid; d < D; d += 256) p[ml.o_lam + d] = tpk::exp_s(th[tm.p_lm + d]);
+  if (tm.o_sg())
+    for (int k = tid; k < K; k += 256) p[ml.o_sig + k] = tpk::exp_s(th[tm.p_sg + k]);
+  if (tm.o_w()) {
+    double mx = -INFINITY;
+    for (int k = tid; k < K; k += 256) mx = fmax(mx, th[tm.p_w + k]);
+    mx = fm::wave_max_dpp(mx);
+    if ((tid & 63) == 0) s_red[tid >> 6] = mx;
+  }
+  __syncthreads();
+  const double nl = tpk::lambda_norm(p + ml.o_lam, D);
+  if (tm.o_w()) {
+    const double mx = fmax(fmax(s_red[0], s_red[1]), fmax(s_red[2], s_red[3]));
+    for (int k = tid; k < K; k += 256) p[ml.o_w + k] = tpk::exp_s(th[tm.p_w + k] - mx);
+  }
+  __syncthreads();
+  if (tm.o_w() && tid < tpk::SUM_WAYS) s_red[4 + tid] = tpk::sum16_partial(p + ml.o_w, K, tid);
+  for (int d = tid; d < D; d += 256) p[ml.o_lam + d] = p[ml.o_lam + d] / nl;
+  for (int k = tid; k < K; k += 256) p[ml.o_sig + k] = p[ml.o_sig + k] * nl;
+  __syncthreads();
+  const double ws = tm.o_w() ? tpk::sum16_combine(s_red + 4) : 1.0;
+  const double nconst = tpk::norm_const(p + ml.o_lam, D, a.pow_2pi);
+  const double l2n = tpk::log2_s(nconst);
+  for (int i = tid; i < K * D; i += 256) {
+    const double m = tm.o_mu() ? th[i] : p[ml.o_mu + i];
+    p[ml.o_mu + i] = m;
+    p[ml.o_mup + i] = m / p[ml.o_lam + i % D];
+  }
+  for (int k = tid; k < K; k += 256) {
+    const double w = tm.o_w() ? p[ml.o_w + k] / ws : p[ml.o_w + k];
+    const tpk::PackK c = tpk::pack_component(p[ml.o_sig + k], w, D, nconst, l2n);
+    p[ml.o_is2 + k] = c.is2;
+    p[ml.o_rc + k] = c.rc;
+    p[ml.o_lrc + k] = c.lrc;
+    p[ml.o_wc + k] = c.wc;
+    p[ml.o_w + k] = w;
+  }
+  for (int d = tid; d < D; d += 256) p[ml.o_ilam + d] = 1.0 / p[ml.o_lam + d];
+  __syncthreads();
+  return ck;
 }
 
 #ifdef FIN_TIMES
@@ -68,6 +163,21 @@
     __syncthreads();
     if (!s_go) return;
   }
+  if (a.theta) {
+    const bool copy = a.mix_copy && blockIdx.x == gridDim.x - 1;
+    if (!copy && (int)blockIdx.x >= a.n_table) return;
+    double* th = lds;
+    double* pack = th + a.n_theta;
+    if (copy) {
+      const uint64_t ck = wire_pack_block<true>(a, th, pack);
+      for (int i = tid; i < a.ml.total; i += 256) a.mix_copy[i] = pack[i];
+      if (a.ident_out) publish_checksum(ck, a.ident_out);
+    } else {
+      wire_pack_block<false>(a, th, pack);
+      ws_table_row_block(pack, a.ml, (int)blockIdx.x, a.DP, a.K4, a.table, pack + a.ml.total);
+    }
+    return;
+  }
   if (a.mix_copy && blockIdx.x == gridDim.x - 1) {
     uint64_t ck = 0;
     constexpr int U = 16;
@@ -89,19 +199,7 @@
         }
       }
     }
-    if (a.ident_out) {
-      __shared__ unsigned long long s_ck[16];
-      if (tid < 16) s_ck[tid] = 0;
-      __syncthreads();
-      atomicAdd(&s_ck[tid & 15], (unsigned long long)ck);
-      __syncthreads();
-      if (tid == 0) {
-        unsigned long long t = 0;
-#pragma unroll
-        for (int i = 0; i < 16; ++i) t += s_ck[i];
-        *a.ident_out = t;
-      }
-    }
+    if (a.ident_out) publish_checksum(ck, a.ident_out);
     return;
   }
   a.mix += (size_t)blockIdx.y * a.mix_stride;
@@ -163,6 +261,11 @@
     if (lt > 150 * 1024) return vbmc_fail(ctx, VBMC_E_UNSUP, "entropy table: K=%d D=%d too large", a.ml.K, D);
     lds = lt > lds ? lt : lds;
   }
+  if (a.theta) {
+    if (gblocks > 0 || a.batch != 1 || !prep_wire_fits(a.ml, a.n_theta, a.K4, a.DP))
+      return vbmc_fail(ctx, VBMC_E_ARG, "prep launch: the wire form does not apply to this launch");
+    lds = prep_wire_lds(a.ml, a.n_theta, a.K4, a.DP);
+  }
   if (lds > 64 * 1024)
     HIP_TRY(ctx, hipFuncSetAttribute((const void*)elbo_prep_kernel, hipFuncAttributeMaxDynamicSharedMemorySize, (int)lds));
   if (gblocks > 0) ++ctx->gp_launches;
diff --git a/pyvbmc_amd/csrc/theta_pack.h b/pyvbmc_amd/csrc/theta_pack.h
--- /dev/null
+++ b/pyvbmc_amd/csrc/theta_pack.h
@@ -0,0 +1,125 @@
+#pragma once
+#include <cmath>
+#include <cstdint>
+#include <cstring>
+
+#if defined(__HIPCC__)
+#define TPK_HD __host__ __device__
+#else
+#define TPK_HD
+#endif
+
+namespace tpk {
+
+TPK_HD inline double exp_s(double x) {
+  if (!(x <= 709.782712893384)) return x != x ? x : INFINITY;
+  if (x < -745.14) return 0.0;
+  const double k = rint(x * 1.44269504088896338700e+00);
+  const double hi = x - k * 6.93147180369123816490e-01;
+  const double lo = k * 1.90821492927058770002e-10;
+  const double r = hi - lo;
+  const double t = r * r;
+  const double c = r - t * (1.66666666666666019037e-01 +
+                            t * (-2.77777777770155933842e-03 +
+                                 t * (6.61375632143793436117e-05 + t * (-1.65339022054652515390e-06 + t * 4.13813679705723846039e-08))));
+  const double y = 1.0 - ((lo - (r * c) / (2.0 - c)) - hi);
+  return ldexp(y, (int)k);
+}
+
+TPK_HD inline double log2_s(double x) {
+  int e;
+  double m = frexp(x, &e);
+  if (m < 0.70710678118654752440) {
+    m *= 2.0;
+    e -= 1;
+  }
+  const double f = m - 1.0;
+  const double s = f / (2.0 + f);
+  const double z = s * s;
+  const double w = z * z;
+  const double t1 = w * (3.999999999940941908e-01 + w * (2.222219843214978396e-01 + w * 1.531383769920937332e-01));
+  const double t2 = z * (6.666666666666735130e-01 +
+                         w * (2.857142874366239149e-01 + w * (1.818357216161805012e-01 + w * 1.479819860511658591e-01)));
+  const double hfsq = 0.5 * f * f;
+  const double lm = f - (hfsq - s * (hfsq + (t2 + t1)));
+  return (double)e + lm * 1.44269504088896338700e+00;
+}
+
+constexpr int SUM_WAYS = 16;
+TPK_HD inline double sum16_partial(const double* v, int n, int j) {
+  double a = 0.0;
+  for (int i = j; i < n; i += SUM_WAYS) a += v[i];
+  return a;
+}
+TPK_HD inline double sum16_combine(const double* a) {
+  return (((a[0] + a[1]) + (a[2] + a[3])) + ((a[4] + a[5]) + (a[6] + a[7]))) +
+         (((a[8] + a[9]) + (a[10] + a[11])) + ((a[12] + a[13]) + (a[14] + a[15])));
+}
+TPK_HD inline double sum16(const double* v, int n) {
+  double a[SUM_WAYS];
+  for (int j = 0; j < SUM_WAYS; ++j) a[j] = sum16_partial(v, n, j);
+  return sum16_combine(a);
+}
+
+TPK_HD inline double lambda_norm(const double* lm_raw, int D) {
+  double s2 = 0.0;
+  for (int d = 0; d < D; ++d) s2 += lm_raw[d] * lm_raw[d];
+  return sqrt(s2 / D);
+}
+
+TPK_HD inline double norm_const(const double* lambd, int D, double pow_2pi) {
+  double prod_lam = 1.0;
+  for (int d = 0; d < D; ++d) prod_lam *= lambd[d];
+  return 1.0 / pow_2pi / prod_lam;
+}
+
+struct PackK {
+  double is2, wc, rc, lrc;
+};
+TPK_HD inline PackK pack_component(double s, double w, int D, double nconst, double l2n) {
+  double sD = 1.0, b = s;
+  for (int e = D; e > 0; e >>= 1) {
+    if (e & 1) sD *= b;
+    b *= b;
+  }
+  PackK r;
+  r.is2 = 1.0 / (s * s);
+  r.rc = nconst / sD;
+  r.lrc = l2n - D * log2_s(s);
+  r.wc = w * nconst / sD;
+  return r;
+}
+
+TPK_HD inline uint64_t ck_term(double v, uint32_t i) {
+  uint64_t b;
+  memcpy(&b, &v, 8);
+  return b * (0x9E3779B97F4A7C15ull + 2ull * i);
+}
+
+inline int wire_fill(double* dst, const double* theta, int n, uint64_t* ck_out) {
+  uint64_t s0 = 0, s1 = 0, s2 = 0, s3 = 0, bad = 0;
+  const uint64_t EXP = 0x7FF0000000000000ull;
+  int i = 0;
+  for (; i + 4 <= n; i += 4) {
+    uint64_t b[4];
+    memcpy(b, theta + i, 32);
+    memcpy(dst + i, b, 32);
+    bad |= (uint64_t)((b[0] & EXP) == EXP) | (uint64_t)((b[1] & EXP) == EXP) | (uint64_t)((b[2] & EXP) == EXP) |
+           (uint64_t)((b[3] & EXP) == EXP);
+    s0 += b[0] * (0x9E3779B97F4A7C15ull + 2ull * (uint32_t)i);
+    s1 += b[1] * (0x9E3779B97F4A7C15ull + 2ull * ((uint32_t)i + 1));
+    s2 += b[2] * (0x9E3779B97F4A7C15ull + 2ull * ((uint32_t)i + 2));
+    s3 += b[3] * (0x9E3779B97F4A7C15ull + 2ull * ((uint32_t)i + 3));
+  }
+  for (; i < n; ++i) {
+    uint64_t b;
+    memcpy(&b, theta + i, 8);
+    memcpy(dst + i, &b, 8);
+    bad |= (uint64_t)((b & EXP) == EXP);
+    s0 += b * (0x9E3779B97F4A7C15ull + 2ull * (uint32_t)i);
+  }
+  *ck_out = (s0 + s1) + (s2 + s3);
+  return bad ? -2 : 0;
+}
+
+}
```

Measured after the change: 11990 evals/s. 0.975x the previous value.
